# YiyanXu/DiFashion

Hardware: AMD Instinct MI355X
Metric: U-Net denoise steps/sec, 4-item outfit @ 64x64x4 latent (higher is better)
Workload: dtype bf16; 1 GPU; BASELINE configs[1]: one 4-item outfit, CFG on (4 branches) -> U-Net batch 16, DDIM-50 schedule, sd15 shape in_channels=8, 64x64x4 latents, 77 text tokens; one outfit per GPU; unet_batch=16, latent=64x64x4, parallelism=outfit-replicas x1 (no data-path collective)

## Files before the change

### difashion_amd/_lib.py

```python
from __future__ import annotations

import ctypes as C
import os
import subprocess

_HERE = os.path.dirname(os.path.abspath(__file__))
CSRC = os.path.join(_HERE, "csrc")
_LIB_NAMES = {"bf16": "libdifashion_hip.so", "fp16": "libdifashion_hip_f16.so"}


def _env_storage() -> str:
    v = (os.environ.get("DFH_STORAGE") or "bf16").strip().lower()
    if v not in _LIB_NAMES:
        raise ValueError(f"DFH_STORAGE={v!r}: the storage format is 'bf16' (default) or 'fp16'")
    return v


_STORAGE = _env_storage()
LIB_PATH = os.environ.get("DFH_LIB") or os.path.join(CSRC, _LIB_NAMES[_STORAGE])
HEADER = os.path.join(os.path.dirname(_HERE), "include", "difashion_hip.h")

DFH_MAX_BLOCKS = 4


# ... 210 lines not shown
    "dfh_imgproc_crop_top": (_i, [_vp]),
    "dfh_imgproc_crop_left": (_i, [_vp]),
    "dfh_imgproc_ksize_x": (_i, [_vp]),
    "dfh_imgproc_ksize_y": (_i, [_vp]),
    "dfh_imgproc_table_bytes": (_sz, [_vp]),
    "dfh_imgproc_fill_tables": (_i, [_vp, _vp, _sz]),
    "dfh_imgproc_run": (_i, [_vp, _vp, _vp, _vp, _i, _i, _vp, _vp, _vp]),
    "dfh_jpeg_quant_tables": (_i, [_i, C.POINTER(C.c_int), C.POINTER(C.c_int)]),
    "dfh_jpeg_workspace_bytes": (_sz, [_i, _i, _i, _i]),
    "dfh_jpeg_coef_count": (_sz, [_i, _i, _i, _i]),
    "dfh_jpeg_roundtrip": (_i, [_vp, _i, _i, _i, _i, _i, _i, _vp, _vp, _vp, _sz, _vp]),
    "dfh_lpips_create": (_i, [C.POINTER(LpipsConfigC), C.POINTER(_vp)]),
    "dfh_lpips_destroy": (None, [_vp]),
    "dfh_lpips_num_params": (_i, [_vp]),
    "dfh_lpips_param_name": (C.c_char_p, [_vp, _i]),
    "dfh_lpips_param_ndim": (_i, [_vp, _i]),
    "dfh_lpips_param_dim": (_i, [_vp, _i, _i]),
    "dfh_lpips_packed_bytes": (_sz, [_vp]),
    "dfh_lpips_pack": (_i, [_vp, C.POINTER(_vp), _i, _vp, _vp]),
    "dfh_lpips_workspace_bytes": (_sz, [_vp, _i, _i, _i]),
    "dfh_lpips_forward": (_i, [_vp, C.POINTER(_vp), _i, _vp, _vp, _vp, _i, _vp, _i, _i, _i, _i, _vp, _vp, _vp, _sz, _vp]),
    "dfh_lpips_group_argmin": (_i, [_vp, _vp, _i, _i, _vp]),
    "dfh_lpips_prep": (_i, [_vp, _i, _vp, _vp, _vp, _i, _vp, _i, _i, _i, _vp]),
    "dfh_lpips_conv3x3_relu": (_i, [_vp, _vp, _i, _vp, _vp, _vp, _i, _i, _i, _i, _i, _vp]),
    "dfh_lpips_maxpool2x2": (_i, [_vp, _vp, _i, _i, _i, _i, _vp]),
    "dfh_lpips_layer_score": (_i, [_vp, _vp, _i, _i, _i, _i, _vp, _vp, _vp]),
    "dfh_incep_create": (_i, [C.POINTER(IncepConfigC), C.POINTER(_vp)]),
    "dfh_incep_destroy": (None, [_vp]),
    "dfh_incep_num_params": (_i, [_vp]),
    "dfh_incep_param_name": (C.c_char_p, [_vp, _i]),
    "dfh_incep_param_ndim": (_i, [_vp, _i]),
    "dfh_incep_param_dim": (_i, [_vp, _i, _i]),
    "dfh_incep_packed_bytes": (_sz, [_vp]),
    "dfh_incep_pack": (_i, [_vp, C.POINTER(_vp), _i, _vp, _vp]),
    "dfh_incep_plan_count": (_i, [_vp, _i, _i, _i]),
    "dfh_incep_plan_entry": (_i, [_vp, _i, _i, _i, _i, C.POINTER(IncepLaunchC)]),
    "dfh_incep_workspace_bytes": (_sz, [_vp, _i, _i, _i]),
    "dfh_incep_forward": (_i, [_vp, C.POINTER(_vp), _i, _vp, _vp, _i, _i, _i, C.POINTER(_vp), _vp, _vp, _sz, _vp]),
    "dfh_incep_prep": (_i, [_vp, _i, _i, _i, _i, _i, _i, _vp, _vp]),
    "dfh_incep_conv_bn_relu": (_i, [_vp, _vp, _i, C.POINTER(_vp), _vp, _vp, _i, _i, _i, _i, _i, _i, _i, _i, _i, _i, _i, _i, _vp]),
    "dfh_incep_pool": (_i, [_vp, _vp, _i, _i, _i, _i, _i, _i, _i, _vp]),
    "dfh_incep_global_mean": (_i, [_vp, _vp, _i, _i, _i, _vp]),
    "dfh_incep_fc_softmax": (_i, [_vp, _vp, _vp, _vp, _vp, _i, _i, _i, _vp]),
    "dfh_incep_is_rows": (_i, [_vp, _vp, _i, _i, _f, _vp, _vp, _vp, _vp, _vp]),
    "dfh_incep_is_splits": (_i, [_vp, _vp, _vp, _i, _i, _vp, _vp]),
    "dfh_incep_stats": (_i, [_vp, _i, _i, _vp, _vp, _vp]),
    "dfh_vae_create": (_i, [C.POINTER(VAEConfigC), C.POINTER(_vp)]),
    "dfh_vae_destroy": (None, [_vp]),
    "dfh_vae_num_params": (_i, [_vp]),
    "dfh_vae_param_name": (C.c_char_p, [_vp, _i]),
    "dfh_vae_param_ndim": (_i, [_vp, _i]),
    "dfh_vae_param_dim": (_i, [_vp, _i, _i]),
    "dfh_vae_arena16_bytes": (_sz, [_vp]),
    "dfh_vae_arena32_bytes": (_sz, [_vp]),
    "dfh_vae_workspace_bytes": (_sz, [_vp, _i, _i, _i]),
    "dfh_vae_bind": (_i, [_vp, _vp, _vp, _vp, _sz]),
    "dfh_vae_pack": (_i, [_vp, C.POINTER(_vp), _i, _vp]),
    "dfh_vae_encode": (_i, [_vp, _vp, _vp, _i, _i, _vp]),
    "dfh_vae_decode": (_i, [_vp, _vp, _vp, _i, _i, _vp]),
    "dfh_unet_arena16t_bytes": (_sz, [_vp]),
    "dfh_unet_grad16_bytes": (_sz, [_vp]),
    "dfh_unet_grad32_bytes": (_sz, [_vp]),
    "dfh_unet_train_workspace_bytes": (_sz, [_vp, _i]),
    "dfh_unet_bind_train": (_i, [_vp, _vp, _vp, _vp, _vp, _sz, _i]),
    "dfh_unet_pack_train": (_i, [_vp, C.POINTER(_vp), _i, _vp]),
    "dfh_unet_pack_all": (_i, [_vp, C.POINTER(_vp), _i, _vp]),
    "dfh_unet_grad_sumsq": (_i, [_vp, _vp]),
    "dfh_unet_forward_train": (_i, [_vp, _vp, _i, _vp, _vp, _i, _vp, _i, _vp]),
    "dfh_unet_backward": (_i, [_vp, _vp, _vp, C.POINTER(_vp), _i, _i, _vp]),
    "dfh_unet_backward_begin": (_i, [_vp, _vp, _vp, _sz, _vp]),
    "dfh_unet_backward_next": (_i, [_vp, C.POINTER(_sz), C.POINTER(_sz), _vp]),
    "dfh_unet_backward_finish": (_i, [_vp, C.POINTER(_vp), _i, _i, _vp]),
    "dfh_gemm_partial_floats": (_sz, [C.POINTER(GemmDesc)]),
    "dfh_gemm": (_i, [C.POINTER(GemmDesc), _vp]),
    "dfh_gemm_wgrad": (_i, [C.POINTER(GemmDesc), _vp, _i, _vp, _i, _i, _vp]),
    "dfh_gemm_wgrad_partial_floats": (_sz, [C.POINTER(GemmDesc), _i]),
    "dfh_groupnorm_fold": (_i, [_vp, _i, _i, _i, _i, _vp, _vp, C.c_float, _vp, _i, _vp, _vp, _i, _i, _vp, _vp, _vp, _vp]),
    "dfh_gemm_wgrad_plan": (_i, [C.POINTER(GemmDesc), _i, C.POINTER(C.c_int), C.POINTER(C.c_int), C.POINTER(C.c_int)]),
    "dfh_gemm_plan": (_i, [C.POINTER(GemmDesc), C.POINTER(GemmPlanExtra), C.POINTER(GemmPlanInfo)]),
    "dfh_colsum": (_i, [_vp, _i, _i, _i, _i, _vp, _i, _vp]),
    "dfh_groupnorm": (_i, [_vp, _i, _vp, _i, _i, _i, _i, _vp, _vp, _f, _i, _vp, _vp, _vp]),
    "dfh_gemm_gstat": (_i, [C.POINTER(GemmDesc), _vp, C.POINTER(C.c_int)]),
    "dfh_groupnorm_pre": (_i, [_vp, _i, _i, _i, _i, _vp, _vp, _f, _i, _vp, _vp, _i, _vp, _vp]),
    "dfh_groupnorm_stats": (_i, [_vp, _i, _vp, _i, _i, _i, _i, _vp, _vp, _f, _i, _vp, _vp, _vp, _vp]),
    "dfh_groupnorm_bwd": (_i, [_vp, _i, _vp, _i, _vp, _i, _i, _i, _vp, _vp, _vp, _i, _vp, _i, _vp, _i, _vp, _vp, _vp, _vp]),
    "dfh_attention_lse": (_i, [_vp, _i, _vp, _i, _vp, _i, _vp, _i, _i, _i, _i, _i, _i, _f, _vp, _vp]),
    "dfh_attention_delta": (_i, [_vp, _vp, _i, _vp, _i, _i, _i, _i, _vp]),
    "dfh_attention_bwd": (_i, [_vp, _i, _vp, _i, _vp, _i, _vp, _i, _vp, _vp, _vp, _i, _vp, _i, _vp, _i, _i, _i, _i, _i, _i, _f, _vp]),
    "dfh_layernorm_bwd": (_i, [_vp, _vp, _vp, _vp, _i, _vp, _vp, _i, _i, _f, _vp]),
    "dfh_pack_matrix_t": (_i, [_vp, _vp, _i, _i, _i, _i, _i, _i, _vp]),
    "dfh_pack_conv3x3_t": (_i, [_vp, _vp, _i, _i, _i, _i, _i, _vp]),
    "dfh_unpack_matrix": (_i, [_vp, _vp, _i, _i, _i, _i, _i, _i, _vp]),
    "dfh_unpack_conv3x3": (_i, [_vp, _vp, _i, _i, _i, _i, _i, _vp]),
    "dfh_unpack_vector": (_i, [_vp, _vp, _i, _i, _i, _vp]),
    "dfh_pool2x2_sum": (_i, [_vp, _vp, _i, _i, _i, _i, _vp]),
    "dfh_add_bf16": (_i, [_vp, _vp, _sz, _i, _vp]),
    "dfh_geglu_fwd": (_i, [_vp, _vp, _sz, _i, _vp]),
    "dfh_geglu_bwd": (_i, [_vp, _vp, _vp, _sz, _i, _vp]),
    "dfh_act_fwd": (_i, [_vp, _vp, _sz, _i, _vp]),
    "dfh_act_bwd": (_i, [_vp, _vp, _vp, _vp, _vp, _sz, _i, _f, _vp]),
    "dfh_nhwc_to_nchw_f32": (_i, [_vp, _vp, _i, _i, _i, _i, _f, _i, _vp]),
    "dfh_transpose_bf16": (_i, [_vp, _vp, _i, _i, _i, _i, _i, _sz, _sz, _vp]),
    "dfh_mse_bwd": (_i, [_vp, _vp, _vp, _vp, _i, _i, _f, _vp, _vp]),
    "dfh_assemble_bwd": (_i, [_vp, _vp, _vp, _i, _i, _f, _vp]),
    "dfh_sumsq": (_i, [_vp, _sz, _vp, _vp]),
    "dfh_adamw": (_i, [_vp, _vp, _vp, _vp, _sz, _f, _f, _f, _f, _f, _i, _vp, _f, _vp]),
    "dfh_ema": (_i, [_vp, _vp, _sz, _f, _vp]),
    "dfh_adamw_ema": (_i, [_vp, _vp, _vp, _vp, _vp, _sz, _f, _f, _f, _f, _f, _i, _vp, _f, _f, _vp]),
    "dfh_q8_table": (_i, [_i, _vp]),
    "dfh_q8_quantize": (_i, [_vp, _vp, _vp, _sz, _i, _vp]),
    "dfh_q8_dequantize": (_i, [_vp, _vp, _vp, _sz, _i, _vp]),
    "dfh_adamw8": (_i, [_vp, _vp, _vp, _vp, _vp, _vp, _vp, _sz, _f, _f, _f, _f, _f, _i, _vp, _f, _f, _vp]),
    "dfh_wire_pack": (_i, [_vp, _vp, _sz, _sz, _vp]),
    "dfh_wire_shard_mean": (_i, [_vp, _vp, _i, _sz, _vp]),
    "dfh_wire_unpack": (_i, [_vp, _vp, _sz, _vp]),
    "dfh_layernorm": (_i, [_vp, _vp, _vp, _vp, _i, _i, _f, _vp]),
    "dfh_gemm_out2": (_i, [C.POINTER(GemmDesc), _vp, _i, _i, _vp]),
    "dfh_ups_phase_fold": (_i, [_vp, _i, _vp, _i, _i, _vp]),
    "dfh_conv_up2x": (_i, [_vp, _i, _i, _i, _i, _vp, _i, _vp, _vp, _vp, _vp]),
    "dfh_wino_weights": (_i, [_vp, _i, _vp, _i, _i, _i, _vp]),
    "dfh_wino_blocked": (_i, [_i, _i]),
    "dfh_prof_saved_flops": (C.c_double, []),
    "dfh_wino_input": (_i, [_vp, _vp, _i, _i, _i, _i, _vp]),
    "dfh_gn_wino_input_ok": (_i, [_i, _i, _i, _i, _i]),
    "dfh_gn_wino_input_chain": (_i, [_vp, _vp, _vp, _i, _i, _i, _vp, _vp, _f, _i, _vp, _i, _i, _i, _vp]),
    "dfh_gn_wino_input": (_i, [_vp, _i, _vp, _i, _vp, _vp, _f, _i, _vp, _i, _i, _i, _vp]),
    "dfh_conv3x3_wino_scratch_bytes": (C.c_size_t, [_i, _i, _i, _i, _i]),
    "dfh_conv3x3_wino": (_i, [_vp, _i, _i, _i, _i, _vp, _i, _i, _vp, _vp, _i, _i, _vp, _vp, _vp, C.c_size_t, _vp, _vp]),
    "dfh_gemm_batched": (_i, [C.POINTER(GemmDesc), _i, C.c_long, C.c_long, C.c_long, _vp]),
    "dfh_ln_fold": (_i, [_vp, _i, _vp, _vp, _vp, _vp, _vp, _vp, _i, _i, _vp]),
    "dfh_gemm_ln": (_i, [C.POINTER(GemmDesc), _vp, C.POINTER(C.c_int), _vp, _i, _i, _f, _vp, _vp]),
    "dfh_quantize_rows_fp8": (_i, [_vp, _i, _vp, _vp, _i, _i, _vp]),
    "dfh_layernorm_fp8": (_i, [_vp, _vp, _vp, _vp, _vp, _i, _i, _f, _vp]),
    "dfh_gemm_fp8": (_i, [C.POINTER(Fp8GemmDesc), _vp]),
    "dfh_mlp_fused_image_bytes": (_sz, []),
    "dfh_mlp_fused_pack": (_i, [_vp, _vp, _vp, _vp, _vp, _i, _vp]),
    "dfh_mlp_fused": (_i, [_vp, _vp, _vp, _vp, _i, _i, _f, _vp, _vp, _i, _i, _vp, _i, _i, _vp]),
    "dfh_groupnorm_fp8": (_i, [_vp, _i, _i, _i, _i, _f, _f, _vp, _vp, _vp]),
    "dfh_attention_fp8out": (_i, [_vp, _i, _vp, _i, _vp, _i, _vp, _i, _vp, _i, _i, _i, _i, _i, _f, _vp]),
    "dfh_amax_slabs": (_i, [_vp, C.c_long, _i, _i, _vp, _vp, _vp, _i, _i, _vp]),
    "dfh_attention_fp8": (_i, [_vp, _i, _vp, _i, _vp, _i, _vp, _i, _vp, _vp, _vp, _vp, _i, _i, _i, _i, _i, _f, _vp]),
    "dfh_attn_scales": (_i, [_vp, _vp, _i, _i, _vp, _vp, _vp, _vp, _vp]),
    "dfh_unet_enable_fp8": (_i, [_vp]),
    "dfh_unet_enable_fp8_attention": (_i, [_vp, _i]),
    "dfh_unet_arena8_bytes": (_sz, [_vp]),
    "dfh_unet_bind_fp8": (_i, [_vp, _vp]),
    "dfh_attention": (_i, [_vp, _i, _vp, _i, _vp, _i, _vp, _i, _i, _i, _i, _i, _i, _f, _vp]),
    "dfh_timestep_embedding": (_i, [_vp, _vp, _i, _i, _vp]),
    "dfh_nchw_to_nhwc_bf16": (_i, [_vp, _i, _vp, _i, _i, _i, _vp]),
    "dfh_cast_f32_to_bf16": (_i, [_vp, _vp, _sz, _vp]),
    "dfh_pack_conv3x3": (_i, [_vp, _vp, _i, _i, _i, _i, _vp]),
    "dfh_pack_matrix": (_i, [_vp, _vp, _i, _i, _i, _i, _i, _i, _vp]),
    "dfh_pack_vector": (_i, [_vp, _vp, _i, _i, _i, _i, _vp]),
    "dfh_mutual_reduce": (_i, [_vp, _vp, _vp, _vp, _vp, _vp, _i, _i, _i, _vp]),
    "dfh_assemble_input": (_i, [_vp, _vp, _vp, _vp, _vp, _vp, _vp, _i, _i, _i, _f, _f, _i, _vp]),
    "dfh_cfg_step": (_i, [_vp, _vp, _vp, _vp, _sz, _i, _f, _f, _f, C.POINTER(StepCoef), _vp]),
    "dfh_cfg_multistep": (_i, [_vp] * 9 + [_sz, _i, _f, _f, _f, C.POINTER(MultistepCoef), _vp]),
    "dfh_noise_mix": (_i, [_vp, _vp, _vp, _vp, _vp, _vp, _vp, _i, _i, _vp]),
    "dfh_mse_rows": (_i, [_vp, _vp, _vp, _i, _i, _vp]),
}
_NO_STATUS = {"dfh_abi_version", "dfh_census_count", "dfh_unet_num_params", "dfh_unet_param_ndim", "dfh_unet_param_dim", "dfh_vae_num_params",
              "dfh_vae_param_ndim", "dfh_vae_param_dim", "dfh_clip_num_params", "dfh_clip_param_ndim", "dfh_clip_param_dim",
              "dfh_clipv_num_params", "dfh_clipv_param_ndim", "dfh_clipv_param_dim", "dfh_lpips_num_params", "dfh_lpips_param_ndim", "dfh_lpips_param_dim",
              "dfh_imgproc_resized_height", "dfh_imgproc_resized_width", "dfh_imgproc_out_height", "dfh_imgproc_out_width", "dfh_imgproc_crop_top",
              "dfh_imgproc_crop_left", "dfh_imgproc_ksize_x", "dfh_imgproc_ksize_y",
              "dfh_incep_num_params", "dfh_incep_param_ndim", "dfh_incep_param_dim"}

_lib = None
_UNBOUND = set()
ABI_VERSION = 8


def storage() -> str:
    return _STORAGE


def set_storage(name: str) -> None:
    global _STORAGE, LIB_PATH
    name = str(name).strip().lower()
    if name not in _LIB_NAMES:
        raise ValueError(f"set_storage({name!r}): the storage format is 'bf16' or 'fp16'")
    if name == _STORAGE:
        return
    if _lib is not None:
        raise DfhError(f"set_storage({name!r}): the {_STORAGE} library is already loaded ({LIB_PATH}); the storage format is fixed "
                       "per process -- set DFH_STORAGE or call set_storage() before the first use")
    _STORAGE = name
    if not os.environ.get("DFH_LIB"):
        LIB_PATH = os.path.join(CSRC, _LIB_NAMES[name])


def storage_dtype():
    import torch
    return torch.float16 if _STORAGE == "fp16" else torch.bfloat16


def dtype_code(t, what: str = "tensor") -> int:
    import torch
    if t.dtype == torch.float32:
        return 0
    if t.dtype == storage_dtype():
        return 1
# ... 144 lines not shown
```

### difashion_amd/csrc/api.hip

```cpp
#include <cstdio>
#include <cstdlib>
#include <cstring>
#include <string>
#include <vector>

#include "../../include/difashion_hip.h"
#include "attention.h"
#include "dfh_common.h"
#include "elementwise.h"
#include "gemm.h"
#include "gemm_plan.h"
#include "mlp_fused.h"
#include "norm.h"
#include "walk_knobs.h"
#include "wgrad.h"
#include "bwd_elementwise.h"

namespace dfh {
static thread_local std::string g_err;
void set_error(const std::string& msg) { g_err = msg; }
const char* last_error() { return g_err.c_str(); }
int check_launch(const char* what) {
  hipError_t e = hipGetLastError();
  if (e != hipSuccess) {
    g_err = std::string(what) + ": " + hipGetErrorString(e);
    return -2;
  }
  return 0;
}

static long g_census[CK_COUNT] = {0};
void census(int id) { if (id >= 0 && id < CK_COUNT) ++g_census[id]; }
static const char* const kCensusNames[CK_COUNT] = {"gemm_wide", "gemm_8wave", "gemm_lean", "gemm_other", "gemm_row", "splitk_reduce",
    "splitk_fused", "gstat_written", "gn_pre", "gn_stats", "gn_small", "gn_mid", "layernorm", "ln_folded", "attention_x32", "attention_16",
    "gemm_fp8", "text_cached", "conv_phase", "conv_wino", "gemm_rows_geglu", "attention_fp8", "mlp_fused", "gn_folded", "token_linear", "dup_prefix", "gemm_persist",
    "clipv_embed", "clipv_linear", "clipv_layernorm", "clipv_attention", "imgproc", "cliph_attention", "cliph_embed"};

struct ProfRec { hipEvent_t e0, e1; int cls; double flops, bytes; };
static std::vector<ProfRec> g_recs;
static std::vector<hipEvent_t> g_pool;
static size_t g_pool_next = 0;
static bool g_prof = false;
bool prof_enabled() { return g_prof; }
static hipEvent_t pool_get() {
  if (g_pool_next == g_pool.size()) { hipEvent_t e; (void)hipEventCreate(&e); g_pool.push_back(e); }
  return g_pool[g_pool_next++];
}
void prof_open(int cls, double flops, double bytes, hipStream_t s) {
  ProfRec r; r.e0 = pool_get(); r.e1 = pool_get(); r.cls = cls; r.flops = flops; r.bytes = bytes;
  (void)hipEventRecord(r.e0, s);
  g_recs.push_back(r);
}
void prof_close(hipStream_t s) { (void)hipEventRecord(g_recs.back().e1, s); }
static double g_prof_saved = 0.0;
void prof_note_saved(double flops) { if (g_prof) g_prof_saved += flops; }
}

static int fill_gemm(const dfh_gemm_desc* d, GemmArgs* g) {
  DFH_REQUIRE(d != nullptr, "null descriptor");
  std::memset(g, 0, sizeof(*g));
  if (d->conv) {
    DFH_REQUIRE(d->stride == 1 || d->stride == 2, "stride must be 1 or 2");
    DFH_REQUIRE(!(d->upsample && d->stride != 1), "upsample only with stride 1");
    g->conv_src = (const bf16_t*)d->conv_src; g->conv_c = d->conv_c; g->ntaps = 9;
    g->Hin = d->Hin; g->Win = d->Win; g->stride = d->stride; g->ups = d->upsample;
    g->Hout = d->upsample ? d->Hin * 2 : (d->stride == 2 ? d->Hin / 2 : d->Hin);
    g->Wout = d->upsample ? d->Win * 2 : (d->stride == 2 ? d->Win / 2 : d->Win);
    DFH_REQUIRE(d->M == d->batch * g->Hout * g->Wout, "M must equal batch * Hout * Wout");
  }
  if (d->a0) { g->p_src[g->nplain] = (const bf16_t*)d->a0; g->p_c[g->nplain] = d->a0_c; ++g->nplain; }
  if (d->a1) { DFH_REQUIRE(d->a0 != nullptr, "a1 without a0"); g->p_src[g->nplain] = (const bf16_t*)d->a1; g->p_c[g->nplain] = d->a1_c; ++g->nplain; }
  g->W = (const bf16_t*)d->W; g->ldw = d->ldw; g->zero = (const bf16_t*)d->zero_page;
  g->M = d->M; g->N = d->N;
  g->bias = d->bias; g->rowvec = d->rowvec; g->rv_ld = d->rv_ld; g->rv_off = d->rv_off;
  g->rows_per_b = d->rows_per_b > 0 ? d->rows_per_b : d->M;
  g->w_img_bs = (long)d->w_img_stride;
  g->resid = (const bf16_t*)d->resid; g->ld_res = d->ld_res;
  g->act = d->act; g->out = d->out; g->ld_out = d->ld_out; g->out_mode = d->out_mode;
  g->partial = d->partial;
  DFH_REQUIRE(g->W && g->out, "null W / out");
  return 0;
}

extern "C" {

int dfh_abi_version(void) { return DFH_ABI_VERSION; }

int dfh_prof_begin(void) {
  dfh::g_recs.clear(); dfh::g_pool_next = 0; dfh::g_prof = true; dfh::g_prof_saved = 0.0;
  return 0;
}
double dfh_prof_saved_flops(void) { return dfh::g_prof_saved; }
int dfh_prof_end(dfh_prof_class* out, int max_classes) {
  dfh::g_prof = false;
  DFH_REQUIRE(out != nullptr && max_classes >= dfh::PC_COUNT, "need room for every kernel class");
  static const char* names[dfh::PC_COUNT] = {"gemm_conv3x3", "gemm_linear", "attention", "groupnorm", "layernorm", "splitk_reduce", "other",
                                                  "gemm_wgrad", "attention_bwd", "norm_bwd", "optimizer", "gemm_linear_fp8"};
  for (int i = 0; i < dfh::PC_COUNT; ++i) {
    std::memset(&out[i], 0, sizeof(out[i]));
    std::strncpy(out[i].name, names[i], sizeof(out[i].name) - 1);
  }
  if (hipDeviceSynchronize() != hipSuccess) { dfh::set_error("hipDeviceSynchronize failed in dfh_prof_end"); return -2; }
  const char* dump_path = std::getenv("DFH_PROF_DUMP");
  FILE* dump = dump_path ? std::fopen(dump_path, "w") : nullptr;
  for (const auto& r : dfh::g_recs) {
    float ms = 0.f;
    if (hipEventElapsedTime(&ms, r.e0, r.e1) != hipSuccess) continue;
    out[r.cls].launches += 1; out[r.cls].ms += ms; out[r.cls].flops += r.flops; out[r.cls].bytes += r.bytes;
    if (dump) std::fprintf(dump, "%s %.0f %.0f %.6f\n", names[r.cls], r.flops, r.bytes, ms);
  }
  if (dump) std::fclose(dump);
  dfh::g_recs.clear();
  return dfh::PC_COUNT;
}
void dfh_census_reset(void) { std::memset(dfh::g_census, 0, sizeof(dfh::g_census)); }
int dfh_census_count(void) { return dfh::CK_COUNT; }
const char* dfh_census_name(int i) { return (i >= 0 && i < dfh::CK_COUNT) ? dfh::kCensusNames[i] : ""; }
// ... 50 lines not shown
  w.partial = d->partial; w.partial_cap = d->partial_floats;
  return 0;
}

int dfh_gemm_wgrad(const dfh_gemm_desc* d, const void* dY, int ldy, float* dW, int ldw, int msplit, void* stream) {
  DFH_BF16_ONLY_TRAINING;
  DFH_REQUIRE(d && dY && dW, "null argument");
  WgradArgs w;
  if (int rc = fill_wgrad(d, dY, ldy, dW, ldw, msplit, w)) return rc;
  return dfh::wgrad_launch(w, (hipStream_t)stream);
}

size_t dfh_gemm_wgrad_partial_floats(const dfh_gemm_desc* d, int msplit) {
  DFH_BF16_ONLY_TRAINING_SIZE;
  WgradArgs w;
  if (!d || fill_wgrad(d, nullptr, 8, nullptr, 8, msplit, w)) return 0;
  return dfh::wgrad_partial_floats(w);
}

int dfh_gemm_wgrad_plan(const dfh_gemm_desc* d, int msplit, int* tiles, int* whole_tiles, int* slices) {
  DFH_BF16_ONLY_TRAINING;
  WgradArgs w;
  DFH_REQUIRE(d && tiles && whole_tiles && slices, "null argument");
  if (int rc = fill_wgrad(d, nullptr, 8, nullptr, 8, msplit, w)) return rc;
  dfh::wgrad_plan_only(w);
  *tiles = w.xblocks; *whole_tiles = w.whole; *slices = w.msplit;
  return 0;
}

int dfh_gemm_plan(const dfh_gemm_desc* d, const dfh_gemm_plan_extra* x, dfh_gemm_plan_info* out) {
  DFH_REQUIRE(d && out, "null argument");
  std::memset(out, 0, sizeof(*out));
  static float present[4];
  dfh_gemm_desc t = *d;
  if (!t.W) t.W = present;
  if (!t.out) t.out = present;
  if (!t.zero_page) t.zero_page = present;
  if (!t.partial) t.partial = present;
  GemmArgs g;
  if (int rc = fill_gemm(&t, &g)) return rc;
  if (d->gstat_cpg > 0 && d->gstat_hw > 0) { g.gstat = present; g.gstat_cpg = d->gstat_cpg; g.gstat_hw = d->gstat_hw; }
  if (x) {
    g.nbatch = x->nbatch; g.w_blocked = x->w_blocked;
    if (x->phase2x) { g.phase2x = x->phase2x; g.ntaps = 4; g.nbatch = 4; }
    if (x->n_split > 0) { g.out2 = present; g.ld_out2 = g.rows_per_b; g.n_split = x->n_split; }
    if (x->want_rowstat) g.rowstat = present;
    if (x->ln_cnt > 0) { g.ln_stat = present; g.ln_s = present; g.ln_cnt = x->ln_cnt; g.ln_parts = g.p_c[0] / x->ln_cnt; g.ln_eps = 1e-5f; }
    if (x->pre_out) { g.pre_out = present; g.ld_pre = g.N; }
  }
  const GemmArgs given = g;
  dfh::GemmPlan p;
  const int rc = dfh::gemm_plan(g, dfh::gemm_force_decode(d->force_tile, d->force_split, d->force_order), dfh::GemmKnobs::from_env(), p);
  dfh::gemm_plan_format(out->line, sizeof(out->line), given, rc ? nullptr : &p, rc ? dfh::last_error() : nullptr);
  if (rc) return rc;
  out->kernel = p.kernel; out->tile = p.tile; out->bm = p.bm; out->bn = p.bn; out->stages = p.stages; out->lean = p.lean; out->wide = p.wide;
  out->split = p.split; out->n_major = p.n_major; out->tm_xm = p.tm_xm; out->tm_gm = p.tm_gm; out->gstat_rows = p.gstat_rows;
  out->rowstat_bn = p.rowstat_bn; out->census = p.census;
  return 0;
}

int dfh_colsum(const void* Y, int ldy, int N, int groups, int rows_per_group, float* out, int ld_out, void* stream) {
  DFH_BF16_ONLY_TRAINING;
  DFH_REQUIRE(Y && out, "null argument");
  return dfh::colsum_launch((const bf16_t*)Y, ldy, N, groups, rows_per_group, out, ld_out, (hipStream_t)stream);
}

int dfh_groupnorm(const void* src0, int c0, const void* src1, int c1, int batch, int hw, int groups, const float* gamma,
                  const float* beta, float eps, int silu, void* out, float* partial, void* stream) {
  GnArgs a; std::memset(&a, 0, sizeof(a));
  a.src0 = (const bf16_t*)src0; a.C0 = c0; a.src1 = (const bf16_t*)src1; a.C1 = src1 ? c1 : 0;
  a.B = batch; a.HW = hw; a.G = groups; a.gamma = gamma; a.beta = beta; a.eps = eps; a.silu = silu;
  a.out = (bf16_t*)out; a.partial = partial;
  return dfh::groupnorm_launch(a, (hipStream_t)stream);
}

int dfh_groupnorm_pre(const void* src, int c, int batch, int hw, int groups, const float* gamma, const float* beta, float eps, int silu,
                      void* out, const float* gstat, int chunks, float* stats_out, void* stream) {
  GnArgs a; std::memset(&a, 0, sizeof(a));
  a.src0 = (const bf16_t*)src; a.C0 = c; a.B = batch; a.HW = hw; a.G = groups; a.gamma = gamma; a.beta = beta; a.eps = eps;
  a.silu = silu; a.out = (bf16_t*)out; a.pre = gstat; a.pre_chunks = chunks; a.stats_out = stats_out;
  return dfh::groupnorm_launch(a, (hipStream_t)stream);
}

int dfh_groupnorm_stats(const void* src0, int c0, const void* src1, int c1, int batch, int hw, int groups, const float* gamma,
                        const float* beta, float eps, int silu, void* out, float* partial, float* stats_out, void* stream) {
  GnArgs a; std::memset(&a, 0, sizeof(a));
  a.src0 = (const bf16_t*)src0; a.C0 = c0; a.src1 = (const bf16_t*)src1; a.C1 = src1 ? c1 : 0;
  a.B = batch; a.HW = hw; a.G = groups; a.gamma = gamma; a.beta = beta; a.eps = eps; a.silu = silu;
  a.out = (bf16_t*)out; a.partial = partial; a.stats_out = stats_out;
  return dfh::groupnorm_launch(a, (hipStream_t)stream);
}
int dfh_groupnorm_bwd(const void* src0, int c0, const void* src1, int c1, const void* dy, int batch, int hw, int groups,
                      const float* gamma, const float* beta, const float* stats, int silu, void* dx0, int acc0, void* dx1,
                      int acc1, float* dgamma, float* dbeta, float* partial, void* stream) {
  DFH_BF16_ONLY_TRAINING;
  GnBwdArgs a; std::memset(&a, 0, sizeof(a));
  a.src0 = (const bf16_t*)src0; a.C0 = c0; a.src1 = (const bf16_t*)src1; a.C1 = src1 ? c1 : 0; a.dy = (const bf16_t*)dy;
  a.B = batch; a.HW = hw; a.G = groups; a.gamma = gamma; a.beta = beta; a.stats = stats; a.silu = silu;
  a.dx0 = (bf16_t*)dx0; a.dx1 = (bf16_t*)dx1; a.acc0 = acc0; a.acc1 = acc1; a.dgamma = dgamma; a.dbeta = dbeta; a.partial = partial;
  return dfh::groupnorm_bwd_launch(a, (hipStream_t)stream);
}
int dfh_attention_lse(const void* Q, int ldq, const void* K, int ldk, const void* Vt, int ldvt, void* O, int ldo, int batch,
                      int heads, int head_dim, int Nq, int Nk, float scale, float* lse, void* stream) {
  AttnArgs a; std::memset(&a, 0, sizeof(a));
  a.Q = (const bf16_t*)Q; a.ldq = ldq; a.K = (const bf16_t*)K; a.ldk = ldk; a.Vt = (const bf16_t*)Vt; a.ldvt = ldvt;
  a.O = (bf16_t*)O; a.ldo = ldo; a.B = batch; a.H = heads; a.D = head_dim; a.Nq = Nq; a.Nk = Nk; a.scale = scale; a.lse = lse;
  return dfh::attention_launch(a, (hipStream_t)stream);
}
int dfh_attention_delta(const void* O, const void* dO, int ld, float* delta, int batch, int heads, int head_dim, int Nq, void* stream) {
  DFH_BF16_ONLY_TRAINING;
  return dfh::attention_delta_launch((const bf16_t*)O, (const bf16_t*)dO, ld, delta, batch, heads, head_dim, Nq, (hipStream_t)stream);
}
int dfh_attention_bwd(const void* Q, int ldq, const void* K, int ldk, const void* V, int ldv, const void* dO, int ldo,
                      const float* lse, const float* delta, void* dQ, int lddq, void* dK, int lddk, void* dV, int lddv, int batch,
                      int heads, int head_dim, int Nq, int Nk, float scale, void* stream) {
  DFH_BF16_ONLY_TRAINING;
  AttnBwdArgs a; std::memset(&a, 0, sizeof(a));
  a.Q = (const bf16_t*)Q; a.ldq = ldq; a.K = (const bf16_t*)K; a.ldk = ldk; a.V = (const bf16_t*)V; a.ldv = ldv;
  a.dO = (const bf16_t*)dO; a.ldo = ldo; a.lse = lse; a.delta = delta;
  a.dQ = (bf16_t*)dQ; a.lddq = lddq; a.dK = (bf16_t*)dK; a.lddk = lddk; a.dV = (bf16_t*)dV; a.lddv = lddv;
  a.B = batch; a.H = heads; a.D = head_dim; a.Nq = Nq; a.Nk = Nk; a.scale = scale;
  return dfh::attention_bwd_launch(a, (hipStream_t)stream);
}
int dfh_layernorm_bwd(const void* x, const void* dy, const float* gamma, void* dx, int accumulate, float* dgamma, float* dbeta,
                      int M, int C, float eps, void* stream) {
  DFH_BF16_ONLY_TRAINING;
  return dfh::layernorm_bwd_launch((const bf16_t*)x, (const bf16_t*)dy, gamma, (bf16_t*)dx, accumulate, dgamma, dbeta, M, C, eps,
                                   (hipStream_t)stream);
}
int dfh_pack_matrix_t(const float* w, void* out, int N, int K, int ldt, int t_row_off, int t_col_off, int geglu, void* stream) {
  DFH_BF16_ONLY_TRAINING;
  return dfh::pack_matrix_t_launch(w, (bf16_t*)out, N, K, ldt, t_row_off, t_col_off, geglu, (hipStream_t)stream);
}
int dfh_pack_conv3x3_t(const float* w, void* out, int Cout, int Cin, int ldt, int t_col_off, int o_pad, void* stream) {
  DFH_BF16_ONLY_TRAINING;
  return dfh::pack_conv3x3_t_launch(w, (bf16_t*)out, Cout, Cin, ldt, t_col_off, o_pad, (hipStream_t)stream);
}
int dfh_unpack_matrix(const float* g, float* grad, int N, int K, int ldw, int row_off, int col_off, int geglu, void* stream) {
  DFH_BF16_ONLY_TRAINING;
  return dfh::unpack_matrix_launch(g, grad, N, K, ldw, row_off, col_off, geglu, (hipStream_t)stream);
}
int dfh_unpack_conv3x3(const float* g, float* grad, int Cout, int Cin, int ldw, int col_off, int cin_pad, void* stream) {
  DFH_BF16_ONLY_TRAINING;
  return dfh::unpack_conv3x3_launch(g, grad, Cout, Cin, ldw, col_off, cin_pad, (hipStream_t)stream);
}
int dfh_unpack_vector(const float* g, float* grad, int N, int off, int geglu, void* stream) {
  DFH_BF16_ONLY_TRAINING;
  return dfh::unpack_vector_launch(g, grad, N, off, geglu, (hipStream_t)stream);
}
int dfh_pool2x2_sum(const void* in, void* out, int batch, int H, int W, int C, void* stream) {
  return dfh::pool2x2_sum_launch((const bf16_t*)in, (bf16_t*)out, batch, H, W, C, (hipStream_t)stream);
}
int dfh_add_bf16(void* dst, const void* src, size_t n, int accumulate, void* stream) {
  return dfh::add_bf16_launch((bf16_t*)dst, (const bf16_t*)src, (long)n, accumulate, (hipStream_t)stream);
}
int dfh_geglu_fwd(const void* pre, void* y, size_t M, int N2, void* stream) {
  return dfh::geglu_fwd_launch((const bf16_t*)pre, (bf16_t*)y, (long)M, N2, (hipStream_t)stream);
}
int dfh_geglu_bwd(const void* pre, const void* dy, void* dpre, size_t M, int N2, void* stream) {
  DFH_BF16_ONLY_TRAINING;
  return dfh::geglu_bwd_launch((const bf16_t*)pre, (const bf16_t*)dy, (bf16_t*)dpre, (long)M, N2, (hipStream_t)stream);
}
int dfh_act_fwd(const void* pre, void* y, size_t n, int kind, void* stream) {
  return dfh::act_fwd_launch((const bf16_t*)pre, (bf16_t*)y, (long)n, kind, (hipStream_t)stream);
}
int dfh_act_bwd(const void* ref_bf16, const float* ref_f32, const void* dy_bf16, const float* dy_f32, void* dpre, size_t n, int kind,
// ... 48 lines not shown
}
int dfh_q8_dequantize(const unsigned char* codes, const float* absmax, float* x, size_t n, int is_signed, void* stream) {
  DFH_BF16_ONLY_TRAINING;
  DFH_REQUIRE(x != nullptr && codes != nullptr && absmax != nullptr, "null pointer");
  return dfh::q8_dequantize_launch(codes, absmax, x, (long)n, is_signed, (hipStream_t)stream);
}
int dfh_adamw8(float* p, const float* g, unsigned char* m8, float* m_absmax, unsigned char* v8, float* v_absmax, float* shadow, size_t n,
               float lr, float beta1, float beta2, float eps, float weight_decay, int step, const float* sumsq, float max_norm,
               float ema_decay, void* stream) {
  DFH_BF16_ONLY_TRAINING;
  DFH_REQUIRE(p != nullptr && g != nullptr && m8 != nullptr && m_absmax != nullptr && v8 != nullptr && v_absmax != nullptr, "null pointer");
  return dfh::adamw8_launch(p, g, m8, m_absmax, v8, v_absmax, shadow, (long)n, lr, beta1, beta2, eps, weight_decay, step, sumsq, max_norm,
                            ema_decay, (hipStream_t)stream);
}

int dfh_wire_pack(const float* g, void* wire, size_t n, size_t n_pad, void* stream) {
  DFH_BF16_ONLY_TRAINING;
  return dfh::wire_pack_launch(g, (bf16_t*)wire, (long)n, (long)n_pad, (hipStream_t)stream);
}
int dfh_wire_shard_mean(const void* recv, void* shard, int world, size_t per, void* stream) {
  DFH_BF16_ONLY_TRAINING;
  return dfh::wire_shard_mean_launch((const bf16_t*)recv, (bf16_t*)shard, world, (long)per, (hipStream_t)stream);
}
int dfh_wire_unpack(const void* wire, float* g, size_t n, void* stream) {
  DFH_BF16_ONLY_TRAINING;
  return dfh::wire_unpack_launch((const bf16_t*)wire, g, (long)n, (hipStream_t)stream);
}

int dfh_layernorm(const void* x, const float* gamma, const float* beta, void* y, int M, int C, float eps, void* stream) {
  return dfh::layernorm_launch((const bf16_t*)x, gamma, beta, (bf16_t*)y, M, C, eps, (hipStream_t)stream);
}

int dfh_groupnorm_fold(const void* x, int B, int HW, int C, int G, const float* gamma, const float* beta, float eps, const float* pre,
                       int pre_chunks, float* partial, const void* W, int ldw, int N, const float* bias, void* Wimg, float* rv, void* stream) {
  GnFoldArgs f; std::memset(&f, 0, sizeof(f));
  f.x = (const bf16_t*)x; f.B = B; f.HW = HW; f.C = C; f.G = G; f.eps = eps; f.gamma = gamma; f.beta = beta; f.pre = pre; f.pre_chunks = pre_chunks;
  f.partial = partial; f.W = (const bf16_t*)W; f.ldw = ldw; f.N = N; f.bias = bias; f.Wimg = (bf16_t*)Wimg; f.rv = rv;
  return dfh::groupnorm_fold_launch(f, (hipStream_t)stream);
}

int dfh_ln_fold(const void* W, int ldw, const float* gamma, const float* beta, const float* bias, void* WF, float* s, float* b, int N, int K,
                void* stream) {
  return dfh::ln_fold_launch((const bf16_t*)W, ldw, gamma, beta, bias, (bf16_t*)WF, s, b, N, K, (hipStream_t)stream);
}

int dfh_gemm_ln(const dfh_gemm_desc* d, float* rowstat, int* rowstat_bn, const float* ln_stat, int ln_parts, int ln_cnt, float ln_eps,
                const float* ln_s, void* stream) {
  GemmArgs g;
  if (int rc = fill_gemm(d, &g)) return rc;
  const size_t need = d->force_split > 1 ? (size_t)d->force_split * g.M * g.N : dfh::gemm_partial_floats(g);
  DFH_REQUIRE(need == 0 || (d->partial && d->partial_floats >= need), "partial buffer too small for split-K");
  g.rowstat = rowstat;
  g.ln_stat = ln_stat; g.ln_parts = ln_parts; g.ln_cnt = ln_cnt; g.ln_eps = ln_eps; g.ln_s = ln_s;
  if (ln_stat) DFH_REQUIRE(dfh::gemm_ln_consumer_ok(g), "this launch shape cannot consume folded-LayerNorm statistics (split-K / unstaged GEGLU)");
  int bn = 0;
  const int rc = dfh::gemm_launch(g, (hipStream_t)stream, d->force_tile, d->force_split, d->force_order, nullptr, &bn);
  if (rowstat_bn) *rowstat_bn = bn;
  return rc;
}

int dfh_gemm_out2(const dfh_gemm_desc* d, void* out2, int ld_out2, int n_split, void* stream) {
  GemmArgs g;
  if (int rc = fill_gemm(d, &g)) return rc;
  DFH_REQUIRE(out2 != nullptr, "null argument");
  g.out2 = out2; g.ld_out2 = ld_out2; g.n_split = n_split;
  DFH_REQUIRE(dfh::gemm_out2_ok(g), "this launch cannot carry a second destination (split-K, or n_split is no multiple of its column tile)");
  const int ft = (d->force_tile == 10 || d->force_tile == 24) ? d->force_tile : 0;
  return dfh::gemm_launch(g, (hipStream_t)stream, ft, 0, d->force_order);
}

int dfh_ups_phase_fold(const void* W, int ldw, void* WP, int N, int C, void* stream) {
  return dfh::ups_phase_fold_launch((const bf16_t*)W, ldw, (bf16_t*)WP, N, C, (hipStream_t)stream);
}
int dfh_conv_up2x(const void* src, int batch, int H, int W, int C, const void* WP, int N, const float* bias, void* out,
                  const void* zero_page, void* stream) {
  DFH_REQUIRE(src && WP && out && zero_page, "null argument");
  DFH_REQUIRE(batch > 0 && H > 0 && W > 0 && C > 0 && C % 8 == 0 && N > 0 && N % 8 == 0, "bad shape (C and N multiples of 8)");
  GemmArgs g; std::memset(&g, 0, sizeof(g));
  g.M = batch * H * W; g.N = N; g.rows_per_b = H * W; g.out_mode = OUT_BF16; g.ld_out = N;
  g.conv_src = (const bf16_t*)src; g.conv_c = C; g.ntaps = 4; g.phase2x = 1; g.nbatch = 4; g.w_bs = (long)N * 4 * C;
  g.Hin = H; g.Win = W; g.Hout = H; g.Wout = W; g.stride = 1;
  g.W = (const bf16_t*)WP; g.ldw = 4 * C; g.bias = bias; g.out = out; g.zero = (const bf16_t*)zero_page;
  return dfh::gemm_launch(g, (hipStream_t)stream, 0, 0, -1);
}
int dfh_wino_weights(const void* W, int ldw, void* U, int N, int C, int blocked, void* stream) {
  return dfh::wino_weight_launch((const bf16_t*)W, ldw, (bf16_t*)U, N, C, blocked, (hipStream_t)stream);
}
int dfh_wino_blocked(int N, int C) { return dfh::wino_blocked(N, C) ? 1 : 0; }
int dfh_wino_input(const void* src, void* V, int batch, int H, int W, int C, void* stream) {
  return dfh::wino_input_launch((const bf16_t*)src, (bf16_t*)V, batch, H, W, C, (hipStream_t)stream);
}
int dfh_gn_wino_input_ok(int c0, int c1, int groups, int H, int W) { return dfh::gn_wino_ok(c0, c1, groups, H, W) ? 1 : 0; }
int dfh_gn_wino_input(const void* src0, int c0, const void* src1, int c1, const float* gamma, const float* beta, float eps, int groups,
                      void* V, int batch, int H, int W, void* stream) {
  return dfh::gn_wino_input_launch((const bf16_t*)src0, c0, (const bf16_t*)src1, c1, gamma, beta, eps, groups, (bf16_t*)V, batch, H, W,
                                   (hipStream_t)stream);
}
int dfh_gn_wino_input_chain(const void* Mprev, const float* pbias, const float* prowvec, int prv_ld, int prv_off, int C, const float* gamma,
                            const float* beta, float eps, int groups, void* V, int batch, int H, int W, void* stream) {
  DFH_REQUIRE(Mprev != nullptr, "null argument");
  return dfh::gn_wino_input_launch((const bf16_t*)Mprev, C, nullptr, 0, gamma, beta, eps, groups, (bf16_t*)V, batch, H, W, (hipStream_t)stream,
                                   (const bf16_t*)Mprev, pbias, prowvec, prv_ld, prv_off);
}
size_t dfh_conv3x3_wino_scratch_bytes(int batch, int H, int W, int C, int N) {
  if (batch <= 0 || H <= 0 || W <= 0 || C <= 0 || N <= 0) return 0;
  const size_t mt = (size_t)batch * (H / 2) * (W / 2);
  return ((16 * mt * C * 2 + 255) & ~(size_t)255) + ((16 * mt * N * 2 + 255) & ~(size_t)255);
}
int dfh_conv3x3_wino(const void* src, int batch, int H, int W, int C, const void* U, int u_blocked, int N, const float* bias, const float* rowvec,
                     int rv_ld, int rv_off, const void* resid, void* out, void* scratch, size_t scratch_bytes, const void* zero_page,
                     void* stream) {
  DFH_REQUIRE(src && U && bias && out && scratch && zero_page, "null argument");
  DFH_REQUIRE(batch > 0 && H > 0 && W > 0 && (H & 1) == 0 && (W & 1) == 0 && C > 0 && C % 8 == 0 && N > 0 && N % 8 == 0,
              "even image sides, channel counts multiples of 8");
  DFH_REQUIRE(scratch_bytes >= dfh_conv3x3_wino_scratch_bytes(batch, H, W, C, N) && (uintptr_t)scratch % 256 == 0, "scratch too small or misaligned");
  const long mt = (long)batch * (H / 2) * (W / 2);
  bf16_t* V = (bf16_t*)scratch;
  bf16_t* Mb = (bf16_t*)((char*)scratch + ((16 * (size_t)mt * C * 2 + 255) & ~(size_t)255));
  hipStream_t s = (hipStream_t)stream;
  if (int rc = dfh::wino_input_launch((const bf16_t*)src, V, batch, H, W, C, s)) return rc;
  GemmArgs g; std::memset(&g, 0, sizeof(g));
  g.M = (int)mt; g.N = N; g.rows_per_b = (int)mt; g.out_mode = OUT_BF16; g.ld_out = N;
  g.p_src[0] = V; g.p_c[0] = C; g.nplain = 1; g.W = (const bf16_t*)U; g.ldw = C;
  g.nbatch = 16; g.a_bs = mt * C; g.w_bs = (long)N * C; g.o_bs = mt * N; g.w_blocked = u_blocked;
  g.out = Mb; g.zero = (const bf16_t*)zero_page;
  g.prof_flops = 2.0 * batch * H * W * (double)N * 9.0 * C;
  if (int rc = dfh::gemm_launch(g, s, dfh::wino_gemm_tile(g), 0, -1)) return rc;
  return dfh::wino_output_launch(Mb, (bf16_t*)out, bias, rowvec, rv_ld, rv_off, (const bf16_t*)resid, batch, H, W, N, s);
}
int dfh_gemm_batched(const dfh_gemm_desc* d, int nbatch, long a_bs, long w_bs, long o_bs, void* stream) {
  GemmArgs g;
  if (int rc = fill_gemm(d, &g)) return rc;
  DFH_REQUIRE(nbatch >= 1, "nbatch must be positive");
  g.nbatch = nbatch; g.a_bs = a_bs; g.w_bs = w_bs; g.o_bs = o_bs;
  return dfh::gemm_launch(g, (hipStream_t)stream, d->force_tile, 0, d->force_order);
}

int dfh_gemm_fp8(const dfh_gemm_fp8_desc* d, void* stream) {
  DFH_BF16_ONLY_FP8;
  DFH_REQUIRE(d != nullptr, "null descriptor");
  Fp8GemmArgs g; std::memset(&g, 0, sizeof(g));
  g.A = (const uint8_t*)d->A; g.lda = d->lda; g.sA = d->sA; g.sa_div = d->sa_div; g.sa_mul = d->sa_mul; g.sx = (const uint8_t*)d->sx;
  g.W = (const uint8_t*)d->W; g.sW = d->sW; g.M = d->M; g.N = d->N; g.K = d->K; g.bias = d->bias;
  g.resid = (const bf16_t*)d->resid; g.ld_res = d->ld_res; g.act = d->act; g.out = d->out; g.ld_out = d->ld_out; g.out_mode = d->out_mode;
  g.out_sx = (uint8_t*)d->out_sx; g.rows_per_b = d->rows_per_b; g.amax = d->amax; g.zero = (const uint8_t*)d->zero_page;
  return dfh::gemm_fp8_launch(g, (hipStream_t)stream);
}
size_t dfh_mlp_fused_image_bytes(void) { return dfh::mlp_fused_image_bytes(); }
int dfh_mlp_fused_pack(const void* w1, const float* s1, const float* b1, const void* w2p, void* img, int form, void* stream) {
#ifdef DFH_PROBES
  if (form == 1) return dfh::mlp_pack_launch((const bf16_t*)w1, s1, b1, (const bf16_t*)w2p, img, (hipStream_t)stream);
#endif
  DFH_REQUIRE(form == 2, "fused MLP: form 2 (form 1 is a probe kernel: scripts/probes)");
  return dfh::mlp2_pack_launch((const bf16_t*)w1, s1, b1, (const bf16_t*)w2p, img, (hipStream_t)stream);
}
int dfh_mlp_fused(const void* x, const void* resid, const void* img, const float* ln_stat, int ln_parts, int ln_cnt, float ln_eps,
                  const float* bias, void* out, int M, int form, float* gstat, int gstat_cpg, int gstat_hw, void* stream) {
#ifndef DFH_PROBES
  DFH_REQUIRE(form == 2, "fused MLP: form 2 (form 1 is a probe kernel: scripts/probes)");
#endif
  DFH_REQUIRE(form == 1 || form == 2, "fused MLP: form 1 or 2");
  DFH_REQUIRE(gstat == nullptr || form == 2, "fused MLP: output statistics are written by form 2 only");
  MlpArgs a; std::memset(&a, 0, sizeof(a));
  a.gstat = gstat; a.gstat_cpg = gstat_cpg; a.gstat_hw = gstat_hw;
  a.x = (const bf16_t*)x; a.resid = (const bf16_t*)resid; a.img = (const unsigned char*)img; a.ln_stat = ln_stat; a.ln_parts = ln_parts;
  a.ln_cnt = ln_cnt; a.ln_eps = ln_eps; a.bias = bias; a.out = (bf16_t*)out; a.M = M;
// ... 136 lines not shown
```

### difashion_amd/csrc/dfh_common.h

```cpp
#pragma once
#include <hip/hip_runtime.h>
#include <stdint.h>

typedef uint16_t bf16_t;

typedef __attribute__((ext_vector_type(4))) float f32x4_t;
typedef __attribute__((ext_vector_type(2))) float f32x2_t;

#define DFH_DEVICE __device__ __forceinline__

#ifdef DFH_F16
#define DFH_STORAGE_NAME "fp16"
typedef __attribute__((ext_vector_type(8))) _Float16 h16x8_t;
typedef __attribute__((ext_vector_type(2))) _Float16 h16x2_t;
#define DFH_MFMA_16x16x32 __builtin_amdgcn_mfma_f32_16x16x32_f16
#define DFH_MFMA_32x32x16 __builtin_amdgcn_mfma_f32_32x32x16_f16
#define DFH_MFMA_16x16x32_ASM "v_mfma_f32_16x16x32_f16"
#define DFH_MFMA_32x32x16_ASM "v_mfma_f32_32x32x16_f16"
#define DFH_H16_ONE 0x3C00
#define DFH_H16_ONE2 0x3c003c00u
#define DFH_H16_ONE_LO 0x00003c00u
constexpr bool DFH_H16_WIDE_EXPONENT = false;
constexpr float DFH_H16_MAX = 65504.0f;

// ... 140 lines not shown

DFH_DEVICE uint2 geglu4p(const f32x4_t v, const f32x4_t g, const float4 bv, const float4 bg, const GeluK& k, uint2& pre_v, uint2& pre_g) {
  const f32x2_t v0 = f32x2_t{v[0] + bv.x, v[1] + bv.y}, v1 = f32x2_t{v[2] + bv.z, v[3] + bv.w};
  const f32x2_t g0 = f32x2_t{g[0] + bg.x, g[1] + bg.y}, g1 = f32x2_t{g[2] + bg.z, g[3] + bg.w};
  pre_v.x = pack2bf(v0[0], v0[1]); pre_v.y = pack2bf(v1[0], v1[1]);
  pre_g.x = pack2bf(g0[0], g0[1]); pre_g.y = pack2bf(g1[0], g1[1]);
  const f32x2_t o0 = v0 * gelu_erf_f2(g0, k), o1 = v1 * gelu_erf_f2(g1, k);
  uint2 o;
  o.x = pack2bf(o0[0], o0[1]); o.y = pack2bf(o1[0], o1[1]);
  return o;
}

DFH_DEVICE float lane_xor16(float x) {
  const unsigned u = __float_as_uint(x);
  const auto r = __builtin_amdgcn_permlane16_swap(u, u, false, false);
  const bool odd_row = (__lane_id() & 16) != 0;
  return __uint_as_float(odd_row ? r[0] : r[1]);
}
DFH_DEVICE float lane_xor32(float x) {
  const unsigned u = __float_as_uint(x);
  const auto r = __builtin_amdgcn_permlane32_swap(u, u, false, false);
  const bool upper = (__lane_id() & 32) != 0;
  return __uint_as_float(upper ? r[0] : r[1]);
}
DFH_DEVICE float rows_max(float x) {
  unsigned u = __float_as_uint(x);
  auto r = __builtin_amdgcn_permlane16_swap(u, u, false, false);
  u = __float_as_uint(fmaxf(__uint_as_float(r[0]), __uint_as_float(r[1])));
  r = __builtin_amdgcn_permlane32_swap(u, u, false, false);
  return fmaxf(__uint_as_float(r[0]), __uint_as_float(r[1]));
}
DFH_DEVICE float rows_sum(float x) {
  unsigned u = __float_as_uint(x);
  auto r = __builtin_amdgcn_permlane16_swap(u, u, false, false);
  u = __float_as_uint(__uint_as_float(r[0]) + __uint_as_float(r[1]));
  r = __builtin_amdgcn_permlane32_swap(u, u, false, false);
  return __uint_as_float(r[0]) + __uint_as_float(r[1]);
}
DFH_DEVICE float wave_sum(float v) {
#pragma unroll
  for (int o = 8; o > 0; o >>= 1) v += __shfl_xor(v, o, 64);
  return rows_sum(v);
}

#include <string>
#include <vector>
namespace dfh {
struct ParamDesc { std::string name; std::vector<int> shape; };
struct ParamList {
  std::vector<ParamDesc> params;
  int add_param(const std::string& name, std::vector<int> shape) { params.push_back({name, std::move(shape)}); return (int)params.size() - 1; }
  int num_params() const { return (int)params.size(); }
  const char* param_name(int i) const { return i >= 0 && i < num_params() ? params[i].name.c_str() : ""; }
  int param_ndim(int i) const { return i >= 0 && i < num_params() ? (int)params[i].shape.size() : 0; }
  int param_dim(int i, int d) const { return d >= 0 && d < param_ndim(i) ? params[i].shape[d] : 0; }
};
void set_error(const std::string& msg);
const char* last_error();
int check_launch(const char* what);
struct WorkspaceCarve {
  float* base; size_t round, floats = 0;
  WorkspaceCarve(void* b, size_t round_floats) : base((float*)b), round(round_floats) {}
  float* take(size_t n) { float* p = base ? base + floats : nullptr; floats += (n + round - 1) / round * round; return p; }
  size_t bytes() const { return floats * sizeof(float) + 256; }
};
template <class NameOf>
int check_param_pointers(const float* const* params, int count, const std::string& who, NameOf name_of) {
  for (int i = 0; i < count; ++i) {
    const char* fault = params[i] == nullptr ? "null parameter pointer" : ((uintptr_t)params[i] & 15) != 0 ? "parameter pointer not 16-byte aligned" : nullptr;
    if (fault) { set_error(who + ": " + fault + name_of(i)); return -1; }
  }
  return 0;
}
inline int require_params(const ParamList& t, const float* const* params, int count, const std::string& who, const std::string& count_query,
                          const std::string& arg = "params") {
  if (!params) { set_error(who + ": null argument: " + arg); return -1; }
  if (count != t.num_params()) { set_error(who + ": " + arg + " count does not match " + count_query); return -1; }
  return check_param_pointers(params, count, who, [&](int i) { return ": " + t.params[i].name; });
}
inline bool aligned16(const void* p) { return ((uintptr_t)p & 15) == 0; }
enum ProfClass { PC_CONV3 = 0, PC_LINEAR = 1, PC_ATTN = 2, PC_GNORM = 3, PC_LNORM = 4, PC_SPLITK = 5, PC_OTHER = 6,
                 PC_WGRAD = 7, PC_ATTN_BWD = 8, PC_NORM_BWD = 9, PC_OPTIM = 10, PC_LINEAR_FP8 = 11, PC_COUNT = 12 };
enum CensusId { CK_GEMM_WIDE = 0, CK_GEMM_8WAVE, CK_GEMM_LEAN, CK_GEMM_OTHER, CK_GEMM_ROW, CK_SPLITK, CK_SPLITK_FUSED, CK_GSTAT_WRITTEN,
                CK_GN_PRE, CK_GN_STATS, CK_GN_SMALL, CK_GN_MID, CK_LAYERNORM, CK_LN_FOLDED, CK_ATTN_X32, CK_ATTN_16, CK_GEMM_FP8,
                CK_TEXT_CACHED, CK_CONV_PHASE, CK_CONV_WINO, CK_GEMM_ROWS_GEGLU, CK_ATTN_FP8, CK_MLP_FUSED, CK_GN_FOLDED, CK_TOKEN_LINEAR, CK_DUP_PREFIX, CK_GEMM_PERSIST,
                CK_CLIPV_EMBED, CK_CLIPV_LINEAR, CK_CLIPV_LAYERNORM, CK_CLIPV_ATTN, CK_IMGPROC, CK_CLIPH_ATTN, CK_CLIPH_EMBED, CK_COUNT };
void census(int id);
bool prof_enabled();
void prof_open(int cls, double flops, double bytes, hipStream_t s);
void prof_close(hipStream_t s);
void prof_note_saved(double flops);
struct ProfScope {
  hipStream_t s; bool on;
  ProfScope(int cls, double flops, double bytes, hipStream_t st) : s(st), on(prof_enabled()) { if (on) prof_open(cls, flops, bytes, s); }
  ~ProfScope() { if (on) prof_close(s); }
};
}
#define DFH_REQUIRE(cond, msg)                                   \
  do {                                                           \
    if (!(cond)) {                                               \
      dfh::set_error(std::string(__func__) + ": " + (msg));      \
      return -1;                                                 \
    }                                                            \
  } while (0)

#ifdef DFH_F16
#define DFH_BF16_ONLY_TRAINING_SIZE do { dfh::set_error(std::string(__func__) + ": refused by the fp16-storage library: training entry points are bf16 only; unset DFH_STORAGE"); return 0; } while (0)
#define DFH_BF16_ONLY_TRAINING DFH_REQUIRE(false, "refused by the fp16-storage library: training / backward / optimizer entry points are bf16 only (no loss scaling); unset DFH_STORAGE")
#define DFH_BF16_ONLY_FP8 DFH_REQUIRE(false, "refused by the fp16-storage library: the fp8 (e4m3) legs are calibrated against bf16 producers; unset DFH_STORAGE")
#else
#define DFH_BF16_ONLY_TRAINING
#define DFH_BF16_ONLY_TRAINING_SIZE
#define DFH_BF16_ONLY_FP8
#endif

DFH_DEVICE int xcd_remap(int bid, int nblk) {
  const int q = nblk >> 3, r = nblk & 7;
  const int xcd = bid & 7, idx = bid >> 3;
  const int base = (xcd < r) ? xcd * (q + 1) : r * (q + 1) + (xcd - r) * q;
  return base + idx;
}

DFH_DEVICE void tile_coords(int bid, int ntm, int ntn, int n_major, int xm, int gm, int& mt, int& nt) {
  if (gm <= 0) {
    const int tile = xcd_remap(bid, ntm * ntn);
    mt = n_major ? tile % ntm : tile / ntn;
    nt = n_major ? tile / ntm : tile % ntn;
    return;
  }
  int rm = ntm, rn = ntn, mbase = 0, nbase = 0, idx;
  const int xn = xm > 0 ? 8 / xm : 0;
  if (xm > 0 && ntm % xm == 0 && ntn % xn == 0) {
    const int xcd = bid & 7;
    rm = ntm / xm; rn = ntn / xn;
    mbase = (xcd / xn) * rm; nbase = (xcd % xn) * rn;
    idx = bid >> 3;
  } else {
    idx = xcd_remap(bid, ntm * ntn);
  }
  const int per = gm * rn, group = idx / per, first = group * gm;
  const int gsz = (rm - first) < gm ? (rm - first) : gm;
  const int w = idx - group * per;
  mt = mbase + first + w % gsz;
  nt = nbase + w / gsz;
}
```

### difashion_amd/csrc/gemm_plan.h

```cpp
#pragma once
#include <stddef.h>
#include "gemm.h"
#include "norm.h"

namespace dfh {

struct GemmForce {
  int tile;
  bool deep;
  bool big, bigg;
  int wide;
  int ws;
  bool halo, persist, token;
  int split, order;
  bool kernel_pinned() const { return wide || ws || halo; }
  bool none() const { return tile == 0 && !kernel_pinned(); }
};
GemmForce gemm_force_decode(int force_tile, int force_split, int force_order);

struct GemmKnobs {
  bool deep4_off, deep4_all;
  int tmap_xm, tmap_gm;
  int big_mode;
  int bigg_mode;
  bool w_blocked_off;
  int wino_tile;
  bool batch_big_off;
  bool batch_nmajor_off;
  bool gstat128_off;
  bool ws_on, halo_on;
  int persist_mode;
  static GemmKnobs defaults();
  static const GemmKnobs& from_env();
};

enum GemmKernel { GK_TILE = 0, GK_BIG, GK_BIG_GEGLU, GK_WIDE,
                  GK_WS, GK_HALO, GK_GEGLU_ROWS, GK_PERSIST, GK_TOKEN_LINEAR,
                  GK_COUNT };
struct GemmTile { int bm, bn, stages; };
extern const GemmTile kGemmTiles[6];
constexpr int kEightWave = 5;

struct GemmPlan {
  int kernel;
  int tile;
  int bm, bn, stages, lean;
  int wide;
  int split;
  int n_major, tm_xm, tm_gm;
  int gstat_rows;
  int rowstat_bn;
  int census;
};

int gemm_plan(GemmArgs& a, const GemmForce& f, const GemmKnobs& k, GemmPlan& p);

bool gemm_lean_plain(const GemmArgs& a);
void gemm_plan_stats(GemmArgs& a, const GemmKnobs& k, GemmPlan& p);
inline bool gstat_chunks_fit(int hw, int rows) { return hw % rows == 0 && hw / rows <= (int)GN_MAX_CHUNKS; }

struct GemmWork { double flops, saved, bytes; int cls; };
GemmWork gemm_work(const GemmArgs& a);

const char* gemm_kernel_name(int kernel);
int gemm_plan_format(char* buf, size_t n, const GemmArgs& given, const GemmPlan* p, const char* refusal);

#ifdef DFH_PROBES
int gemm_plan_probes(GemmArgs& a, const GemmForce& f, const GemmKnobs& k, GemmPlan& p, bool wide_ok);
int gemm_launch_probes(const GemmPlan& p, const GemmArgs& a, hipStream_t stream);
#endif
}
```

### difashion_amd/csrc/gemm_plan.hip

```cpp
#include "gemm_plan.h"

#include <algorithm>
#include <cstdio>
#include <cstdlib>
#include <cstring>
#include <string>

namespace dfh {

namespace {
constexpr int BK = 64;
constexpr int BKW = 32;
constexpr int kNumTiles = 5;
}

const GemmTile kGemmTiles[6] = {{256, 160, 3}, {256, 128, 3}, {128, 64, 3}, {128, 160, 2}, {128, 128, 2}, {128, 160, 2}};

GemmForce gemm_force_decode(int force_tile, int force_split, int force_order) {
  GemmForce f{};
  f.split = force_split; f.order = force_order;
  switch (force_tile) {
    case GF_8WAVE: f.deep = true; break;
    case GF_WS_160: f.ws = 160; break;
    case GF_WS_128: f.ws = 128; break;
    case GF_HALO: f.halo = true; break;
    case GF_BIG: f.big = true; break;
    case GF_BIG_GEGLU: f.bigg = true; break;
    case GF_PERSIST: f.persist = true; break;
    case GF_TOKEN_LINEAR: f.token = true;
    default:
      if (force_tile > kNumTiles) f.wide = force_tile - GF_WIDE + 1;
      else f.tile = force_tile;
  }
  return f;
}

GemmKnobs GemmKnobs::defaults() {
  GemmKnobs k{};
  k.deep4_all = true; k.tmap_xm = -1; k.big_mode = 2; k.bigg_mode = 1; k.wino_tile = -1;
  return k;
}

const GemmKnobs& GemmKnobs::from_env() {
  static const GemmKnobs knobs = [] {
    GemmKnobs k = defaults();
    const auto is = [](const char* name, char c) { const char* e = getenv(name); return e && e[0] == c; };
    const auto num = [](const char* name, int dflt) { const char* e = getenv(name); return e ? atoi(e) : dflt; };
    k.deep4_off = is("DFH_DEEP4", '0');
    k.deep4_all = !is("DFH_DEEP4", '1');
    if (const char* e = getenv("DFH_TMAP")) { const char* c = strchr(e, ','); k.tmap_xm = atoi(e); k.tmap_gm = c ? atoi(c + 1) : 0; }
    k.big_mode = num("DFH_GEMM_BIG", k.big_mode);
    k.bigg_mode = num("DFH_GEMM_BIGG", k.bigg_mode);
    k.w_blocked_off = is("DFH_W_BLOCKED", '0');
    k.wino_tile = num("DFH_WINO_TILE", k.wino_tile);
    k.batch_big_off = is("DFH_BATCH_BIG", '0');
    k.batch_nmajor_off = is("DFH_BATCH_NMAJOR", '0');
    k.gstat128_off = is("DFH_GSTAT128", '0');
    k.ws_on = is("DFH_GEMM_WS", '1'); k.halo_on = is("DFH_GEMM_HALO", '1'); k.persist_mode = num("DFH_PERSIST", 0);
    return k;
  }();
  return knobs;
}

int gemm_count_ksteps(const GemmArgs& a) {
  int n = a.ntaps * ((a.conv_c + BK - 1) / BK);
  for (int i = 0; i < a.nplain; ++i) n += (a.p_c[i] + BK - 1) / BK;
  return n;
}

int gemm_wide_ksteps(const GemmArgs& a) {
  int n = a.ntaps * ((a.conv_c + BKW - 1) / BKW);
  for (int i = 0; i < a.nplain; ++i) n += (a.p_c[i] + BKW - 1) / BKW;
  return n;
}

bool gemm_lean_plain(const GemmArgs& a) {
  if (a.ntaps != 0 || a.nplain < 1 || a.p_c[0] % BK != 0 || a.p_c[0] <= 0) return false;
  const double amax = (double)a.M * std::max(a.p_c[0], a.nplain > 1 ? a.p_c[1] : 0) * 2.0, wmax = (double)a.N * a.ldw * 2.0;
  if (amax >= 4.0e9 || wmax >= 4.0e9) return false;
  return a.nplain == 1 || (a.p_c[1] % BK == 0 && a.p_c[1] > 0);
}

int gemm_pick_split(const GemmArgs& a, int* tile_out) {
  const bool geglu = a.act == ACT_GEGLU;
  const bool n160 = !geglu && (a.N % 160 == 0 || (a.N % 128 != 0 && a.N > 128));
  const int ksteps = gemm_count_ksteps(a);
  if (gemm_act_is_xact(a.act)) {
    if (tile_out) *tile_out = kEightWave;
    return 1;
  }
  int tile;
  if (a.N <= 64 && !geglu) tile = 2;
  else if (a.M > 128 && a.M <= 1024 && ksteps >= 64) tile = n160 ? 0 : 1;
  else tile = n160 ? kEightWave : 4;
  const GemmTile ti = kGemmTiles[tile];
  const int blocks = ((a.M + ti.bm - 1) / ti.bm) * ((a.N + ti.bn - 1) / ti.bn);
  int split = 1;
  if (!geglu && blocks < 384 && ksteps >= (a.ntaps ? 64 : 160)) {
    const int target = ti.bm == 256 ? 256 : 512;
    split = std::max(1, std::min((target + blocks / 2) / blocks, ksteps / 16));
  } else if (!geglu && blocks < 160 && ksteps >= 16) {
    split = std::min({(256 + blocks - 1) / blocks, ksteps / 8, 64});
    if (split < 1) split = 1;
  }
  if (tile_out) *tile_out = tile;
  return split;
}

size_t gemm_partial_floats(const GemmArgs& a) {
  if (a.nbatch > 1) return 0;
  const int s = gemm_pick_split(a, nullptr);
  return s > 1 ? (size_t)s * a.M * a.N : 0;
}

static bool out2_fits(const GemmArgs& a, int tile, int split) {
  return split == 1 && a.n_split > 0 && a.n_split % kGemmTiles[tile].bn == 0 && a.out_mode == OUT_BF16 && a.act != ACT_GEGLU && !a.resid;
}
static bool ln_single_pass(const GemmArgs& a, int split) { return split == 1 && !a.rowvec && !a.resid; }
static bool ln_geglu_staged(const GemmArgs& a) { return a.act != ACT_GEGLU || (a.ld_out & 7) == 0; }

bool gemm_out2_ok(GemmArgs a) {
  int tile;
  const int split = gemm_pick_split(a, &tile);
  return a.out2 != nullptr && a.n_split < a.N && out2_fits(a, tile, split);
}

bool gemm_ln_consumer_ok(GemmArgs a) {
  return ln_single_pass(a, gemm_pick_split(a, nullptr)) && ln_geglu_staged(a) && (a.act != ACT_GEGLU || a.N % 32 == 0) && a.ntaps == 0;
}

static void gemm_pick_tile_order(GemmArgs& a, const GemmKnobs& k, int split, int bm, int bn) {
  a.tm_xm = 0; a.tm_gm = 0;
  if (k.tmap_xm >= 0) {
    a.tm_xm = (k.tmap_xm == 1 || k.tmap_xm == 2 || k.tmap_xm == 4 || k.tmap_xm == 8) ? k.tmap_xm : 0; a.tm_gm = k.tmap_gm; return;
  }
  if (split > 1 || a.n_major) return;
  double kk = (double)a.ntaps * a.conv_c;
  for (int i = 0; i < a.nplain; ++i) kk += a.p_c[i];
  const double w_bytes = (double)a.N * kk * 2.0;
  const double a_bytes = a.ntaps ? (double)(a.M / (a.Hout * a.Wout)) * a.Hin * a.Win * a.conv_c * 2.0 : (double)a.M * kk * 2.0;
  const int ntm = (a.M + bm - 1) / bm, ntn = (a.N + bn - 1) / bn;
  if (w_bytes <= 2.0e6 || ntm < 16) return;
  if (ntn >= 16) { a.tm_gm = 8; return; }
  if (!a.ntaps) return;
  int best = 8; double cost = a_bytes + 8.0 * w_bytes;
  for (int xm = 4; xm >= 2; xm >>= 1) {
    if (ntm % xm || ntn % (8 / xm)) continue;
    const double c = (8.0 / xm) * a_bytes + xm * w_bytes;
    if (c < 0.95 * cost) { cost = c; best = xm; }
  }
  if (best != 8) { a.tm_xm = best; a.tm_gm = 8; }
}

static bool whole_rounds(long tiles, long always_from) {
  const long rem = tiles % 256;
  return tiles >= 224 && (rem == 0 || rem >= 224 || tiles >= always_from);
}

static bool gemm_big_pick(const GemmArgs& a, const GemmKnobs& k) {
  if (k.big_mode == 0) return false;
  if (a.out_mode != OUT_BF16 || a.act == ACT_GEGLU || a.ln_stat) return false;
  if (a.N % 320 != 0 || (a.ld_out & 7) || (a.resid && (a.ld_res & 7))) return false;
  if (a.ksteps < 16 && (a.ntaps || k.big_mode < 3)) return false;
  if (a.ntaps == 0 && k.big_mode < 2) return false;
  return whole_rounds((long)((a.M + 255) / 256) * (a.N / 320), 1024);
}

static bool gemm_big_geglu_pick(const GemmArgs& a, const GemmKnobs& k) {
  if (k.bigg_mode == 0 || a.act != ACT_GEGLU || a.out_mode != OUT_BF16 || a.resid || a.rowvec) return false;
  if (a.N % 256 != 0 || (a.ld_out & 7)) return false;
  return whole_rounds((long)((a.M + 255) / 256) * (a.N / 256), 512);
}

static bool batched_big_pick(const GemmArgs& a, const GemmKnobs& k) {
  if (k.batch_big_off || a.nbatch <= 1 || a.M < 512 || a.N % 320 != 0) return false;
  return whole_rounds((long)((a.M + 255) / 256) * (a.N / 320) * a.nbatch, 1024);
}

bool wino_blocked(int N, int C) {
  return !GemmKnobs::from_env().w_blocked_off && N % 160 == 0 && C % 64 == 0;
}

int wino_gemm_tile(const GemmArgs&) {
  const int pin = GemmKnobs::from_env().wino_tile;
  return pin >= 0 ? pin : 0;
}

int gemm_wide_pick(const GemmArgs& a) {
  if (a.out_mode != OUT_BF16) return 0;
  if (a.ln_stat && !(a.act == ACT_GEGLU && a.N % 128 == 0)) return 0;
  if (a.act == ACT_GEGLU && (a.resid || a.rowvec)) return 0;
  if ((a.N & 7) || (a.ld_out & 7) || (a.resid && (a.ld_res & 7))) return 0;
  if (a.act == ACT_GEGLU && a.N % 128 == 0) return (long)((a.M + 255) / 256) * (a.N / 128) >= 448 ? 4 : 0;
  if (a.act == ACT_GEGLU && a.N % 160 != 0) return 0;
  if (a.N % 160 != 0 && a.N % 128 == 0) {
    return (long)((a.M + 255) / 256) * (a.N / 128) >= 448 ? 4 : 0;
  }
  if (a.N % 160 != 0 && a.N < 640) return 0;
  if (a.ntaps == 0 && a.N % 160 == 0 && !(a.resid && a.nplain == 1 && a.p_c[0] <= 320 && !a.rowstat)) return 0;
  const long nt = (a.N + 159) / 160;
  return (long)((a.M + 255) / 256) * nt >= 448 ? 1 : 0;
}

bool gemm_wide_eligible(const GemmArgs& a) {
  if (a.out_mode != OUT_BF16) return false;
  if (a.act == ACT_GEGLU && (a.N % 160 != 0 || a.resid || a.rowvec)) return false;
  if ((a.N & 7) || (a.ld_out & 7) || (a.resid && (a.ld_res & 7))) return false;
  if (a.N % 160 != 0 && a.N < 640) return false;
  const long tiles = (long)((a.M + 255) / 256) * ((a.N + 159) / 160);
  return tiles >= 448;
}

void gemm_plan_stats(GemmArgs& a, const GemmKnobs& k, GemmPlan& p) {
  const bool big = p.kernel == GK_BIG, wide1 = p.kernel == GK_WIDE && p.wide == 1, halo = p.kernel == GK_HALO;
  const bool tile = p.kernel == GK_TILE || p.kernel == GK_PERSIST;
  const bool staged = p.split == 1 && a.out_mode == OUT_BF16 && (a.N & 7) == 0 && (a.ld_out & 7) == 0;
  const int gbn = big ? 320 : 160;
  const bool gst256 = (halo || big || wide1) && a.M % 256 == 0 && gstat_chunks_fit(a.gstat_hw, 256);
  const bool gst128 = !k.gstat128_off && tile && p.tile == kEightWave && staged && a.M % 128 == 0 && gstat_chunks_fit(a.gstat_hw, 128) &&
                      a.nbatch <= 1 && !a.phase2x && a.out2 == nullptr;
  const bool gst_ok = a.gstat && (gst256 || gst128) && a.gstat_cpg > 0 && gbn % a.gstat_cpg == 0 && a.N % gbn == 0 &&
                      a.N % a.gstat_cpg == 0 && a.act != ACT_GEGLU;
  p.gstat_rows = !gst_ok ? 0 : gst256 ? 256 : 128;
  if (!gst_ok) a.gstat = nullptr;
  const int bn = big ? 320 : wide1 ? 160 : (p.kernel == GK_WIDE && (p.wide == 4 || p.wide == 5)) ? 128 : (tile || p.kernel == GK_BIG_GEGLU) ? kGemmTiles[p.tile].bn : 0;
  const bool rs_ok = a.rowstat && bn > 0 && staged && a.act != ACT_GEGLU && a.N % bn == 0;
  p.rowstat_bn = rs_ok ? bn : 0;
  if (!rs_ok) a.rowstat = nullptr;
}

#define PLAN_REQUIRE(cond, msg) \
  do { if (!(cond)) { set_error(std::string("gemm_launch: ") + (msg)); return -1; } } while (0)

int gemm_plan(GemmArgs& a, const GemmForce& f, const GemmKnobs& k, GemmPlan& p) {
  p = GemmPlan{};
  PLAN_REQUIRE(a.M > 0 && a.N > 0, "empty GEMM");
  PLAN_REQUIRE(a.N % 4 == 0, "N must be a multiple of 4");
  PLAN_REQUIRE(a.ntaps == 0 || a.ntaps == 9 || (a.ntaps == 4 && a.phase2x), "ntaps must be 0 or 9 (4 for the phase planes of an upsample conv)");
  PLAN_REQUIRE(a.ntaps + a.nplain >= 1, "no K segment");
  PLAN_REQUIRE(a.ntaps == 0 || a.conv_c % 8 == 0, "conv channels must be a multiple of 8");
  for (int i = 0; i < a.nplain; ++i) PLAN_REQUIRE(a.p_c[i] % 8 == 0, "segment length must be a multiple of 8");
  PLAN_REQUIRE(a.zero != nullptr, "zero page missing");
  if (a.rows_per_b <= 0) a.rows_per_b = a.M;
  a.ksteps = gemm_count_ksteps(a);

  int tile;
  int split = gemm_pick_split(a, &tile);
  if (f.deep) tile = kEightWave;
  if (f.tile > 0) tile = f.tile - 1;
  if (f.split > 0) split = f.split;
  if (a.act == ACT_GEGLU) {
    PLAN_REQUIRE(a.N % 32 == 0 && kGemmTiles[tile].bn != 160 && split == 1, "GEGLU needs N % 32 == 0, a 64/128-wide tile and no split-K");
    PLAN_REQUIRE(a.out_mode == OUT_BF16 && !a.resid && !a.rowvec, "GEGLU epilogue is bias-only, bf16 out");
  }
  const bool xact = gemm_act_is_xact(a.act);
  if (xact) {
    PLAN_REQUIRE(a.out_mode == OUT_BF16 && a.ntaps == 0 && a.nbatch <= 1 && !a.out2 && !a.pre_out && !a.ln_stat && !a.w_img_bs && !a.w_blocked &&
                 !a.phase2x && (a.N & 7) == 0 && (a.ld_out & 7) == 0 && (!a.resid || (a.ld_res & 7) == 0),
                 "GELU / quick-GELU epilogue: plain linears with a row-major 16-bit output and 16-byte aligned rows only");
    tile = kEightWave; split = 1;
  }
  split = std::min(split, a.ksteps);
  {
    double kk = (double)a.ntaps * a.conv_c;
    for (int i = 0; i < a.nplain; ++i) kk += a.p_c[i];
    const double w_bytes = (double)a.N * kk, a_bytes = (double)a.M * (a.ntaps ? (double)a.conv_c : kk);
    const bool conv_like = a.ntaps || (a.nbatch > 1 && !k.batch_nmajor_off);
    a.n_major = (f.order == 2 || (f.order < 0 && conv_like && w_bytes > a_bytes && a.N > 160)) ? 1 : 0;
  }
  if (a.nbatch > 1) {
    split = 1;
    PLAN_REQUIRE(((a.ntaps == 0 && a.nplain == 1) || (a.phase2x && a.nplain == 0)) && a.out_mode == OUT_BF16 && a.act != ACT_GEGLU &&
                 !a.resid && !a.rowvec && !a.out2 && !a.rowstat && !a.ln_stat && (a.N & 7) == 0 && (a.ld_out & 7) == 0 && f.split <= 1,
                 "batched launch: one plain segment (or the four phase planes of an upsample conv), plain bf16 row-major output, no split-K");
    a.gstat = nullptr;
    if (f.tile == 0 && !f.deep) tile = (a.N % 160 == 0) ? kEightWave : 4;
  }
  PLAN_REQUIRE(!a.phase2x || (a.nbatch == 4 && a.ntaps == 4 && a.stride == 1 && a.ups == 0 && !a.pad0 && a.Hin == a.Hout && a.Win == a.Wout &&
                              a.M % (a.Hout * a.Wout) == 0), "phase planes of an upsample conv: four planes over the source image");
  if (split > 1) PLAN_REQUIRE(a.partial != nullptr, "split-K needs a partial buffer");
  if (a.ln_stat) {
    PLAN_REQUIRE(ln_single_pass(a, split) && a.ln_parts > 0 && a.ln_cnt > 0 && a.ln_s != nullptr,
                 "folded LayerNorm: single-pass launches without rowvec / residual only (gemm_ln_consumer_ok)");
    PLAN_REQUIRE(ln_geglu_staged(a), "folded LayerNorm + GEGLU needs 16-byte aligned output rows");
  }
  if (a.w_img_bs) {
    split = 1;
    PLAN_REQUIRE(a.ntaps == 0 && a.nbatch <= 1 && !a.w_blocked && a.rows_per_b % kGemmTiles[tile].bm == 0 && a.M % a.rows_per_b == 0,
                 "per-image weights: plain segments, images of whole row tiles");
  }
  if (a.w_blocked) PLAN_REQUIRE(gemm_lean_plain(a) && a.N % 16 == 0 && a.ldw % 64 == 0 && a.N % 160 == 0 && f.tile == 0 && split == 1,
                                "blocked W: LEAN launches (plain 64-multiple segments) on the 128 x 160 / 256 x 320 tiles only");
  if (a.out2) PLAN_REQUIRE(out2_fits(a, tile, split) && f.tile == 0, "second destination: single pass, n_split a multiple of the column tile (gemm_out2_ok)");
  if (a.resid) PLAN_REQUIRE((double)a.M * a.ld_res * 2.0 < 4.0e9, "residual tensor must be smaller than 4 GB (32-bit lane offsets)");
  a.ksplit = p.split = split;
  p.tile = tile;

  const bool wide_ok0 = !xact && split == 1 && a.out2 == nullptr && a.out_mode == OUT_BF16 && (a.act != ACT_GEGLU || a.N % 160 == 0 || a.N % 128 == 0) && (a.N & 7) == 0 &&
                        (a.ld_out & 7) == 0 && (!a.resid || (a.ld_res & 7) == 0);
  const bool wide_ok = wide_ok0 && a.nbatch <= 1 && !a.w_img_bs;
  const bool heur = f.none() && f.split == 0;
  const bool force_big = f.big || (a.nbatch > 1 && f.none() && !f.bigg && !f.persist && !f.deep && batched_big_pick(a, k));
  const bool pre = a.pre_out != nullptr;
  if (pre) PLAN_REQUIRE(wide_ok && a.act == ACT_GEGLU && a.N % 128 == 0 && !a.ln_stat && !a.resid && !a.rowvec && (a.ld_pre & 7) == 0 && a.ld_pre >= a.N,
                        "pre_out: GEGLU launches with N % 128 == 0, no split-K, no folded LayerNorm");
  const bool bigg = !pre && wide_ok && !f.deep && !f.persist && a.act == ACT_GEGLU && a.N % 32 == 0 && !a.resid && !a.rowvec &&
                    (f.bigg || (heur && gemm_big_geglu_pick(a, k)));
  const bool big = wide_ok0 && !f.deep && a.act != ACT_GEGLU && !a.ln_stat && (a.nbatch <= 1 || force_big) && !a.w_img_bs && !f.persist &&
                   (force_big || (heur && gemm_big_pick(a, k)));
  p.wide = pre ? 5 : (!wide_ok || f.deep || big || force_big || bigg || f.bigg || f.persist) ? 0 : f.kernel_pinned() ? f.wide : heur ? gemm_wide_pick(a) : 0;
  p.kernel = bigg ? GK_BIG_GEGLU : big ? GK_BIG : p.wide ? GK_WIDE : GK_TILE;
#ifdef DFH_PROBES
  if (const int r = gemm_plan_probes(a, f, k, p, wide_ok)) return r < 0 ? r : 0;
#else
  PLAN_REQUIRE(!f.ws && !f.halo && !(f.wide >= 8 && f.wide <= 14),
               "tile ids 11-20 are probe kernels: build scripts/probes (make -C scripts/probes) and load it with DFH_LIB");
  PLAN_REQUIRE(!f.persist, "tile id 24 is a probe kernel: build scripts/probes (make -C scripts/probes) and load it with DFH_LIB");
#endif

  const bool lean = gemm_lean_plain(a);
  switch (p.kernel) {
    case GK_BIG_GEGLU: case GK_GEGLU_ROWS: p.bm = 256; p.bn = 256; p.stages = 2; p.lean = lean; break;
    case GK_BIG: p.bm = 256; p.bn = 320; p.stages = 2; p.lean = lean; break;
    case GK_WIDE: case GK_HALO: p.bm = p.wide == 2 ? 128 : 256; p.bn = p.wide == 3 ? 320 : (p.wide == 4 || p.wide == 5) ? 128 : 160; p.stages = p.wide == 3 ? 4 : 3; break;
    case GK_WS: p.bm = 256; break;
    default: {
      const GemmTile t = kGemmTiles[p.tile];
      p.bm = t.bm; p.bn = t.bn; p.stages = t.stages;
      if (p.tile == kEightWave) {
        const long wgs = (long)((a.M + 127) / 128) * ((a.N + 159) / 160) * (a.nbatch > 1 ? a.nbatch : 1) * a.ksplit;
        if (!xact && !k.deep4_off && (a.nbatch > 1 || k.deep4_all) && wgs <= 320) p.stages = 4;
        p.lean = lean;
      }
    }
  }
  gemm_pick_tile_order(a, k, split, p.bm, p.bn);
  p.n_major = a.n_major; p.tm_xm = a.tm_xm; p.tm_gm = a.tm_gm;
  gemm_plan_stats(a, k, p);
  p.census = (big || bigg) ? CK_GEMM_ROW : (p.kernel == GK_WIDE || p.kernel == GK_HALO) ? CK_GEMM_WIDE :
             (p.kernel != GK_WS && p.tile == kEightWave) ? (lean ? CK_GEMM_LEAN : CK_GEMM_8WAVE) : CK_GEMM_OTHER;
  return 0;
}

GemmWork gemm_work(const GemmArgs& a) {
  double kreal = (double)a.ntaps * a.conv_c;
  double abytes = a.ntaps ? (double)(a.M / (a.Hout * a.Wout)) * a.Hin * a.Win * a.conv_c * 2.0 : 0.0;
  for (int i = 0; i < a.nplain; ++i) { kreal += a.p_c[i]; abytes += (double)a.M * a.p_c[i] * 2.0; }
  const double obytes = (double)a.M * (a.act == ACT_GEGLU ? a.N / 2 : a.N) * ((a.out_mode == OUT_F32 || a.out_mode == OUT_F32_T) ? 4.0 : 2.0) +
                        (a.resid ? (double)a.M * a.N * 2.0 : 0.0) +
                        (a.pre_out ? (double)a.M * a.N * 2.0 : 0.0);
  const double planes = a.nbatch > 1 ? (double)a.nbatch : 1.0;
  GemmWork w;
  w.flops = a.prof_flops > 0.0 ? a.prof_flops : (a.phase2x ? 9.0 / 4.0 : 1.0) * planes * 2.0 * a.M * a.N * kreal;
  w.saved = w.flops - planes * 2.0 * a.M * a.N * kreal;
  w.bytes = (a.phase2x == 1 ? abytes : planes * abytes) + planes * ((double)a.N * kreal * 2.0 + obytes);
  w.cls = (a.ntaps || a.prof_flops > 0.0) ? PC_CONV3 : PC_LINEAR;
  return w;
}
// ... 20 lines not shown
```

### difashion_amd/csrc/gemm_wide_epilogue.h

```cpp
#pragma once
#include "gemm.h"

namespace {

template <int BM, int BN, int WN, int LDS_BYTES>
DFH_DEVICE void wide_epilogue(const GemmArgs& a, f32x4_t (&acc)[BM / 2 / 16][BN / WN / 16], unsigned char* smem, const int tid,
                              const int wm, const int wn, const int fr, const int fg, const int m0, const int n0) {
  constexpr int NWV = 2 * WN;
  constexpr int TM = BM / 2, TN = BN / WN;
  constexpr int FN = TN / 16;
  constexpr int RSF = BN * 4 + 16;
  constexpr int CPR = BN / 8;
  constexpr int EPI = (64 * CPR) / (NWV * 64);
  static_assert(64 * RSF <= LDS_BYTES, "epilogue tile must fit the pipeline buffers");
  static_assert((64 * CPR) % (NWV * 64) == 0, "whole chunks per thread");
  uint4 rnext[EPI];
  auto fetch_one = [&](int q, int e) {
    const int c = tid + e * NWV * 64;
    const int row = c / CPR, cchunk = c - row * CPR;
    const int m = m0 + q * 64 + row, n = n0 + cchunk * 8;
    rnext[e] = make_uint4(0u, 0u, 0u, 0u);
    if (m < a.M && n < a.N) rnext[e] = *(const uint4*)(a.resid + (long)m * a.ld_res + n);
  };
  auto fetch_resid = [&](int q) {
// ... 95 lines not shown
      } else if (a.act == ACT_LEAKY) {
#pragma unroll
        for (int r = 0; r < 8; ++r) v[r] = v[r] > 0.f ? v[r] : 0.01f * v[r];
      } else if (a.act == ACT_TANH) {
#pragma unroll
        for (int r = 0; r < 8; ++r) v[r] = tanhf(v[r]);
      }
      if (has_resid) {
        float f[8];
        unpack8(rcur, f);
#pragma unroll
        for (int r = 0; r < 8; ++r) v[r] += f[r];
      }
      const uint4 packed = pack8(v);
      long orow = m;
      if (a.phase2x == 1) {
        const int hw = a.Hout * a.Wout, pb = m / hw, rem = m - pb * hw;
        const int oy = rem / a.Wout, ox = rem - oy * a.Wout;
        orow = (long)pb * 4 * hw + (long)(2 * oy + (int)(blockIdx.y >> 1)) * (2 * a.Wout) + 2 * ox + (int)(blockIdx.y & 1);
      }
      *(uint4*)((bf16_t*)a.out + (long)blockIdx.y * a.o_bs + orow * a.ld_out + n) = packed;
      if (gst || rst) {
        float f[8];
        unpack8(packed, f);
        *(float4*)(smem + row * RSF + cchunk * 32) = float4{f[0], f[1], f[2], f[3]};
        *(float4*)(smem + row * RSF + cchunk * 32 + 16) = float4{f[4], f[5], f[6], f[7]};
      }
    }
    if (rst) {
      static_assert(NWV * 64 >= 256, "four threads per row of a 64-row pass");
      __syncthreads();
      if (tid < 256) {
        const int row = tid >> 2, part = tid & 3;
        const unsigned char* src = smem + row * RSF;
        float sum = 0.f;
        for (int c = part; c < BN / 4; c += 4) { const float4 x = *(const float4*)(src + c * 16); sum += (x.x + x.y) + (x.z + x.w); }
        sum += __shfl_xor(sum, 1, 64); sum += __shfl_xor(sum, 2, 64);
        const float mean = sum * (1.0f / BN);
        float m2 = 0.f;
        for (int c = part; c < BN / 4; c += 4) {
          const float4 x = *(const float4*)(src + c * 16);
          const float d0 = x.x - mean, d1 = x.y - mean, d2 = x.z - mean, d3 = x.w - mean;
          m2 = fmaf(d0, d0, m2); m2 = fmaf(d1, d1, m2); m2 = fmaf(d2, d2, m2); m2 = fmaf(d3, d3, m2);
        }
        m2 += __shfl_xor(m2, 1, 64); m2 += __shfl_xor(m2, 2, 64);
        const int m = m0 + q * 64 + row;
        if (part == 0 && m < a.M) *(float2*)(a.rowstat + ((long)(n0 / BN) * a.M + m) * 2) = float2{mean, m2};
      }
    }
    if (gst) {
      __syncthreads();
      if (tid < 4 * CQ) {
        const int cq = tid % CQ, r0 = (tid / CQ) * 16;
#pragma unroll 4
        for (int r = 0; r < 16; ++r) {
          const float4 x = *(const float4*)(smem + (r0 + r) * RSF + cq * 16);
          col_s.x += x.x; col_s.y += x.y; col_s.z += x.z; col_s.w += x.w;
          col_q.x += x.x * x.x; col_q.y += x.y * x.y; col_q.z += x.z * x.z; col_q.w += x.w * x.w;
        }
      }
    }
  }
  if (gst) {
    __syncthreads();
    float* cst = (float*)smem;
    float* qrt = cst + 2 * BN;
    if (tid < 4 * CQ) {
      const int cq = tid % CQ, rq = tid / CQ;
      float* d = qrt + (rq * BN + cq * 4) * 2;
      d[0] = col_s.x; d[1] = col_q.x; d[2] = col_s.y; d[3] = col_q.y; d[4] = col_s.z; d[5] = col_q.z; d[6] = col_s.w; d[7] = col_q.w;
    }
    __syncthreads();
    if (tid < BN) {
      float ss = 0.f, qq = 0.f;
#pragma unroll
      for (int rq = 0; rq < 4; ++rq) { ss += qrt[(rq * BN + tid) * 2]; qq += qrt[(rq * BN + tid) * 2 + 1]; }
      cst[tid * 2] = ss; cst[tid * 2 + 1] = qq;
    }
    __syncthreads();
    const int cpg = a.gstat_cpg;
    if (tid < BN / cpg) {
      float ss = 0.f, qq = 0.f;
      for (int c = tid * cpg; c < (tid + 1) * cpg; ++c) { ss += cst[c * 2]; qq += cst[c * 2 + 1]; }
      const int b = m0 / a.gstat_hw, chunk = (m0 - b * a.gstat_hw) / BM, chunks = a.gstat_hw / BM;
      const int g = (n0 + tid * cpg) / cpg, G = a.N / cpg;
      float* dst = a.gstat + (((long)b * G + g) * chunks + chunk) * 2;
      dst[0] = ss; dst[1] = qq;
    }
  }
}

}
```

### difashion_amd/csrc/norm.h

```cpp
#pragma once
#include "dfh_common.h"
#include <algorithm>

enum { GN_MAX_CHUNKS = 64 };

struct GnArgs {
  const bf16_t* src0; const bf16_t* src1;
  int C0, C1;
  int B, HW, G;
  const float* gamma; const float* beta;
  float eps; int silu;
  bf16_t* out;
  uint8_t* out8; float q_mul;
  float* partial;
  float* stats_out;
  const float* pre; int pre_chunks;
  int C, PL, chunks, pix_per_chunk, apix_per_chunk;
};

struct GnBwdArgs {
  const bf16_t* src0; const bf16_t* src1; int C0, C1;
  const bf16_t* dy;
  int B, HW, G;
  const float* gamma; const float* beta; const float* stats; int silu;
  bf16_t* dx0; bf16_t* dx1; int acc0, acc1;
  float* dgamma; float* dbeta;
  float* partial;
  int C, PL, chunks, pix_per_chunk, apix_per_chunk;
};

struct GnFoldArgs {
  const bf16_t* x; int B, HW, C, G; float eps;
  const float* gamma; const float* beta;
  const float* pre; int pre_chunks;
  float* partial;
  const bf16_t* W; int ldw; int N; const float* bias;
  bf16_t* Wimg;
  float* rv;
};

namespace dfh {
struct GnTwoKernel { int block, achunks; size_t lds; };
template <class Args>
int gn_two_kernel_geometry(Args& a, int stats_target, int apply_target, GnTwoKernel* g) {
  const int C8 = a.C / 8;
  a.PL = std::max(1, std::min(256 / C8, a.HW));
  g->block = ((C8 * a.PL + 63) / 64) * 64;
  DFH_REQUIRE(g->block <= 512, "block too large (more than 4096 channels)");
  const int max_by_pix = (a.HW + a.PL - 1) / a.PL;
  const int chunks = std::max(1, std::min({(stats_target + a.B - 1) / a.B, max_by_pix, (int)GN_MAX_CHUNKS}));
  a.pix_per_chunk = (a.HW + chunks - 1) / chunks;
  a.chunks = (a.HW + a.pix_per_chunk - 1) / a.pix_per_chunk;
  const int ac = std::max(1, std::min((apply_target + a.B - 1) / a.B, max_by_pix));
  a.apix_per_chunk = (a.HW + ac - 1) / ac;
  g->achunks = (a.HW + a.apix_per_chunk - 1) / a.apix_per_chunk;
  g->lds = (size_t)a.PL * a.C * 2 * sizeof(float);
  DFH_REQUIRE(g->lds <= 64 * 1024, "GroupNorm LDS reduction too large");
  return 0;
}

int groupnorm_fold_launch(GnFoldArgs a, hipStream_t stream);
int groupnorm_bwd_launch(GnBwdArgs a, hipStream_t stream);
int layernorm_bwd_launch(const bf16_t* x, const bf16_t* dy, const float* gamma, bf16_t* dx, int accumulate, float* dgamma,
                         float* dbeta, int M, int C, float eps, hipStream_t stream);
int groupnorm_launch(GnArgs a, hipStream_t stream);
int layernorm_launch(const bf16_t* x, const float* gamma, const float* beta, bf16_t* y, int M, int C, float eps,
                     hipStream_t stream);
}
```

### difashion_amd/csrc/norm.hip

```cpp
#include "dfh_common.h"
#include "norm.h"
#include "norm_steps.h"
#include "walk_knobs.h"
#include <cstring>
#include <cstdlib>

namespace {

DFH_DEVICE void gn_sum_sq(const uint4& raw, float* s, float* q) {
  float f[8];
  unpack8(raw, f);
#pragma unroll
  for (int k = 0; k < 8; ++k) { s[k] += f[k]; q[k] += f[k] * f[k]; }
}

__global__ __launch_bounds__(512) void gn_stats_kernel(const GnArgs a) {
  extern __shared__ __attribute__((aligned(16))) float red[];
  const int C8 = a.C >> 3;
  const int tid = threadIdx.x;
  const int o = tid % C8, pl = tid / C8;
  const int b = blockIdx.y;
  const int p_begin = blockIdx.x * a.pix_per_chunk;
  const int p_end = min(a.HW, p_begin + a.pix_per_chunk);
  float s[8], q[8];
#pragma unroll
  for (int k = 0; k < 8; ++k) { s[k] = 0.f; q[k] = 0.f; }
  if (pl < a.PL) {
    int p = p_begin + pl;
    for (; p + 7 * a.PL < p_end; p += 8 * a.PL) {
      uint4 v[8];
#pragma unroll
      for (int u = 0; u < 8; ++u) v[u] = *gn_src(a, b, p + u * a.PL, o);
#pragma unroll
      for (int u = 0; u < 8; ++u) gn_sum_sq(v[u], s, q);
    }
    for (; p + 3 * a.PL < p_end; p += 4 * a.PL) {
      uint4 v[4];
#pragma unroll
      for (int u = 0; u < 4; ++u) v[u] = *gn_src(a, b, p + u * a.PL, o);
#pragma unroll
      for (int u = 0; u < 4; ++u) gn_sum_sq(v[u], s, q);
    }
    for (; p < p_end; p += a.PL) gn_sum_sq(*gn_src(a, b, p, o), s, q);
#pragma unroll
    for (int k = 0; k < 8; ++k) {
      red[((pl * a.C) + o * 8 + k) * 2 + 0] = s[k];
      red[((pl * a.C) + o * 8 + k) * 2 + 1] = q[k];
    }
  }
  __syncthreads();
  if (tid < a.G) {
    const int cpg = a.C / a.G;
    float ss = 0.f, qq = 0.f;
    for (int l = 0; l < a.PL; ++l)
      for (int c = tid * cpg; c < (tid + 1) * cpg; ++c) {
        ss += red[(l * a.C + c) * 2 + 0];
        qq += red[(l * a.C + c) * 2 + 1];
      }
    float* dst = a.partial + (((long)b * a.G + tid) * gridDim.x + blockIdx.x) * 2;
    dst[0] = ss; dst[1] = qq;
  }
}

constexpr int GN_PRE = 6;
__global__ void gn_apply_kernel(const GnArgs a) {
  __shared__ float mean_s[64], rstd_s[64];
  const int C8 = a.C >> 3;
  const int tid = threadIdx.x;
  const int o = tid % C8, pl = tid / C8;
  const int b = blockIdx.y;
  const int cpg = a.C / a.G;
  const int p_begin = blockIdx.x * a.apix_per_chunk;
  const int p_end = min(a.HW, p_begin + a.apix_per_chunk);
  const bool live = pl < a.PL;
  uint4 pre[GN_PRE];
#pragma unroll
  for (int u = 0; u < GN_PRE; ++u) {
    const int p = p_begin + pl + u * a.PL;
    pre[u] = make_uint4(0u, 0u, 0u, 0u);
    if (live && p < p_end) pre[u] = *gn_src(a, b, p, o);
  }
  float gmr[8], btr[8];
  if (live && !a.out8) { load8f(a.gamma + o * 8, gmr); load8f(a.beta + o * 8, btr); }
  __shared__ float2 run_s[64][8];
  const float2 sums = gn_chunk_sums(a.partial, a.chunks, a.G, b, blockDim.x >= (unsigned)a.G * 8u, run_s);
  if (tid < a.G) {
    const float2 mr = gn_mean_rstd(sums, (float)a.HW * (float)cpg, a.eps);
    mean_s[tid] = mr.x;
    rstd_s[tid] = mr.y;
    if (a.stats_out && blockIdx.x == 0) {
      a.stats_out[((long)b * a.G + tid) * 2 + 0] = mr.x;
      a.stats_out[((long)b * a.G + tid) * 2 + 1] = mr.y;
    }
  }
  __syncthreads();
  if (!live) return;
  float sc[8], sh[8];
#pragma unroll
  for (int k = 0; k < 8; ++k) {
    const int c = o * 8 + k;
    const int g = c / cpg;
    const float w = (a.out8 ? a.q_mul : gmr[k]) * rstd_s[g];
    sc[k] = w;
    sh[k] = (a.out8 ? 0.f : btr[k]) - mean_s[g] * w;
  }
  auto emit = [&](const uint4& raw, int p) {
    float f[8];
    unpack8(raw, f);
    if (a.out8) {
#pragma unroll
      for (int k = 0; k < 8; ++k) f[k] = sat_e4m3(f[k] * sc[k] + sh[k]);
      uint2 w;
      w.x = pack4_e4m3(f[0], f[1], f[2], f[3]);
      w.y = pack4_e4m3(f[4], f[5], f[6], f[7]);
      *(uint2*)(a.out8 + ((long)(b * a.HW + p) * a.C + o * 8)) = w;
      return;
    }
#pragma unroll
    for (int k = 0; k < 8; ++k) {
      float y = f[k] * sc[k] + sh[k];
      f[k] = a.silu ? silu_f(y) : y;
    }
    *(uint4*)(a.out + ((long)(b * a.HW + p) * a.C + o * 8)) = pack8(f);
  };
#pragma unroll
  for (int u = 0; u < GN_PRE; ++u) {
    const int p = p_begin + pl + u * a.PL;
    if (p < p_end) emit(pre[u], p);
  }
  int p = p_begin + pl + GN_PRE * a.PL;
  for (; p + 3 * a.PL < p_end; p += 4 * a.PL) {
    uint4 v[4];
#pragma unroll
    for (int u = 0; u < 4; ++u) v[u] = *gn_src(a, b, p + u * a.PL, o);
#pragma unroll
    for (int u = 0; u < 4; ++u) emit(v[u], p + u * a.PL);
  }
  for (; p < p_end; p += a.PL) emit(*gn_src(a, b, p, o), p);
}

template <int MAXO, int R>
__global__ __launch_bounds__(256) void layernorm_kernel(const bf16_t* __restrict__ x, const float* __restrict__ gamma,
                                                        const float* __restrict__ beta, bf16_t* __restrict__ y,
                                                        int M, int C, float eps) {
  const int lane = threadIdx.x & 63;
  const int row0 = (blockIdx.x * 4 + (threadIdx.x >> 6)) * R;
  if (row0 >= M) return;
  const int C8 = C >> 3;
  uint4 raw[R][MAXO];
  ln_load_rows<MAXO, R>(x, row0, M, C, lane, raw);
  float gg[MAXO][8], bb[MAXO][8];
#pragma unroll
  for (int i = 0; i < MAXO; ++i) {
    const int o = lane + i * 64;
    if (o < C8) { load8f(gamma + o * 8, gg[i]); load8f(beta + o * 8, bb[i]); }
  }
#pragma unroll
  for (int r = 0; r < R; ++r) {
    if (row0 + r >= M) break;
    float v[MAXO][8];
#pragma unroll
    for (int i = 0; i < MAXO; ++i) unpack8(raw[r][i], v[i]);
    ln_centre<MAXO>(v, lane, C);
    float q = 0.f;
    {
#pragma clang fp contract(off)
#pragma unroll
      for (int i = 0; i < MAXO; ++i) {
// ... 128 lines not shown
    float t = 0.f;
    for (int k = 0; k < upp; ++k) t += colsum[slot][gi * upp + k];
    return t;
  };
  const float mean = group_total(s, 0) / n;
  float q = 0.f;
#pragma unroll
  for (int u = 0; u < UNITS; ++u) {
    if (pp + u * ppb < a.HW) {
      const float d0 = h16lo(v[u].x) - mean, d1 = h16hi(v[u].x) - mean;
      const float d2 = h16lo(v[u].y) - mean, d3 = h16hi(v[u].y) - mean;
      q += (d0 * d0 + d1 * d1) + (d2 * d2 + d3 * d3);
    }
  }
  const float rstd = rsqrtf(group_total(q, 1) / n + a.eps);
  if (!active) return;
  if (a.stats_out && pp == 0 && j == gi * upp) {
    a.stats_out[((long)b * a.G + g0 + gi) * 2] = mean; a.stats_out[((long)b * a.G + g0 + gi) * 2 + 1] = rstd;
  }
  const float4 gm = *(const float4*)(a.gamma + c), bt = *(const float4*)(a.beta + c);
  const float w0 = rstd * gm.x, w1 = rstd * gm.y, w2 = rstd * gm.z, w3 = rstd * gm.w;
  bf16_t* dst = a.out + (long)b * a.HW * a.C + c;
#pragma unroll
  for (int u = 0; u < UNITS; ++u) {
    const int p = pp + u * ppb;
    if (p < a.HW) {
      float y[4] = {(h16lo(v[u].x) - mean) * w0 + bt.x, (h16hi(v[u].x) - mean) * w1 + bt.y,
                    (h16lo(v[u].y) - mean) * w2 + bt.z, (h16hi(v[u].y) - mean) * w3 + bt.w};
      if (a.silu) {
#pragma unroll
        for (int k = 0; k < 4; ++k) y[k] = silu_f(y[k]);
      }
      uint2 o; o.x = pack2bf(y[0], y[1]); o.y = pack2bf(y[2], y[3]);
      *(uint2*)(dst + (long)p * a.C) = o;
    }
  }
}

namespace {
__global__ __launch_bounds__(256) void gn_fold_kernel(const GnFoldArgs a, const float* __restrict__ partial, int chunks) {
  __shared__ float mean_s[64], rstd_s[64];
  const int tid = threadIdx.x, b = blockIdx.y;
  const int cpg = a.C / a.G;
  const float2 sums = gn_chunk_sums(partial, chunks, a.G, b, false, nullptr);
  if (tid < a.G) {
    const float2 mr = gn_mean_rstd(sums, (float)a.HW * (float)cpg, a.eps);
    mean_s[tid] = mr.x;
    rstd_s[tid] = mr.y;
  }
  __syncthreads();
  const int wave = tid >> 6, lane = tid & 63;
  for (int r = wave; r < 8; r += 4) {
    const int n = blockIdx.x * 8 + r;
    if (n >= a.N) break;
    float acc = 0.f;
    for (int ch = lane; ch < (a.C >> 3); ch += 64) {
      float w[8], o[8];
      unpack8(*(const uint4*)(a.W + (long)n * a.ldw + ch * 8), w);
#pragma unroll
      for (int k = 0; k < 8; ++k) {
        const int c = ch * 8 + k, g = c / cpg;
        o[k] = w[k] * a.gamma[c] * rstd_s[g];
      }
      const uint4 packed = pack8(o);
      float wr[8];
      unpack8(packed, wr);
#pragma unroll
      for (int k = 0; k < 8; ++k) {
        const int c = ch * 8 + k;
        acc += w[k] * a.beta[c] - wr[k] * mean_s[c / cpg];
      }
      *(uint4*)(a.Wimg + ((long)b * a.N + n) * a.C + ch * 8) = packed;
    }
#pragma unroll
    for (int off = 32; off > 0; off >>= 1) acc += __shfl_xor(acc, off, 64);
    if (lane == 0) a.rv[(long)b * a.N + n] = (a.bias ? a.bias[n] : 0.f) + acc;
  }
}
}

namespace dfh {

namespace {
enum GnPath { GN_PRODUCER_STATS, GN_ONE_SLAB, GN_GROUP_QUAD, GN_TWO_KERNEL };
struct GnPlan {
  GnPath path;
  int units;
  int gq, ppb, threads;
};

GnPlan gn_select(const GnArgs& a, const WalkKnobs& knobs) {
  if (a.pre) return {GN_PRODUCER_STATS, 0, 0, 0, 0};
  const int cpg = a.C / a.G, upp = cpg >> 2;
  const long slab = (long)a.HW * upp;
  const bool one_source_per_group = a.C1 == 0 || a.C0 % cpg == 0;
  if ((cpg & 3) == 0 && slab <= 256 * knobs.gn_small_max && one_source_per_group && (long)a.B * a.G >= 64)
    return {GN_ONE_SLAB, slab <= 256 * 8 ? 8 : slab <= 256 * 16 ? 16 : 32, 0, 0, 256};
  if (knobs.gn_mid && !a.out8 && (cpg & 3) == 0 && a.HW <= 256 && a.G % 2 == 0) {
    for (int gq = 4; gq >= 2; gq >>= 1) {
      if (a.G % gq || (long)a.B * (a.G / gq) < 128 || gq * upp > 256) continue;
      const int uppb = gq * upp;
      int threads = 256;
      auto units_at = [&](int t) { return t / uppb < 1 ? 1 << 30 : (a.HW + t / uppb - 1) / (t / uppb); };
      while (threads < 1024 && units_at(threads) > 24) threads *= 2;
      if (threads == 1024 && units_at(1024) > 16) threads = 512;
      const int ppb = threads / uppb;
      if (ppb < 1) continue;
      const int units = (a.HW + ppb - 1) / ppb;
      if (units > 24) continue;
      return {GN_GROUP_QUAD, units <= 4 ? 4 : units <= 8 ? 8 : units <= 16 ? 16 : 24, gq, ppb, threads};
    }
  }
  return {GN_TWO_KERNEL, 0, 0, 0, 0};
}
}

int groupnorm_launch(GnArgs a, hipStream_t stream) {
  a.C = a.C0 + a.C1;
  DFH_REQUIRE(a.C % 8 == 0 && a.C0 % 8 == 0 && a.C1 % 8 == 0, "channels must be multiples of 8");
  DFH_REQUIRE(a.G > 0 && a.G <= 64 && a.C % a.G == 0, "bad group count");
  DFH_REQUIRE(a.C <= 4096, "GroupNorm over more than 4096 channels is not supported");
  DFH_REQUIRE((a.partial != nullptr || a.pre != nullptr) && (a.out != nullptr || a.out8 != nullptr) && a.src0 != nullptr, "null pointer");
  if (a.out8) DFH_REQUIRE(a.C1 == 0 && !a.silu && a.q_mul > 0.f && !a.stats_out, "e4m3 GroupNorm output: one source, no SiLU, a positive scale");
  DFH_REQUIRE(a.C1 == 0 || a.src1 != nullptr, "second source missing");
  if (a.pre) DFH_REQUIRE(a.C1 == 0 && a.pre_chunks > 0 && a.pre_chunks <= (int)GN_MAX_CHUNKS, "producer statistics: one source, 1..64 chunks");
  const WalkKnobs& knobs = WalkKnobs::get();
  const GnPlan plan = gn_select(a, knobs);
  GnTwoKernel tk{};
  if (plan.path == GN_PRODUCER_STATS || plan.path == GN_TWO_KERNEL)
    if (int rc = gn_two_kernel_geometry(a, knobs.gn_sc, knobs.gn_ac, &tk)) return rc;
  ProfScope ps(PC_GNORM, 0.0, (a.out8 ? 3.0 : 4.0) * a.B * (double)a.HW * a.C, stream);
  switch (plan.path) {
    case GN_PRODUCER_STATS:
      a.partial = const_cast<float*>(a.pre); a.chunks = a.pre_chunks;
      census(CK_GN_PRE);
      break;
    case GN_ONE_SLAB: {
      const auto kernel = plan.units == 8 ? gn_small_kernel<8> : plan.units == 16 ? gn_small_kernel<16> : gn_small_kernel<32>;
      census(CK_GN_SMALL);
      hipLaunchKernelGGL(kernel, dim3(a.G, a.B), dim3(plan.threads), 0, stream, a);
      return check_launch("gn_small_kernel");
    }
    case GN_GROUP_QUAD: {
      const auto kernel = plan.units == 4 ? gn_mid_kernel<4> : plan.units == 8 ? gn_mid_kernel<8> : plan.units == 16 ? gn_mid_kernel<16>
                                                                                                  : gn_mid_kernel<24, 512>;
      census(CK_GN_MID);
      hipLaunchKernelGGL(kernel, dim3(a.G / plan.gq, a.B), dim3(plan.threads), 0, stream, a, plan.gq, plan.ppb);
      return check_launch("gn_mid_kernel");
    }
    case GN_TWO_KERNEL:
      census(CK_GN_STATS);
      hipLaunchKernelGGL(gn_stats_kernel, dim3(a.chunks, a.B), dim3(tk.block), tk.lds, stream, a);
      if (int rc = check_launch("gn_stats_kernel")) return rc;
      break;
  }
  hipLaunchKernelGGL(gn_apply_kernel, dim3(tk.achunks, a.B), dim3(tk.block), 0, stream, a);
  return check_launch("gn_apply_kernel");
}

int groupnorm_fold_launch(GnFoldArgs f, hipStream_t stream) {
  DFH_REQUIRE(f.x && f.gamma && f.beta && f.W && f.Wimg && f.rv && (f.pre || f.partial), "groupnorm fold: null pointer");
  DFH_REQUIRE(f.C % 8 == 0 && f.G > 0 && f.G <= 64 && f.C % f.G == 0 && f.C <= 4096 && f.ldw % 8 == 0 && f.ldw >= f.C && f.N > 0, "groupnorm fold: bad shape");
  const float* partial = f.pre;
  int chunks = f.pre_chunks;
  if (!partial) {
    GnArgs a; std::memset(&a, 0, sizeof(a));
    a.src0 = f.x; a.C0 = a.C = f.C; a.B = f.B; a.HW = f.HW; a.G = f.G; a.partial = f.partial;
    GnTwoKernel tk;
    if (int rc = gn_two_kernel_geometry(a, WalkKnobs::get().gn_sc, WalkKnobs::get().gn_ac, &tk)) return rc;
    ProfScope ps(PC_GNORM, 0.0, 2.0 * a.B * (double)a.HW * a.C, stream);
    census(CK_GN_STATS);
    hipLaunchKernelGGL(gn_stats_kernel, dim3(a.chunks, a.B), dim3(tk.block), tk.lds, stream, a);
    if (int rc = check_launch("gn_stats_kernel")) return rc;
    partial = f.partial; chunks = a.chunks;
  } else {
    DFH_REQUIRE(chunks > 0 && chunks <= (int)GN_MAX_CHUNKS, "producer statistics: 1..64 chunks");
  }
  ProfScope ps(PC_GNORM, 0.0, (double)f.N * f.C * 2.0 * (1.0 + f.B), stream);
  census(CK_GN_FOLDED);
  hipLaunchKernelGGL(gn_fold_kernel, dim3((f.N + 7) / 8, f.B), dim3(256), 0, stream, f, partial, chunks);
  return check_launch("gn_fold_kernel");
}

int layernorm_launch(const bf16_t* x, const float* gamma, const float* beta, bf16_t* y, int M, int C, float eps,
                     hipStream_t stream) {
  DFH_REQUIRE(C % 8 == 0 && C <= 8 * 64 * 4, "LayerNorm width must be a multiple of 8 and <= 2048");
  const dim3 block(256);
  ProfScope ps(PC_LNORM, 0.0, 4.0 * (double)M * C, stream);
  census(CK_LAYERNORM);
  if (C <= 512) hipLaunchKernelGGL((layernorm_kernel<1, 4>), dim3((M + 15) / 16), block, 0, stream, x, gamma, beta, y, M, C, eps);
  else if (C <= 1024) hipLaunchKernelGGL((layernorm_kernel<2, 2>), dim3((M + 7) / 8), block, 0, stream, x, gamma, beta, y, M, C, eps);
  else hipLaunchKernelGGL((layernorm_kernel<4, 1>), dim3((M + 3) / 4), block, 0, stream, x, gamma, beta, y, M, C, eps);
  return check_launch("layernorm_kernel");
}

}
```

### difashion_amd/csrc/norm_steps.h

```cpp
#pragma once
#include "dfh_common.h"

template <class Args>
DFH_DEVICE const uint4* gn_src(const Args& a, int b, int p, int o) {
  const int o0 = a.C0 >> 3;
  if (o < o0) return (const uint4*)(a.src0 + ((long)(b * a.HW + p) * a.C0 + o * 8));
  return (const uint4*)(a.src1 + ((long)(b * a.HW + p) * a.C1 + (o - o0) * 8));
}

DFH_DEVICE void load8f(const float* p, float* f) {
  const float4 lo = *(const float4*)p, hi = *(const float4*)(p + 4);
  f[0] = lo.x; f[1] = lo.y; f[2] = lo.z; f[3] = lo.w; f[4] = hi.x; f[5] = hi.y; f[6] = hi.z; f[7] = hi.w;
}

DFH_DEVICE float2 gn_chunk_sums(const float* partial, int chunks, int G, int b, bool wide, float2 (*run_s)[8]) {
  const int tid = threadIdx.x;
  if (wide) {
    if (tid < G * 8) {
      const int g = tid >> 3, sub = tid & 7;
      const int per = (chunks + 7) >> 3, c0 = sub * per, c1 = min(chunks, c0 + per);
      const float2* src = (const float2*)(partial + ((long)b * G + g) * chunks * 2);
      float ss = 0.f, qq = 0.f;
      for (int c = c0; c < c1; ++c) { const float2 v = src[c]; ss += v.x; qq += v.y; }
      run_s[g][sub] = float2{ss, qq};
    }
    __syncthreads();
  }
  float ss = 0.f, qq = 0.f;
  if (tid < G) {
    if (wide) {
#pragma unroll
      for (int sub = 0; sub < 8; ++sub) { ss += run_s[tid][sub].x; qq += run_s[tid][sub].y; }
    } else {
      const float2* src = (const float2*)(partial + ((long)b * G + tid) * chunks * 2);
      for (int c = 0; c < chunks; ++c) { ss += src[c].x; qq += src[c].y; }
    }
  }
  return float2{ss, qq};
}

DFH_DEVICE float2 gn_mean_rstd(float2 sums, float n, float eps) {
  const float mean = sums.x / n;
  const float var = fmaxf(sums.y / n - mean * mean, 0.f);
  return float2{mean, rsqrtf(var + eps)};
}

DFH_DEVICE float block_sum4(float x, float* red4) {
  x = wave_sum(x);
  if ((threadIdx.x & 63) == 0) red4[threadIdx.x >> 6] = x;
  __syncthreads();
  return (red4[0] + red4[1]) + (red4[2] + red4[3]);
}

template <int MAXO, int R>
DFH_DEVICE void ln_load_rows(const bf16_t* __restrict__ x, int row0, int M, int C, int lane, uint4 (&raw)[R][MAXO]) {
  const int C8 = C >> 3;
#pragma unroll
  for (int r = 0; r < R; ++r)
#pragma unroll
    for (int i = 0; i < MAXO; ++i) {
      const int o = lane + i * 64;
      raw[r][i] = make_uint4(0u, 0u, 0u, 0u);
      if (o < C8 && row0 + r < M) raw[r][i] = *(const uint4*)(x + (long)(row0 + r) * C + o * 8);
    }
}
template <int MAXO>
DFH_DEVICE void ln_centre(float (&v)[MAXO][8], int lane, int C) {
  const int C8 = C >> 3;
  float s = 0.f;
#pragma unroll
  for (int i = 0; i < MAXO; ++i) {
    if (lane + i * 64 < C8) {
#pragma unroll
      for (int k = 0; k < 8; ++k) s += v[i][k];
    }
  }
  const float mean = wave_sum(s) / (float)C;
#pragma unroll
  for (int i = 0; i < MAXO; ++i) {
    if (lane + i * 64 < C8) {
#pragma unroll
      for (int k = 0; k < 8; ++k) v[i][k] -= mean;
    }
  }
}
```

### difashion_amd/csrc/unet_walk.hip

```cpp
#include "unet_model.h"

struct dfh_unet::Run : WalkBase {
  dfh_unet* u;
  int temb_ld = 0;
  float* amax_self = nullptr; const float* amax_cross = nullptr;
  const dfh::WalkKnobs& kn = dfh::WalkKnobs::get();

  int Ba;
  Run(dfh_unet* u_, int B_, hipStream_t s_, bool dry_) : WalkBase(*u_, u_->cfg.norm_num_groups, B_, s_, dry_), u(u_), Ba(B_) {}
  Tensor palloc(int H, int W, int C) { return Tensor{(bf16_t*)persist.alloc((size_t)Ba * H * W * C * 2), H, W, C}; }
  Tensor talloc(int H, int W, int C) { return Tensor{(bf16_t*)temp.alloc((size_t)Ba * H * W * C * 2), H, W, C}; }
  void dup_bytes(void* p, size_t per_image, int n) {
    if (rc || dry || n <= 0) return;
    char* c = (char*)p;
    if (hipMemcpyAsync(c + (size_t)(Ba - n) * per_image, c + (size_t)(Ba - 2 * n) * per_image, (size_t)n * per_image, hipMemcpyDeviceToDevice, s) != hipSuccess) {
      dfh::set_error("hipMemcpyAsync failed (dup_bytes)"); rc = -2;
    }
  }
  void dup_images(Tensor& t, int n) {
    t.gst = nullptr;
    dup_bytes(t.p, (size_t)t.H * t.W * t.C * 2, n);
  }

  void gemm(GemmArgs g, Tensor* o = nullptr, Bump* bump = nullptr, int* rs_bn = nullptr) {
    if (rs_bn) *rs_bn = 0;
    if (rc) return;
    float* gst = nullptr;
    const int G = groups;
    if (o && bump && kn.gn_pre && o->C % G == 0 && (dfh::gstat_chunks_fit(o->H * o->W, 256) || dfh::gstat_chunks_fit(o->H * o->W, 128))) {
      gst = (float*)bump->alloc((size_t)Ba * G * ((o->H * o->W) / 128) * 2 * sizeof(float));
      g.gstat = gst; g.gstat_cpg = o->C / G; g.gstat_hw = o->H * o->W;
    }
    if (!gemm_ready(g)) return;
    int gst_rows = 0;
    rc = dfh::gemm_launch(g, s, 0, 0, -1, &gst_rows, rs_bn);
    if (o && gst_rows) { o->gst = gst; o->gst_cpg = g.gstat_cpg; o->gst_chunks = g.gstat_hw / gst_rows; }
  }
  void linear(const bf16_t* x, int M, int K, const Mat& W, const Vec* bias, int act, const bf16_t* resid, void* out,
              int N, int out_mode = OUT_BF16, int ld_out = -1, int rows_per_b = 0, Tensor* o = nullptr, Bump* bump = nullptr,
              float* rowstat = nullptr, int* rs_bn = nullptr) {
    GemmArgs g = linear_desc(x, M, K, W, bias, resid, out, N, out_mode);
    g.act = act; g.ld_out = ld_out < 0 ? (act == ACT_GEGLU ? N / 2 : N) : ld_out;
    if (rows_per_b) g.rows_per_b = rows_per_b;
    g.rowstat = rowstat;
    gemm(g, o, bump, rs_bn);
  }
  GemmArgs folded(const bf16_t* x, int M, const Fold& f, const float* st, int st_bn, int act, void* out, int out_mode, int ld_out,
                  int rows_per_b) const {
    GemmArgs g = base(M, f.N);
    g.p_src[0] = x; g.p_c[0] = f.K; g.nplain = 1;
    g.W = u->fold_w() + f.w; g.ldw = f.K;
    g.bias = u->fold_v() + f.b; g.ln_s = u->fold_v() + f.s;
    g.ln_stat = st; g.ln_cnt = st_bn; g.ln_parts = st_bn > 0 ? f.K / st_bn : 0; g.ln_eps = 1e-5f;
    g.act = act; g.out = out; g.out_mode = out_mode; g.ld_out = ld_out < 0 ? (act == ACT_GEGLU ? f.N / 2 : f.N) : ld_out;
    if (rows_per_b) g.rows_per_b = rows_per_b;
    return g;
  }
  void groupnorm(const Tensor& x0, const Tensor* x1, const Vec& w, const Vec& b, float eps, int silu, Tensor& out) {
    if (rc || dry) return;
    GnArgs a = gn_args(x0.p, x0.C, x1 ? x1->p : nullptr, x1 ? x1->C : 0, x0.H * x0.W, w, b, eps, silu, out.p);
    if (!x1 && x0.gst && x0.gst_cpg == x0.C / a.G) { a.pre = x0.gst; a.pre_chunks = x0.gst_chunks; }
    rc = dfh::groupnorm_launch(a, s);
  }
  bool use8(const Mat8& m) const { return u->fp8 && m.on; }
  void layernorm8(const bf16_t* x, const Vec& w, const Vec& b, uint8_t* q, float* sc, int M, int C) {
    if (rc || dry) return;
    rc = dfh::layernorm_fp8_launch(x, v32(w), v32(b), q, sc, M, C, 1e-5f, s);
  }
  void linear8(const uint8_t* q, const float* sc, int M, const Mat8& W, const Vec* bias, int act, void* out, int out_mode = OUT_BF16,
               int ld_out = -1, int rows_per_b = 0, float* amax = nullptr) {
    if (rc || dry) return;
    Fp8GemmArgs g; std::memset(&g, 0, sizeof(g));
    g.A = q; g.sA = sc; g.W = u->arena8 + W.off; g.sW = (const float*)(u->arena8 + W.soff);
    g.M = M; g.N = W.N; g.K = W.K; g.bias = bias ? v32(*bias) : nullptr; g.act = act;
    g.out = out; g.out_mode = out_mode; g.ld_out = ld_out < 0 ? (act == ACT_GEGLU ? W.N / 2 : W.N) : ld_out;
    g.rows_per_b = rows_per_b; g.zero = (const uint8_t*)zero; g.amax = amax;
    rc = dfh::gemm_fp8_launch(g, s);
  }
  Fp8GemmArgs args8(const uint8_t* A, int M, const Mat8& W, const Vec* bias, void* out) const {
    Fp8GemmArgs g; std::memset(&g, 0, sizeof(g));
    g.A = A; g.W = u->arena8 + W.off; g.sW = (const float*)(u->arena8 + W.soff);
    g.M = M; g.N = W.N; g.K = W.K; g.bias = bias ? v32(*bias) : nullptr;
    g.out = out; g.out_mode = OUT_BF16; g.ld_out = W.N; g.zero = (const uint8_t*)zero;
    return g;
  }
  void gemm8(const Fp8GemmArgs& g) {
    if (rc || dry) return;
    rc = dfh::gemm_fp8_launch(g, s);
  }
  void groupnorm8(const Tensor& x, float eps, uint8_t* q) {
    if (rc || dry) return;
    GnArgs a; std::memset(&a, 0, sizeof(a));
    a.src0 = x.p; a.C0 = x.C; a.B = B; a.HW = x.H * x.W; a.G = u->cfg.norm_num_groups; a.eps = eps; a.partial = gn_partial;
    a.out8 = q; a.q_mul = 448.0f / dfh_unet::GN_Z;
    if (x.gst && x.gst_cpg == x.C / a.G) { a.pre = x.gst; a.pre_chunks = x.gst_chunks; }
    rc = dfh::groupnorm_launch(a, s);
  }
  void attention8(const bf16_t* Q, int ldq, const bf16_t* K, int ldk, const bf16_t* Vt, int ldvt, uint8_t* O8, const float* amax, int C,
                  int heads, int Nq, int Nk, long vt_bstride = 0, const float* f8 = nullptr) {
    if (rc || dry) return;
    AttnArgs a = attn_args(Q, ldq, K, ldk, Vt, ldvt, C, heads, Nq, Nk, vt_bstride);
    if (f8) { a.f8_rq = f8; a.f8_rk = f8 + C; a.f8_rv = f8 + 2 * C; a.f8_hs = f8 + 3 * C; }
    a.O8 = O8; a.o_amax = amax;
    rc = dfh::attention_launch(a, s);
  }
  void layernorm(const bf16_t* x, const Vec& w, const Vec& b, bf16_t* y, int M, int C) {
    if (rc || dry) return;
    rc = dfh::layernorm_launch(x, v32(w), v32(b), y, M, C, 1e-5f, s);
  }
  void attention(const bf16_t* Q, int ldq, const bf16_t* K, int ldk, const bf16_t* Vt, int ldvt, bf16_t* O, int C,
                 int heads, int Nq, int Nk, long vt_bstride = 0) {
    if (rc || dry) return;
    AttnArgs a = attn_args(Q, ldq, K, ldk, Vt, ldvt, C, heads, Nq, Nk, vt_bstride);
    a.O = O;
    rc = dfh::attention_launch(a, s);
  }

  void temb_rows(const bf16_t* tsin, bf16_t* e1, bf16_t* e2, float* rows) {
    const int c0 = u->cfg.block_out_channels[0], temb = 4 * c0;
    linear(tsin, B, c0, u->te1, &u->te1b, ACT_SILU, nullptr, e1, temb);
    linear(e1, B, temb, u->te2, &u->te2b, ACT_SILU, nullptr, e2, temb);
    linear(e2, B, temb, u->tproj, &u->tprojb, ACT_NONE, nullptr, rows, u->temb_total, OUT_F32);
  }
  void text_kv_all(const void* ehs, int ehs_bf16, bf16_t* ehs16, bf16_t* kx, bf16_t* vxt) {
    const int T = u->cfg.text_len, X = u->cfg.cross_attention_dim, Tp = (T + 7) & ~7;
    if (!dry && !rc) {
      if (ehs_bf16) (void)hipMemcpyAsync(ehs16, ehs, (size_t)B * T * X * 2, hipMemcpyDeviceToDevice, s);
      else rc = dfh::cast_f32_to_bf16_launch((const float*)ehs, ehs16, (long)B * T * X, s);
    }
    linear(ehs16, B * T, X, u->kx_all, nullptr, ACT_NONE, nullptr, kx, u->x_total);
    linear(ehs16, B * T, X, u->vx_all, nullptr, ACT_NONE, nullptr, vxt, u->x_total, OUT_BF16_T, Tp, T);
  }

  Tensor conv(const Tensor& x, const ConvL& c, int stride, int ups, bool to_persist) {
    const int Ho = ups ? x.H * 2 : (stride == 2 ? x.H / 2 : x.H);
    const int Wo = ups ? x.W * 2 : (stride == 2 ? x.W / 2 : x.W);
    Tensor o = to_persist ? palloc(Ho, Wo, c.cout) : talloc(Ho, Wo, c.cout);
    if (ups == 1 && c.has_ph && u->fold_valid && kn.ups_phase && !dry && x.C == c.cin) {
      GemmArgs g = base(B * x.H * x.W, c.cout);
      g.conv_src = x.p; g.conv_c = x.C; g.ntaps = 4; g.phase2x = 1; g.nbatch = 4; g.w_bs = (long)c.cout * 4 * x.C;
      g.Hin = x.H; g.Win = x.W; g.Hout = x.H; g.Wout = x.W; g.stride = 1; g.rows_per_b = x.H * x.W;
      g.W = u->fold_w() + c.ph; g.ldw = 4 * x.C; g.bias = v32(c.b);
      g.out = o.p;
      gemm(g);
      return o;
    }
    GemmArgs g = conv_desc(x.p, x.C, x.H, x.W, Ho, Wo, stride, ups, c.w, c.b);
    g.out = o.p;
    gemm(g, &o, to_persist ? &persist : &temp);
    return o;
  }

  bf16_t* wino_in(const Tensor& x, const Tensor* x1, const Vec* nw, const Vec* nb, const bf16_t* Mprev = nullptr, const Vec* pbias = nullptr,
                  const float* prowvec = nullptr, int prv_off = 0) {
    const int C = x.C + (x1 ? x1->C : 0);
    const long mt = (long)B * (x.H / 2) * (x.W / 2);
    bf16_t* V = (bf16_t*)temp.alloc((size_t)16 * mt * C * 2);
    if (rc || dry) return V;
    if (nw) rc = dfh::gn_wino_input_launch(x.p, x.C, x1 ? x1->p : nullptr, x1 ? x1->C : 0, v32(*nw), v32(*nb), u->cfg.norm_eps,
                                           u->cfg.norm_num_groups, V, B, x.H, x.W, s, Mprev, pbias ? v32(*pbias) : nullptr, prowvec, temb_ld, prv_off);
    else rc = dfh::wino_input_launch(x.p, V, B, x.H, x.W, C, s);
    return V;
  }
  bf16_t* wino_gemm(const bf16_t* V, int H, int W, int C, size_t uoff, int cout) {
    const long mt = (long)B * (H / 2) * (W / 2);
    bf16_t* Mb = (bf16_t*)temp.alloc((size_t)16 * mt * cout * 2);
    if (rc || dry) return Mb;
    GemmArgs g = base((int)mt, cout);
    g.p_src[0] = V; g.p_c[0] = C; g.nplain = 1; g.W = u->fold_w() + uoff; g.ldw = C;
    g.nbatch = 16; g.a_bs = mt * C; g.w_bs = (long)cout * C; g.o_bs = mt * cout; g.w_blocked = dfh::wino_blocked(cout, C);
    g.out = Mb; g.zero = zero;
    g.prof_flops = 2.0 * B * H * W * (double)cout * 9.0 * C;
    rc = dfh::gemm_launch(g, s, dfh::wino_gemm_tile(g), 0, -1);
    dfh::census(dfh::CK_CONV_WINO);
    return Mb;
  }
  void wino_out(const bf16_t* Mb, const Vec& bias, const float* rowvec, int rv_off, const bf16_t* resid, Tensor& o) {
    if (rc || dry) return;
    rc = dfh::wino_output_launch(Mb, o.p, v32(bias), rowvec, temb_ld, rv_off, resid, B, o.H, o.W, o.C, s);
  }

  Tensor resnet(const Tensor& x0, const Tensor* x1, const ResL& r, const float* temb_all) {
    const int H = x0.H, W = x0.W;
    Tensor out = palloc(H, W, r.cout);
    const size_t mark = temp.off;
    Tensor g1 = talloc(H, W, r.cin);
    Tensor h1 = talloc(H, W, r.cout);
    const bool wino = r.has_u && (dry || u->fold_valid) && ((kn.wino >= 1 && H * W <= 64) || (kn.wino >= 2 && H * W <= kn.wino_maxhw));
    if (wino) {
      const int G = u->cfg.norm_num_groups;
      const bf16_t* V1;
      if (kn.wino_gn && dfh::gn_wino_ok(x0.C, x1 ? x1->C : 0, G, H, W)) V1 = wino_in(x0, x1, &r.n1w, &r.n1b);
      else {
        groupnorm(x0, x1, r.n1w, r.n1b, u->cfg.norm_eps, 1, g1);
        V1 = wino_in(g1, nullptr, nullptr, nullptr);
      }
      const bf16_t* M1 = wino_gemm(V1, H, W, r.cin, r.u1, r.cout);
      const bool gn2 = kn.wino_gn && dfh::gn_wino_ok(r.cout, 0, G, H, W);
      const bool chain = gn2 && kn.wino_chain;
      Tensor g2 = talloc(H, W, r.cout);
      const bf16_t* V2;
      if (chain) V2 = wino_in(h1, nullptr, &r.n2w, &r.n2b, M1, &r.b1, temb_all, r.temb_off);
      else {
        wino_out(M1, r.b1, temb_all, r.temb_off, nullptr, h1);
        if (gn2) V2 = wino_in(h1, nullptr, &r.n2w, &r.n2b);
        else {
          groupnorm(h1, nullptr, r.n2w, r.n2b, u->cfg.norm_eps, 1, g2);
          V2 = wino_in(g2, nullptr, nullptr, nullptr);
        }
      }
      const bf16_t* resid = x0.p;
      if (r.shortcut) {
        Tensor sc = talloc(H, W, r.cout);
        GemmArgs g = conv2_desc(nullptr, H, W, r.cout, r.w2, r.b2, true, x0.p, x0.C, x1 ? x1->p : nullptr, x1 ? x1->C : 0);
        g.out = sc.p;
        gemm(g);
        resid = sc.p;
      }
      const bf16_t* M2 = wino_gemm(V2, H, W, r.cout, r.u2, r.cout);
      wino_out(M2, r.b2, nullptr, 0, resid, out);
      temp.off = mark;
      return out;
    }
    groupnorm(x0, x1, r.n1w, r.n1b, u->cfg.norm_eps, 1, g1);
    {
      GemmArgs g = conv_desc(g1.p, r.cin, H, W, H, W, 1, 0, r.w1, r.b1);
      g.rowvec = temb_all; g.rv_ld = temb_ld; g.rv_off = r.temb_off; g.rows_per_b = H * W;
      g.out = h1.p;
      gemm(g, &h1, &temp);
    }
    Tensor g2 = talloc(H, W, r.cout);
    groupnorm(h1, nullptr, r.n2w, r.n2b, u->cfg.norm_eps, 1, g2);
    {
      GemmArgs g = conv2_desc(g2.p, H, W, r.cout, r.w2, r.b2, r.shortcut, x0.p, x0.C, x1 ? x1->p : nullptr, x1 ? x1->C : 0);
      g.out = out.p;
      gemm(g, &out, &persist);
    }
    temp.off = mark;
    return out;
  }

  struct Block {
    int C, N, Np, pre_n; bool pre;
    size_t mark; Tensor out, h0, n1, qk, at, h1, h2;
    float* st;
    uint8_t* n8; float* s8; bf16_t* vt;
  };
  Block block_enter(const Tensor& x, int C, int pre_n) {
    Block b{}; b.C = C; b.N = x.H * x.W; b.pre_n = pre_n;
    b.out = palloc(x.H, x.W, C);
    b.mark = temp.off;
    b.pre = pre_n > 0 && !dry && 2 * pre_n <= B;
    if (b.pre) B -= pre_n;
    b.st = (float*)temp.alloc((size_t)Ba * b.N * ((C + 63) / 64) * 2 * sizeof(float));
    b.h0 = talloc(x.H, x.W, C);
    return b;
  }
  void block_scratch(Block& b, bool f8) {
    const int H = b.out.H, W = b.out.W, C = b.C;
    b.n1 = talloc(H, W, C);
    b.n8 = f8 ? (uint8_t*)temp.alloc((size_t)Ba * b.N * C) : nullptr;
    b.s8 = f8 ? (float*)temp.alloc((size_t)Ba * b.N * sizeof(float)) : nullptr;
    b.qk = talloc(H, W, 2 * C);
    b.Np = (b.N + 7) & ~7;
    b.vt = (bf16_t*)temp.alloc((size_t)Ba * C * b.Np * 2);
    b.at = talloc(H, W, C); b.h1 = talloc(H, W, C); b.h2 = talloc(H, W, C);
  }
  void prefix_end(Block& b) {
    B += b.pre_n;
    dup_images(b.h0, b.pre_n);
    dfh::census(dfh::CK_DUP_PREFIX);
  }
  Tensor block_leave(const Block& b) { temp.off = b.mark; return b.out; }
  struct TextKV { const bf16_t* k; int ldk; const bf16_t* vt; int ldvt; long vt_bs; };
  TextKV text_kv(const AttL& a, const bf16_t* kx, const bf16_t* vxt, int T) const {
    const int Tp = (T + 7) & ~7, XT = u->x_total;
    return {kx + a.x_off, XT, vxt + (size_t)a.x_off * Tp, Tp, (long)XT * Tp};
  }

  Tensor transformer(const Tensor& x, const AttL& a, const bf16_t* kx, const bf16_t* vxt, int T, int pre_n = 0) {
    if (use8(a.qk8) && a.pin8.on) return transformer_fp8(x, a, kx, vxt, T, pre_n);
    const int H = x.H, W = x.W, C = a.C, N = H * W;
    const bool f8 = use8(a.qk8);
    const bool fold = u->fold_valid && kn.ln_fold && !f8 && !dry;
    Block b = block_enter(x, C, pre_n);
    Tensor &out = b.out, &h0 = b.h0;
    float* const st = b.st;
    int M = B * N, bn = 0;
    auto try_folded = [&](std::initializer_list<GemmArgs> gs) {
      if (!fold || bn <= 0 || C % bn) return false;
      for (const GemmArgs& g : gs) if (!dfh::gemm_ln_consumer_ok(g)) return false;
      for (const GemmArgs& g : gs) gemm(g);
      dfh::census(dfh::CK_LN_FOLDED);
      return true;
    };
#ifdef DFH_PROBES
    const bool tl = fold && kn.token_linear && a.has_tl && dfh::token_linear_eligible(C, C, M);
    auto token_linear = [&](const bf16_t* xin, size_t img, const float* bias, const bf16_t* resid, const Fold* f, bf16_t* o, bool stats) {
      if (rc) return;
      TokLinArgs t; std::memset(&t, 0, sizeof(t));
      t.x = xin; t.img = (const unsigned char*)(u->fold_w() + img); t.bias = bias; t.resid = resid; t.out = o; t.M = M;
      if (f) { t.ln_stat = st; t.ln_parts = C / bn; t.ln_cnt = bn; t.ln_eps = 1e-5f; t.ln_s = u->fold_v() + f->s; t.bias = u->fold_v() + f->b; }
      if (stats) t.rowstat = st;
      rc = dfh::token_linear_launch(t, s);
      if (stats) bn = C;
    };
#else
    constexpr bool tl = false;
    auto token_linear = [](const bf16_t*, size_t, const float*, const bf16_t*, const Fold*, bf16_t*, bool) {};
#endif
    const bool gfold = !tl && C <= kn.gn_fold && N % 128 == 0 && a.pin.K == C && a.pin.N == C;
    if (gfold) {
      bf16_t* wimg = (bf16_t*)temp.alloc((size_t)Ba * C * C * 2);
      float* rv = (float*)temp.alloc((size_t)Ba * C * sizeof(float));
      if (!rc && !dry) {
        GnFoldArgs f; std::memset(&f, 0, sizeof(f));
        f.x = x.p; f.B = B; f.HW = N; f.C = C; f.G = u->cfg.norm_num_groups; f.eps = 1e-6f; f.gamma = v32(a.nw); f.beta = v32(a.nb);
        if (x.gst && x.gst_cpg == C / f.G) { f.pre = x.gst; f.pre_chunks = x.gst_chunks; }
        f.partial = gn_partial; f.W = w16(a.pin); f.ldw = a.pin.K; f.N = C; f.bias = v32(a.pinb); f.Wimg = wimg; f.rv = rv;
        rc = dfh::groupnorm_fold_launch(f, s);
      }
      GemmArgs g = base(M, C);
      g.p_src[0] = x.p; g.p_c[0] = C; g.nplain = 1;
      g.W = wimg; g.ldw = C; g.w_img_bs = (long)C * C;
      g.rowvec = rv; g.rv_ld = C; g.rv_off = 0; g.rows_per_b = N;
      g.out = h0.p; g.rowstat = fold ? st : nullptr;
      gemm(g, nullptr, nullptr, &bn);
    } else {
      Tensor gn = talloc(H, W, C);
      groupnorm(x, nullptr, a.nw, a.nb, 1e-6f, 0, gn);
      if (tl) token_linear(gn.p, a.tl_pin, v32(a.pinb), nullptr, nullptr, h0.p, true);
      else linear(gn.p, M, C, a.pin, &a.pinb, ACT_NONE, nullptr, h0.p, C, OUT_BF16, -1, 0, nullptr, nullptr, fold ? st : nullptr, &bn);
    }
    block_scratch(b, f8);
    Tensor &n1 = b.n1, &qk = b.qk, &at = b.at, &h1 = b.h1, &h2 = b.h2;
    uint8_t* const n8 = b.n8; float* const s8 = b.s8; bf16_t* const vt = b.vt; const int Np = b.Np;
    auto with_v = [&](GemmArgs g) {
      g.N = 3 * C; g.out2 = vt; g.ld_out2 = Np; g.n_split = 2 * C; g.rows_per_b = N;
      return g;
    };
    const bool v_contig = a.v.off == a.qk.off + (size_t)2 * C * C && a.v.K == a.qk.K;
    bool done = false;
    if (!f8 && kn.qkv_merge && !dry) {
      GemmArgs gq = with_v(folded(h0.p, M, a.fqk, st, bn, ACT_NONE, qk.p, OUT_BF16, 2 * C, 0));
      if (dfh::gemm_out2_ok(gq)) done = try_folded({gq});
    }
    if (!done) done = try_folded({folded(h0.p, M, a.fqk, st, bn, ACT_NONE, qk.p, OUT_BF16, -1, 0),
                                  folded(h0.p, M, a.fv, st, bn, ACT_NONE, vt, OUT_BF16_T, Np, N)});
    if (!done) {
      if (f8) layernorm8(h0.p, a.l1w, a.l1b, n8, s8, M, C);
      else layernorm(h0.p, a.l1w, a.l1b, n1.p, M, C);
      bool merged = false;
      if (!f8 && kn.qkv_merge && !dry && v_contig) {
        GemmArgs g = base(M, 2 * C);
        g.p_src[0] = n1.p; g.p_c[0] = C; g.nplain = 1; g.W = w16(a.qk); g.ldw = C; g.out = qk.p; g.ld_out = 2 * C;
        g = with_v(g);
        if (dfh::gemm_out2_ok(g)) { gemm(g); merged = true; }
      }
      if (!merged) {
        if (f8) linear8(n8, s8, M, a.qk8, nullptr, ACT_NONE, qk.p);
        else linear(n1.p, M, C, a.qk, nullptr, ACT_NONE, nullptr, qk.p, 2 * C);
        if (f8) linear8(n8, s8, M, a.v8, nullptr, ACT_NONE, vt, OUT_BF16_T, Np, N);
        else linear(n1.p, M, C, a.v, nullptr, ACT_NONE, nullptr, vt, C, OUT_BF16_T, Np, N);
      }
    }
    attention(qk.p, 2 * C, qk.p + C, 2 * C, vt, Np, at.p, C, a.heads, N, N);
    if (b.pre) {
      prefix_end(b); dup_images(at, pre_n);
      M = B * N;
    }
    if (tl) token_linear(at.p, a.tl_o1, v32(a.o1b), h0.p, nullptr, h1.p, true);
    else linear(at.p, M, C, a.o1, &a.o1b, ACT_NONE, h0.p, h1.p, C, OUT_BF16, -1, 0, nullptr, nullptr, fold ? st : nullptr, &bn);
    if (tl && bn > 0 && C % bn == 0) {
      token_linear(h1.p, a.tl_q2, nullptr, nullptr, &a.fq2, qk.p, false);
      dfh::census(dfh::CK_LN_FOLDED);
    } else if (!try_folded({folded(h1.p, M, a.fq2, st, bn, ACT_NONE, qk.p, OUT_BF16, -1, 0)})) {
      if (f8) { layernorm8(h1.p, a.l2w, a.l2b, n8, s8, M, C); linear8(n8, s8, M, a.q28, nullptr, ACT_NONE, qk.p); }
      else {
        layernorm(h1.p, a.l2w, a.l2b, n1.p, M, C);
        linear(n1.p, M, C, a.q2, nullptr, ACT_NONE, nullptr, qk.p, C);
      }
    }
    const TextKV t = text_kv(a, kx, vxt, T);
    attention(qk.p, C, t.k, t.ldk, t.vt, t.ldvt, at.p, C, a.heads, N, T, t.vt_bs);
    if (tl) token_linear(at.p, a.tl_o2, v32(a.o2b), h1.p, nullptr, h2.p, true);
    else linear(at.p, M, C, a.o2, &a.o2b, ACT_NONE, h1.p, h2.p, C, OUT_BF16, -1, 0, nullptr, nullptr, fold ? st : nullptr, &bn);
    const int G = u->cfg.norm_num_groups;
    const bool mlp_gst_ok = a.has_mlp && N % 128 == 0 && C % G == 0 && N / 128 <= (int)GN_MAX_CHUNKS;
    float* mlp_gst = mlp_gst_ok ? (float*)persist.alloc((size_t)B * G * (N / 128) * 2 * sizeof(float)) : nullptr;
    Tensor ff = talloc(H, W, 4 * C);
    const bool mlp_off = dfh::mlp_fused_form() == 0;
    if (fold && !mlp_off && a.has_mlp && bn > 0 && C % bn == 0 && dfh::mlp_fused_eligible(C, M)) {
      MlpArgs ma; std::memset(&ma, 0, sizeof(ma));
      ma.x = h2.p; ma.resid = x.p; ma.img = (const unsigned char*)(u->fold_w() + a.mlp_img);
      ma.ln_stat = st; ma.ln_parts = C / bn; ma.ln_cnt = bn; ma.ln_eps = 1e-5f;
      ma.bias = u->fold_v() + a.fffp.b; ma.out = out.p; ma.M = M;
      if (dfh::mlp_fused_form() == 2 && mlp_gst && kn.gn_pre) {
        ma.gstat = mlp_gst; ma.gstat_cpg = C / G; ma.gstat_hw = N;
        out.gst = mlp_gst; out.gst_cpg = C / G; out.gst_chunks = N / 128;
        dfh::census(dfh::CK_GSTAT_WRITTEN);
      }
#ifdef DFH_PROBES
      if (!rc && dfh::mlp_fused_form() == 1) rc = dfh::mlp_fused_launch(ma, s); else
#endif
      if (!rc) rc = dfh::mlp2_fused_launch(ma, s);
      dfh::census(dfh::CK_LN_FOLDED);
      return block_leave(b);
    }
    if (!try_folded({folded(h2.p, M, a.fff1, st, bn, ACT_GEGLU, ff.p, OUT_BF16, -1, 0)})) {
      if (f8) { layernorm8(h2.p, a.l3w, a.l3b, n8, s8, M, C); linear8(n8, s8, M, a.ff18, &a.ff1b, ACT_GEGLU, ff.p); }
      else {
        layernorm(h2.p, a.l3w, a.l3b, n1.p, M, C);
        linear(n1.p, M, C, a.ff1, &a.ff1b, ACT_GEGLU, nullptr, ff.p, 8 * C);
      }
    }
    GemmArgs gf = base(M, C);
    gf.p_src[0] = ff.p; gf.p_c[0] = 4 * C; gf.p_src[1] = h2.p; gf.p_c[1] = C; gf.nplain = 2;
    gf.ldw = 5 * C; gf.resid = x.p; gf.ld_res = C; gf.out = out.p;
    if (dry) gemm(gf);
    if (u->fold_valid && kn.ffp_fold && !dry) {
      gf.W = u->fold_w() + a.fffp.w; gf.bias = u->fold_v() + a.fffp.b;
      gemm(gf, &out, &persist);
    } else {
      linear(ff.p, M, 4 * C, a.ff2, &a.ff2b, ACT_NONE, h2.p, h0.p, C);
      linear(h0.p, M, C, a.pout, &a.poutb, ACT_NONE, x.p, out.p, C, OUT_BF16, -1, 0, &out, &persist);
    }
    return block_leave(b);
  }

  Tensor transformer_fp8(const Tensor& x, const AttL& a, const bf16_t* kx, const bf16_t* vxt, int T, int pre_n) {
    const int C = a.C, N = x.H * x.W;
    Block b = block_enter(x, C, pre_n);
    uint8_t* a8 = (uint8_t*)temp.alloc((size_t)Ba * N * C);
    block_scratch(b, true);
    float* am_self = amax_self + (size_t)a.idx * Ba;
    const float* am_cross = amax_cross + (size_t)a.idx * Ba;
    int M = B * N;
    groupnorm8(x, 1e-6f, a8);
    Fp8GemmArgs g = args8(a8, M, a.pin8, nullptr, b.h0.p);
    g.bias = (const float*)(u->arena8 + a.pin8.boff); g.sa_mul = dfh_unet::GN_Z / 448.0f;
    gemm8(g);
    layernorm8(b.h0.p, a.l1w, a.l1b, b.n8, b.s8, M, C);
    linear8(b.n8, b.s8, M, a.qk8, nullptr, ACT_NONE, b.qk.p);
    linear8(b.n8, b.s8, M, a.v8, nullptr, ACT_NONE, b.vt, OUT_BF16_T, b.Np, N, am_self);
    const float* f8attn = (a.f8a && N % 64 == 0) ? (const float*)(u->arena8 + a.f8a_off) : nullptr;
    attention8(b.qk.p, 2 * C, b.qk.p + C, 2 * C, b.vt, b.Np, a8, am_self, C, a.heads, N, N, 0, f8attn);
    if (b.pre) {
      prefix_end(b); dup_bytes(a8, (size_t)N * C, pre_n); dup_bytes(am_self, sizeof(float), pre_n);
      M = B * N;
    }
    g = args8(a8, M, a.o18, &a.o1b, b.h1.p);
    g.sA = am_self; g.sa_div = N; g.sa_mul = 1.0f / 448.0f; g.resid = b.h0.p; g.ld_res = C;
    gemm8(g);
    layernorm8(b.h1.p, a.l2w, a.l2b, b.n8, b.s8, M, C);
    linear8(b.n8, b.s8, M, a.q28, nullptr, ACT_NONE, b.qk.p);
    const TextKV t = text_kv(a, kx, vxt, T);
    attention8(b.qk.p, C, t.k, t.ldk, t.vt, t.ldvt, a8, am_cross, C, a.heads, N, T, t.vt_bs);
    g = args8(a8, M, a.o28, &a.o2b, b.h2.p);
    g.sA = am_cross; g.sa_div = N; g.sa_mul = 1.0f / 448.0f; g.resid = b.h1.p; g.ld_res = C;
    gemm8(g);
    uint8_t* ff8 = (uint8_t*)temp.alloc((size_t)M * 4 * C);
    uint8_t* ffsx = (uint8_t*)temp.alloc((size_t)(4 * C / 32) * M + 256);
    uint8_t* t8 = (uint8_t*)temp.alloc((size_t)M * C);
    uint8_t* tsx = (uint8_t*)temp.alloc((size_t)(C / 32) * M + 256);
    layernorm8(b.h2.p, a.l3w, a.l3b, b.n8, b.s8, M, C);
    g = args8(b.n8, M, a.ff18, &a.ff1b, ff8);
    g.sA = b.s8; g.act = ACT_GEGLU; g.out_mode = OUT_FP8_MX; g.ld_out = 4 * C; g.out_sx = ffsx;
    gemm8(g);
    g = args8(ff8, M, a.ff28, &a.ff2b, t8);
    g.sx = ffsx; g.resid = b.h2.p; g.ld_res = C; g.out_mode = OUT_FP8_MX; g.ld_out = C; g.out_sx = tsx;
    gemm8(g);
    g = args8(t8, M, a.pout8, &a.poutb, b.out.p);
    g.sx = tsx; g.resid = x.p; g.ld_res = C;
    gemm8(g);
    return block_leave(b);
  }
};

int dfh_unet::cross_amax(const bf16_t* vxt, int B, float* out, hipStream_t s) {
  const int Tp = (cfg.text_len + 7) & ~7;
  return dfh::amax_slabs_launch(vxt, (long)x_total * Tp, Tp, cfg.text_len, slab_row0(), slab_rows(), out, n_att, B, s);
}


int dfh_unet::run(const void* sample, int sample_bf16, const float* timestep, const void* ehs, int ehs_bf16, float* out, int B,
                  hipStream_t s, bool dry, const RunCache* rcache) {
  if (!dry && B != plan.batch) run(nullptr, 0, nullptr, nullptr, 0, nullptr, B, nullptr, true);
  Run r(this, B, s, dry);
  r.temb_ld = (rcache && rcache->temb_row) ? 0 : temb_total;
  const int dup = (!dry && dup_tail > 0 && 2 * dup_tail <= B) ? dup_tail : 0;
  if (!dry) dup_tail = 0;
  const int S = cfg.sample_size, T = cfg.text_len, X = cfg.cross_attention_dim;
  const int* boc = cfg.block_out_channels;
  const int nb = cfg.num_blocks, temb = boc[0] * 4;
  if (!dry && !r.bind(ws + fold_bytes(), walk_bytes(), plan)) return r.rc;
  if (!dry && fold_dirty) { if (int rc = fold_layernorms(s)) return rc; }
  taps.clear();

  bf16_t* tsin = (bf16_t*)r.persist.alloc((size_t)B * boc[0] * 2);
  bf16_t* e1 = (bf16_t*)r.persist.alloc((size_t)B * temb * 2);
  bf16_t* e2 = (bf16_t*)r.persist.alloc((size_t)B * temb * 2);
  float* temb_all = (float*)r.persist.alloc((size_t)B * temb_total * 4);
  const bool t_cached = rcache && rcache->temb_row, x_cached = rcache && rcache->kx && rcache->vxt;
  if (!dry && !t_cached) r.rc = dfh::timestep_embed_launch(timestep, tsin, B, boc[0], s);
  if (dry || !t_cached) r.temb_rows(tsin, e1, e2, temb_all);
  else temb_all = const_cast<float*>(rcache->temb_row);

  const int Tp = (T + 7) & ~7;
  bf16_t* ehs16 = (bf16_t*)r.persist.alloc((size_t)B * T * X * 2);
  bf16_t* kx = (bf16_t*)r.persist.alloc((size_t)B * T * x_total * 2);
  bf16_t* vxt = (bf16_t*)r.persist.alloc((size_t)B * x_total * Tp * 2);
  if (dry || !x_cached) r.text_kv_all(ehs, ehs_bf16, ehs16, kx, vxt);
  else {
    kx = const_cast<bf16_t*>(rcache->kx); vxt = const_cast<bf16_t*>(rcache->vxt);
    dfh::census(dfh::CK_TEXT_CACHED);
  }
  if (fp8) {
    r.amax_self = (float*)r.persist.alloc((size_t)n_att * B * 4);
    float* xam = (float*)r.persist.alloc((size_t)n_att * B * 4);
    r.amax_cross = xam;
    if (!dry && !r.rc) {
      if (hipMemsetAsync(r.amax_self, 0, (size_t)n_att * B * 4, s) != hipSuccess) { dfh::set_error("hipMemsetAsync failed"); return -2; }
      if (x_cached && rcache->xamax) r.amax_cross = rcache->xamax;
      else r.rc = cross_amax(vxt, B, xam, s);
    }
  }
  Tensor x = r.palloc(S, S, conv_in.cin);
  if (!dry && !r.rc) r.rc = dfh::nchw_to_nhwc_launch(sample, sample_bf16, x.p, B, cfg.in_channels, S * S, s);
  if (dup && !r.rc) {
    if (dfh::WalkKnobs::get().check_dup) {
      const size_t per = (size_t)S * S * conv_in.cin * 2, n = (size_t)dup * per;
      std::vector<char> a(n), b(n);
      if (hipStreamSynchronize(s) != hipSuccess || hipMemcpy(a.data(), (char*)x.p + (size_t)(B - 2 * dup) * per, n, hipMemcpyDeviceToHost) != hipSuccess ||
          hipMemcpy(b.data(), (char*)x.p + (size_t)(B - dup) * per, n, hipMemcpyDeviceToHost) != hipSuccess) { dfh::set_error("DFH_CHECK_DUP: copy failed"); return -2; }
      if (std::memcmp(a.data(), b.data(), n) != 0) { dfh::set_error("dfh_unet_set_dup_tail: the last images do NOT repeat the inputs of the ones before them"); return -1; }
      if (timestep && !(rcache && rcache->temb_row)) {
        std::vector<float> t(B);
        if (hipMemcpy(t.data(), timestep, (size_t)B * 4, hipMemcpyDeviceToHost) != hipSuccess) { dfh::set_error("DFH_CHECK_DUP: copy failed"); return -2; }
        for (int i = 0; i < dup; ++i)
          if (t[B - dup + i] != t[B - 2 * dup + i]) { dfh::set_error("dfh_unet_set_dup_tail: the repeated images sit at other timesteps"); return -1; }
      }
    }
  }

  if (dup) r.B = B - dup;
  Tensor h = r.conv(x, conv_in, 1, 0, true);
  taps["conv_in"] = h;
  std::vector<Tensor> skips{h};
  for (int i = 0; i < nb; ++i) {
    for (int j = 0; j < cfg.layers_per_block; ++j) {
      const bool first = dup && i == 0 && j == 0;
      h = r.resnet(h, nullptr, down_res[i][j], temb_all);
      if (first) {
        r.B = B;
        r.dup_images(skips[0], dup); taps["conv_in"] = skips[0];
        if (!cfg.down_attn[i]) r.dup_images(h, dup);
        else { const float* g = h.gst; r.dup_images(h, dup); h.gst = g; }
      }
      if (cfg.down_attn[i]) h = r.transformer(h, down_att[i][j], kx, vxt, T, first ? dup : 0);
      skips.push_back(h);
    }
    if (i != nb - 1) { h = r.conv(h, down_samp[i], 2, 0, true); skips.push_back(h); }
    taps["down" + std::to_string(i)] = h;
  }
  h = r.resnet(h, nullptr, mid_res[0], temb_all);
  h = r.transformer(h, mid_att, kx, vxt, T);
  h = r.resnet(h, nullptr, mid_res[1], temb_all);
  taps["mid"] = h;
  for (int i = 0; i < nb; ++i) {
    for (int j = 0; j < (int)up_res[i].size(); ++j) {
      Tensor sk = skips.back(); skips.pop_back();
      h = r.resnet(h, &sk, up_res[i][j], temb_all);
      if (!up_att[i].empty()) h = r.transformer(h, up_att[i][j], kx, vxt, T);
    }
    if (i != nb - 1) h = r.conv(h, up_samp[i], 1, 1, true);
    taps["up" + std::to_string(i)] = h;
  }
  Tensor g = r.palloc(h.H, h.W, h.C);
  r.groupnorm(h, nullptr, cnw, cnb, cfg.norm_eps, 1, g);
  {
    GemmArgs ga = r.conv_desc(g.p, g.C, S, S, S, S, 1, 0, conv_out.w, conv_out.b);
    ga.out = out; ga.out_mode = OUT_F32_T; ga.ld_out = S * S; ga.rows_per_b = S * S;
    r.gemm(ga);
  }
  if (dry) { plan = r.plan(); taps.clear(); }
  else last_batch = B;
  return r.rc;
}

int dfh_unet::run_cache(const void* ehs, int ehs_bf16, int B, const float* timesteps, int n_t, void* cache, hipStream_t s) {
  if (B != plan.batch) run(nullptr, 0, nullptr, nullptr, 0, nullptr, B, nullptr, true);
  Run r(this, B, s, false);
  if (!r.bind(ws + fold_bytes(), walk_bytes(), plan)) return r.rc;
  const int T = cfg.text_len, X = cfg.cross_attention_dim;
  const int temb = cfg.block_out_channels[0] * 4, c0 = cfg.block_out_channels[0];
  bf16_t* kx = (bf16_t*)cache;
  bf16_t* vxt = (bf16_t*)((char*)cache + cache_kx_bytes(*this, B));
  float* table = (float*)((char*)cache + cache_kx_bytes(*this, B) + cache_vxt_bytes(*this, B));
  float* xamax = (float*)((char*)table + (((size_t)n_t * temb_total * 4 + 255) & ~(size_t)255));
  bf16_t* ehs16 = (bf16_t*)r.persist.alloc((size_t)B * T * X * 2);
  r.text_kv_all(ehs, ehs_bf16, ehs16, kx, vxt);
  if (fp8 && !r.rc) r.rc = cross_amax(vxt, B, xamax, s);
  bf16_t* tsin = (bf16_t*)r.persist.alloc((size_t)B * c0 * 2);
  bf16_t* e1 = (bf16_t*)r.persist.alloc((size_t)B * temb * 2);
  bf16_t* e2 = (bf16_t*)r.persist.alloc((size_t)B * temb * 2);
  float* trow = (float*)r.persist.alloc((size_t)B * temb_total * 4);
  for (int t0 = 0; t0 < n_t && !r.rc; t0 += B) {
    const int n = std::min(B, n_t - t0);
    r.rc = dfh::timestep_embed_launch(timesteps + t0, tsin, n, c0, s);
    if (r.rc) break;
    if (n < B) (void)hipMemsetAsync(tsin + (size_t)n * c0, 0, (size_t)(B - n) * c0 * 2, s);
    r.temb_rows(tsin, e1, e2, trow);
    if (!r.rc) (void)hipMemcpyAsync(table + (size_t)t0 * temb_total, trow, (size_t)n * temb_total * 4, hipMemcpyDeviceToDevice, s);
  }
  return r.rc;
}
```

### include/difashion_hip.h

```cpp
#ifndef DIFASHION_HIP_H
#define DIFASHION_HIP_H

#include <stddef.h>
#include <stdint.h>

#ifdef __cplusplus
extern "C" {
#endif

#define DFH_ABI_VERSION 8
#define DFH_MAX_BLOCKS 4

int dfh_abi_version(void);
const char* dfh_last_error(void);
const char* dfh_build_info(void);

typedef struct dfh_prof_class {
  char name[32];
  int launches;
  double ms, flops, bytes;
} dfh_prof_class;
int dfh_prof_begin(void);
int dfh_prof_end(dfh_prof_class* out, int max_classes);
double dfh_prof_saved_flops(void);
// ... 321 lines not shown
  int src_region, dst_region;
  size_t src_off, src_floats, dst_off, dst_floats;
  char name[48];
} dfh_incep_launch;
typedef struct dfh_incep dfh_incep;
int dfh_incep_create(const dfh_incep_config* cfg, dfh_incep** out);
void dfh_incep_destroy(dfh_incep* c);
int dfh_incep_num_params(const dfh_incep* c);
const char* dfh_incep_param_name(const dfh_incep* c, int i);
int dfh_incep_param_ndim(const dfh_incep* c, int i);
int dfh_incep_param_dim(const dfh_incep* c, int i, int d);
size_t dfh_incep_packed_bytes(const dfh_incep* c);
int dfh_incep_pack(dfh_incep* c, const float* const* params, int count, void* packed, void* stream);
int dfh_incep_plan_count(const dfh_incep* c, int n, int H, int W);
int dfh_incep_plan_entry(const dfh_incep* c, int n, int H, int W, int i, dfh_incep_launch* out);
size_t dfh_incep_workspace_bytes(const dfh_incep* c, int n, int H, int W);
int dfh_incep_forward(dfh_incep* c, const float* const* params, int count, const void* packed, const float* in, int n, int H, int W,
                      float* const* taps, float* probs, void* workspace, size_t workspace_bytes, void* stream);
int dfh_incep_prep(const float* src, int n, int H, int W, int resize, int normalize, int affine, float* out, void* stream);
int dfh_incep_conv_bn_relu(const float* x, const float* weight, int w_cin, const float* const* bn, float* packed, float* out, int n, int H, int W,
                           int C_in, int C_out, int KH, int KW, int stride, int padH, int padW, int ldc, int offset, void* stream);
int dfh_incep_pool(const float* x, float* out, int mode, int n, int H, int W, int C, int ldc, int offset, void* stream);
int dfh_incep_global_mean(const float* x, float* out, int n, int HW, int C, void* stream);
int dfh_incep_fc_softmax(const float* feat, const float* weight, const float* bias, float* logits, float* probs, int n, int K, int classes,
                         void* stream);
int dfh_incep_is_rows(const float* probs, const int64_t* cate, int n, int classes, float eps, int64_t* label, float* ent, float* kl,
                      float* correct, void* stream);
int dfh_incep_is_splits(const float* ent, const float* kl, const float* correct, int n, int splits, float* out, void* stream);
int dfh_incep_stats(const float* act, int N, int D, double* mu, double* sigma, void* stream);

typedef struct dfh_gemm_desc {
  const void* conv_src; int conv_c; int conv;
  int batch, Hin, Win, stride, upsample;
  const void* a0; int a0_c; const void* a1; int a1_c;
  const void* W; int ldw;
  int M, N;
  const float* bias;
  const float* rowvec; int rv_ld, rv_off, rows_per_b;
  const void* resid; int ld_res;
  int act;
  void* out; int ld_out; int out_mode;
  float* partial; size_t partial_floats;
  const void* zero_page;
  int force_tile, force_split, force_order;
  float* gstat; int gstat_cpg, gstat_hw;
  size_t w_img_stride;
} dfh_gemm_desc;
size_t dfh_gemm_partial_floats(const dfh_gemm_desc* d);
int dfh_gemm(const dfh_gemm_desc* d, void* stream);
int dfh_gemm_gstat(const dfh_gemm_desc* d, void* stream, int* written);
int dfh_groupnorm_fold(const void* x, int B, int HW, int C, int G, const float* gamma, const float* beta, float eps, const float* pre,
                       int pre_chunks, float* partial, const void* W, int ldw, int N, const float* bias, void* Wimg, float* rv, void* stream);
int dfh_gemm_wgrad(const dfh_gemm_desc* d, const void* dY, int ldy, float* dW, int ldw, int msplit, void* stream);
size_t dfh_gemm_wgrad_partial_floats(const dfh_gemm_desc* d, int msplit);
int dfh_gemm_wgrad_plan(const dfh_gemm_desc* d, int msplit, int* tiles, int* whole_tiles, int* slices);
typedef struct dfh_gemm_plan_extra {
  int nbatch;
  int phase2x;
  int w_blocked;
  int n_split;
  int want_rowstat;
  int ln_cnt;
  int pre_out;
} dfh_gemm_plan_extra;
typedef struct dfh_gemm_plan_info {
  int kernel;
  int tile;
  int bm, bn, stages, lean;
  int wide;
  int split;
  int n_major, tm_xm, tm_gm;
  int gstat_rows;
  int rowstat_bn;
  int census;
  char line[512];
} dfh_gemm_plan_info;
int dfh_gemm_plan(const dfh_gemm_desc* d, const dfh_gemm_plan_extra* x, dfh_gemm_plan_info* out);
int dfh_colsum(const void* Y, int ldy, int N, int groups, int rows_per_group, float* out, int ld_out, void* stream);

int dfh_groupnorm(const void* src0, int c0, const void* src1, int c1, int batch, int hw, int groups,
                  const float* gamma, const float* beta, float eps, int silu, void* out, float* partial, void* stream);
int dfh_groupnorm_pre(const void* src, int c, int batch, int hw, int groups, const float* gamma, const float* beta, float eps,
                      int silu, void* out, const float* gstat, int chunks, float* stats_out, void* stream);
int dfh_layernorm(const void* x, const float* gamma, const float* beta, void* y, int M, int C, float eps, void* stream);
int dfh_gemm_out2(const dfh_gemm_desc* d, void* out2, int ld_out2, int n_split, void* stream);
int dfh_ln_fold(const void* W, int ldw, const float* gamma, const float* beta, const float* bias, void* WF, float* s, float* b, int N, int K,
                void* stream);
int dfh_gemm_ln(const dfh_gemm_desc* d, float* rowstat, int* rowstat_bn, const float* ln_stat, int ln_parts, int ln_cnt, float ln_eps,
                const float* ln_s, void* stream);
int dfh_ups_phase_fold(const void* W, int ldw, void* WP, int N, int C, void* stream);
int dfh_conv_up2x(const void* src, int batch, int H, int W, int C, const void* WP, int N, const float* bias, void* out,
                  const void* zero_page, void* stream);
int dfh_wino_weights(const void* W, int ldw, void* U, int N, int C, int blocked, void* stream);
int dfh_wino_input(const void* src, void* V, int batch, int H, int W, int C, void* stream);
int dfh_gn_wino_input_ok(int c0, int c1, int groups, int H, int W);
int dfh_gn_wino_input(const void* src0, int c0, const void* src1, int c1, const float* gamma, const float* beta, float eps, int groups,
                      void* V, int batch, int H, int W, void* stream);
int dfh_gn_wino_input_chain(const void* Mprev, const float* pbias, const float* prowvec, int prv_ld, int prv_off, int C, const float* gamma,
                            const float* beta, float eps, int groups, void* V, int batch, int H, int W, void* stream);
int dfh_wino_blocked(int N, int C);
size_t dfh_conv3x3_wino_scratch_bytes(int batch, int H, int W, int C, int N);
int dfh_conv3x3_wino(const void* src, int batch, int H, int W, int C, const void* U, int u_blocked, int N, const float* bias, const float* rowvec,
                     int rv_ld, int rv_off, const void* resid, void* out, void* scratch, size_t scratch_bytes, const void* zero_page,
                     void* stream);
int dfh_gemm_batched(const dfh_gemm_desc* d, int nbatch, long a_bs, long w_bs, long o_bs, void* stream);
typedef struct dfh_gemm_fp8_desc {
  const void* A; int lda;
  const float* sA; int sa_div; float sa_mul;
  const void* sx;
  const void* W; const float* sW;
  int M, N, K;
  const float* bias; const void* resid; int ld_res; int act;
  void* out; int ld_out; int out_mode; void* out_sx; int rows_per_b; float* amax;
  const void* zero_page;
} dfh_gemm_fp8_desc;
int dfh_quantize_rows_fp8(const void* x, int ldx, void* q, float* scale, int R, int K, void* stream);
int dfh_layernorm_fp8(const void* x, const float* gamma, const float* beta, void* q, float* scale, int M, int C, float eps, void* stream);
int dfh_gemm_fp8(const dfh_gemm_fp8_desc* d, void* stream);
size_t dfh_mlp_fused_image_bytes(void);
int dfh_mlp_fused_pack(const void* w1, const float* s1, const float* b1, const void* w2p, void* img, int form, void* stream);
int dfh_mlp_fused(const void* x, const void* resid, const void* img, const float* ln_stat, int ln_parts, int ln_cnt, float ln_eps,
                  const float* bias, void* out, int M, int form, float* gstat, int gstat_cpg, int gstat_hw, void* stream);
int dfh_groupnorm_fp8(const void* src, int batch, int HW, int C, int groups, float eps, float q_mul, void* q, float* partial, void* stream);
int dfh_attention_fp8out(const void* Q, int ldq, const void* K, int ldk, const void* Vt, int ldvt, void* O8, int ldo, const float* v_amax,
                         int batch, int heads, int head_dim, int Nq, int Nk, float scale, void* stream);
int dfh_amax_slabs(const void* x, long bstride, int ld, int cols, const int* row0, const int* nrows, float* out, int nslab, int batch,
                   void* stream);
int dfh_attention_fp8(const void* Q, int ldq, const void* K, int ldk, const void* Vt, int ldvt, void* O, int ldo, const float* rq,
                      const float* rk, const float* rv, const float* hs, int batch, int heads, int head_dim, int Nq, int Nk, float scale,
                      void* stream);
int dfh_attn_scales(const void* wf, const float* bf, int C, int heads, float* rq, float* rk, float* rv, float* hs, void* stream);
int dfh_attention(const void* Q, int ldq, const void* K, int ldk, const void* Vt, int ldvt, void* O, int ldo,
                  int batch, int heads, int head_dim, int Nq, int Nk, float scale, void* stream);
int dfh_timestep_embedding(const float* t, void* out, int batch, int dim, void* stream);
int dfh_nchw_to_nhwc_bf16(const void* x, int x_bf16, void* out, int batch, int C, int HW, void* stream);
int dfh_cast_f32_to_bf16(const float* x, void* y, size_t n, void* stream);

int dfh_pack_conv3x3(const float* w_oihw, void* out, int Cout, int Cin, int ldw, int col_off, void* stream);
int dfh_pack_matrix(const float* w, void* out, int N, int K, int ldw, int row_off, int col_off, int geglu, void* stream);
int dfh_pack_vector(const float* v, float* out, int N, int off, int geglu, int accumulate, void* stream);

int dfh_groupnorm_stats(const void* src0, int c0, const void* src1, int c1, int batch, int hw, int groups,
                        const float* gamma, const float* beta, float eps, int silu, void* out, float* partial,
                        float* stats_out, void* stream);
int dfh_groupnorm_bwd(const void* src0, int c0, const void* src1, int c1, const void* dy, int batch, int hw, int groups,
                      const float* gamma, const float* beta, const float* stats, int silu, void* dx0, int acc0,
                      void* dx1, int acc1, float* dgamma, float* dbeta, float* partial, void* stream);
int dfh_attention_lse(const void* Q, int ldq, const void* K, int ldk, const void* Vt, int ldvt, void* O, int ldo,
                      int batch, int heads, int head_dim, int Nq, int Nk, float scale, float* lse, void* stream);
int dfh_attention_delta(const void* O, const void* dO, int ld, float* delta, int batch, int heads, int head_dim, int Nq, void* stream);
int dfh_attention_bwd(const void* Q, int ldq, const void* K, int ldk, const void* V, int ldv, const void* dO, int ldo,
                      const float* lse, const float* delta, void* dQ, int lddq, void* dK, int lddk, void* dV, int lddv,
                      int batch, int heads, int head_dim, int Nq, int Nk, float scale, void* stream);
int dfh_layernorm_bwd(const void* x, const void* dy, const float* gamma, void* dx, int accumulate, float* dgamma,
                      float* dbeta, int M, int C, float eps, void* stream);
int dfh_pack_matrix_t(const float* w, void* out, int N, int K, int ldt, int t_row_off, int t_col_off, int geglu, void* stream);
int dfh_pack_conv3x3_t(const float* w, void* out, int Cout, int Cin, int ldt, int t_col_off, int o_pad, void* stream);
int dfh_unpack_matrix(const float* g, float* grad, int N, int K, int ldw, int row_off, int col_off, int geglu, void* stream);
int dfh_unpack_conv3x3(const float* g, float* grad, int Cout, int Cin, int ldw, int col_off, int cin_pad, void* stream);
int dfh_unpack_vector(const float* g, float* grad, int N, int off, int geglu, void* stream);
int dfh_pool2x2_sum(const void* in, void* out, int batch, int H, int W, int C, void* stream);
int dfh_add_bf16(void* dst, const void* src, size_t n, int accumulate, void* stream);
int dfh_geglu_fwd(const void* pre, void* y, size_t M, int N2, void* stream);
int dfh_geglu_bwd(const void* pre, const void* dy, void* dpre, size_t M, int N2, void* stream);
int dfh_act_fwd(const void* pre, void* y, size_t n, int kind, void* stream);
int dfh_act_bwd(const void* ref_bf16, const float* ref_f32, const void* dy_bf16, const float* dy_f32, void* dpre, size_t n,
                int kind, float scale, void* stream);
int dfh_nhwc_to_nchw_f32(const void* src, float* dst, int batch, int HW, int Cp, int C, float scale, int accumulate, void* stream);
int dfh_transpose_bf16(const void* in, void* out, int batch, int R, int C, int ld_in, int ld_out, size_t in_bstride,
                       size_t out_bstride, void* stream);
int dfh_mse_bwd(const float* pred, const float* target, const float* w, float* dpred, int rows, int L, float loss_scale,
                const float* scale_dev , void* stream);
int dfh_assemble_bwd(const float* dx, const uint8_t* mutual_real, float* dmutual, int rows, int CL, float eta, void* stream);
int dfh_sumsq(const float* g, size_t n, float* out, void* stream);
int dfh_adamw(float* p, const float* g, float* m, float* v, size_t n, float lr, float beta1, float beta2, float eps,
// ... 48 lines not shown
```

Measured before the change: 64.77 steps/s.

## Reuse producer GroupNorm statistics for concatenated up-block inputs

The up-path resnets apply GroupNorm to a concat of the hidden state and a skip tensor. Previously that always went through a separate statistics kernel. Now producers (the folded FF GEMM, the 2x upsample phase conv, and skips) write per-record partial sums at a granularity compatible with the concat's group split. The GroupNorm apply kernel can then combine records from both sources directly, and only a source without producer statistics gets a small stats launch. The upsample phase-conv epilogue gains phase-aware chunk indexing, and image duplication now keeps the statistics by copying them. This adds complexity in record bookkeeping and carries a risk of mismatch if the groups and channels per record do not align.

```diff
diff --git a/difashion_amd/_lib.py b/difashion_amd/_lib.py
--- a/difashion_amd/_lib.py
+++ b/difashion_amd/_lib.py
@@ -316,6 +316,7 @@
     "dfh_groupnorm": (_i, [_vp, _i, _vp, _i, _i, _i, _i, _vp, _vp, _f, _i, _vp, _vp, _vp]),
     "dfh_gemm_gstat": (_i, [C.POINTER(GemmDesc), _vp, C.POINTER(C.c_int)]),
     "dfh_groupnorm_pre": (_i, [_vp, _i, _i, _i, _i, _vp, _vp, _f, _i, _vp, _vp, _i, _vp, _vp]),
+    "dfh_groupnorm_cat_pre": (_i, [_vp, _i, _vp, _i, _i, _i, _i, _vp, _vp, _f, _i, _vp, _vp, _i, _i, _vp, _i, _i, _vp, _vp, _vp]),
     "dfh_groupnorm_stats": (_i, [_vp, _i, _vp, _i, _i, _i, _i, _vp, _vp, _f, _i, _vp, _vp, _vp, _vp]),
     "dfh_groupnorm_bwd": (_i, [_vp, _i, _vp, _i, _vp, _i, _i, _i, _vp, _vp, _vp, _i, _vp, _i, _vp, _i, _vp, _vp, _vp, _vp]),
     "dfh_attention_lse": (_i, [_vp, _i, _vp, _i, _vp, _i, _vp, _i, _i, _i, _i, _i, _i, _f, _vp, _vp]),
@@ -352,6 +353,7 @@
     "dfh_gemm_out2": (_i, [C.POINTER(GemmDesc), _vp, _i, _i, _vp]),
     "dfh_ups_phase_fold": (_i, [_vp, _i, _vp, _i, _i, _vp]),
     "dfh_conv_up2x": (_i, [_vp, _i, _i, _i, _i, _vp, _i, _vp, _vp, _vp, _vp]),
+    "dfh_conv_up2x_gstat": (_i, [_vp, _i, _i, _i, _i, _vp, _i, _vp, _vp, _vp, _i, _vp, _i, C.POINTER(C.c_int), _vp]),
     "dfh_wino_weights": (_i, [_vp, _i, _vp, _i, _i, _i, _vp]),
     "dfh_wino_blocked": (_i, [_i, _i]),
     "dfh_prof_saved_flops": (C.c_double, []),
diff --git a/difashion_amd/csrc/api.hip b/difashion_amd/csrc/api.hip
--- a/difashion_amd/csrc/api.hip
+++ b/difashion_amd/csrc/api.hip
@@ -32,7 +32,7 @@
 static long g_census[CK_COUNT] = {0};
 void census(int id) { if (id >= 0 && id < CK_COUNT) ++g_census[id]; }
 static const char* const kCensusNames[CK_COUNT] = {"gemm_wide", "gemm_8wave", "gemm_lean", "gemm_other", "gemm_row", "splitk_reduce",
-    "splitk_fused", "gstat_written", "gn_pre", "gn_stats", "gn_small", "gn_mid", "layernorm", "ln_folded", "attention_x32", "attention_16",
+    "splitk_fused", "gstat_written", "gn_pre", "gn_stats", "gn_small", "gn_mid", "gn_pre_cat", "layernorm", "ln_folded", "attention_x32", "attention_16",
     "gemm_fp8", "text_cached", "conv_phase", "conv_wino", "gemm_rows_geglu", "attention_fp8", "mlp_fused", "gn_folded", "token_linear", "dup_prefix", "gemm_persist",
     "clipv_embed", "clipv_linear", "clipv_layernorm", "clipv_attention", "imgproc", "cliph_attention", "cliph_embed"};
 
@@ -249,6 +249,18 @@
   return dfh::groupnorm_launch(a, (hipStream_t)stream);
 }
 
+int dfh_groupnorm_cat_pre(const void* src0, int c0, const void* src1, int c1, int batch, int hw, int groups, const float* gamma,
+                          const float* beta, float eps, int silu, void* out, const float* gstat0, int chunks0, int u0, const float* gstat1,
+                          int chunks1, int u1, float* partial, float* stats_out, void* stream) {
+  DFH_REQUIRE(src1 != nullptr && c1 > 0, "dfh_groupnorm_cat_pre: two sources");
+  GnArgs a; std::memset(&a, 0, sizeof(a));
+  a.src0 = (const bf16_t*)src0; a.C0 = c0; a.src1 = (const bf16_t*)src1; a.C1 = c1;
+  a.B = batch; a.HW = hw; a.G = groups; a.gamma = gamma; a.beta = beta; a.eps = eps; a.silu = silu;
+  a.out = (bf16_t*)out; a.partial = partial; a.stats_out = stats_out;
+  a.pre = gstat0; a.pre_chunks = chunks0; a.pre_u = u0; a.pre1 = gstat1; a.pre1_chunks = chunks1; a.pre1_u = u1;
+  return dfh::groupnorm_launch(a, (hipStream_t)stream);
+}
+
 int dfh_groupnorm_stats(const void* src0, int c0, const void* src1, int c1, int batch, int hw, int groups, const float* gamma,
                         const float* beta, float eps, int silu, void* out, float* partial, float* stats_out, void* stream) {
   GnArgs a; std::memset(&a, 0, sizeof(a));
@@ -463,6 +475,21 @@
   g.Hin = H; g.Win = W; g.Hout = H; g.Wout = W; g.stride = 1;
   g.W = (const bf16_t*)WP; g.ldw = 4 * C; g.bias = bias; g.out = out; g.zero = (const bf16_t*)zero_page;
   return dfh::gemm_launch(g, (hipStream_t)stream, 0, 0, -1);
+}
+int dfh_conv_up2x_gstat(const void* src, int batch, int H, int W, int C, const void* WP, int N, const float* bias, void* out,
+                        const void* zero_page, int force_tile, float* gstat, int gstat_cpg, int* written, void* stream) {
+  DFH_REQUIRE(src && WP && out && zero_page && gstat && written, "null argument");
+  DFH_REQUIRE(batch > 0 && H > 0 && W > 0 && C > 0 && C % 8 == 0 && N > 0 && N % 8 == 0, "bad shape (C and N multiples of 8)");
+  GemmArgs g; std::memset(&g, 0, sizeof(g));
+  g.M = batch * H * W; g.N = N; g.rows_per_b = H * W; g.out_mode = OUT_BF16; g.ld_out = N;
+  g.conv_src = (const bf16_t*)src; g.conv_c = C; g.ntaps = 4; g.phase2x = 1; g.nbatch = 4; g.w_bs = (long)N * 4 * C;
+  g.Hin = H; g.Win = W; g.Hout = H; g.Wout = W; g.stride = 1;
+  g.W = (const bf16_t*)WP; g.ldw = 4 * C; g.bias = bias; g.out = out; g.zero = (const bf16_t*)zero_page;
+  g.gstat = gstat; g.gstat_cpg = gstat_cpg; g.gstat_hw = 4 * H * W;
+  int rows = 0;
+  const int rc = dfh::gemm_launch(g, (hipStream_t)stream, force_tile, 0, -1, &rows);
+  *written = rows;
+  return rc;
 }
 int dfh_wino_weights(const void* W, int ldw, void* U, int N, int C, int blocked, void* stream) {
   return dfh::wino_weight_launch((const bf16_t*)W, ldw, (bf16_t*)U, N, C, blocked, (hipStream_t)stream);
diff --git a/difashion_amd/csrc/dfh_common.h b/difashion_amd/csrc/dfh_common.h
--- a/difashion_amd/csrc/dfh_common.h
+++ b/difashion_amd/csrc/dfh_common.h
@@ -246,7 +246,7 @@
 enum ProfClass { PC_CONV3 = 0, PC_LINEAR = 1, PC_ATTN = 2, PC_GNORM = 3, PC_LNORM = 4, PC_SPLITK = 5, PC_OTHER = 6,
                  PC_WGRAD = 7, PC_ATTN_BWD = 8, PC_NORM_BWD = 9, PC_OPTIM = 10, PC_LINEAR_FP8 = 11, PC_COUNT = 12 };
 enum CensusId { CK_GEMM_WIDE = 0, CK_GEMM_8WAVE, CK_GEMM_LEAN, CK_GEMM_OTHER, CK_GEMM_ROW, CK_SPLITK, CK_SPLITK_FUSED, CK_GSTAT_WRITTEN,
-                CK_GN_PRE, CK_GN_STATS, CK_GN_SMALL, CK_GN_MID, CK_LAYERNORM, CK_LN_FOLDED, CK_ATTN_X32, CK_ATTN_16, CK_GEMM_FP8,
+                CK_GN_PRE, CK_GN_STATS, CK_GN_SMALL, CK_GN_MID, CK_GN_PRE_CAT, CK_LAYERNORM, CK_LN_FOLDED, CK_ATTN_X32, CK_ATTN_16, CK_GEMM_FP8,
                 CK_TEXT_CACHED, CK_CONV_PHASE, CK_CONV_WINO, CK_GEMM_ROWS_GEGLU, CK_ATTN_FP8, CK_MLP_FUSED, CK_GN_FOLDED, CK_TOKEN_LINEAR, CK_DUP_PREFIX, CK_GEMM_PERSIST,
                 CK_CLIPV_EMBED, CK_CLIPV_LINEAR, CK_CLIPV_LAYERNORM, CK_CLIPV_ATTN, CK_IMGPROC, CK_CLIPH_ATTN, CK_CLIPH_EMBED, CK_COUNT };
 void census(int id);
diff --git a/difashion_amd/csrc/gemm_plan.h b/difashion_amd/csrc/gemm_plan.h
--- a/difashion_amd/csrc/gemm_plan.h
+++ b/difashion_amd/csrc/gemm_plan.h
@@ -28,6 +28,7 @@
   bool batch_big_off;
   bool batch_nmajor_off;
   bool gstat128_off;
+  bool gn_cat_pre;
   bool ws_on, halo_on;
   int persist_mode;
   static GemmKnobs defaults();
diff --git a/difashion_amd/csrc/gemm_plan.hip b/difashion_amd/csrc/gemm_plan.hip
--- a/difashion_amd/csrc/gemm_plan.hip
+++ b/difashion_amd/csrc/gemm_plan.hip
@@ -56,6 +56,7 @@
     k.batch_big_off = is("DFH_BATCH_BIG", '0');
     k.batch_nmajor_off = is("DFH_BATCH_NMAJOR", '0');
     k.gstat128_off = is("DFH_GSTAT128", '0');
+    k.gn_cat_pre = is("DFH_GN_CAT_PRE", '1');
     k.ws_on = is("DFH_GEMM_WS", '1'); k.halo_on = is("DFH_GEMM_HALO", '1'); k.persist_mode = num("DFH_PERSIST", 0);
     return k;
   }();
@@ -216,7 +217,8 @@
   const bool tile = p.kernel == GK_TILE || p.kernel == GK_PERSIST;
   const bool staged = p.split == 1 && a.out_mode == OUT_BF16 && (a.N & 7) == 0 && (a.ld_out & 7) == 0;
   const int gbn = big ? 320 : 160;
-  const bool gst256 = (halo || big || wide1) && a.M % 256 == 0 && gstat_chunks_fit(a.gstat_hw, 256);
+  const bool phase_ok = !a.phase2x || (big && a.rows_per_b % 256 == 0 && a.gstat_hw == 4 * a.rows_per_b);
+  const bool gst256 = (halo || big || wide1) && a.M % 256 == 0 && gstat_chunks_fit(a.gstat_hw, 256) && phase_ok;
   const bool gst128 = !k.gstat128_off && tile && p.tile == kEightWave && staged && a.M % 128 == 0 && gstat_chunks_fit(a.gstat_hw, 128) &&
                       a.nbatch <= 1 && !a.phase2x && a.out2 == nullptr;
   const bool gst_ok = a.gstat && (gst256 || gst128) && a.gstat_cpg > 0 && gbn % a.gstat_cpg == 0 && a.N % gbn == 0 &&
@@ -273,7 +275,7 @@
     PLAN_REQUIRE(((a.ntaps == 0 && a.nplain == 1) || (a.phase2x && a.nplain == 0)) && a.out_mode == OUT_BF16 && a.act != ACT_GEGLU &&
                  !a.resid && !a.rowvec && !a.out2 && !a.rowstat && !a.ln_stat && (a.N & 7) == 0 && (a.ld_out & 7) == 0 && f.split <= 1,
                  "batched launch: one plain segment (or the four phase planes of an upsample conv), plain bf16 row-major output, no split-K");
-    a.gstat = nullptr;
+    if (!a.phase2x) a.gstat = nullptr;
     if (f.tile == 0 && !f.deep) tile = (a.N % 160 == 0) ? kEightWave : 4;
   }
   PLAN_REQUIRE(!a.phase2x || (a.nbatch == 4 && a.ntaps == 4 && a.stride == 1 && a.ups == 0 && !a.pad0 && a.Hin == a.Hout && a.Win == a.Wout &&
diff --git a/difashion_amd/csrc/gemm_wide_epilogue.h b/difashion_amd/csrc/gemm_wide_epilogue.h
--- a/difashion_amd/csrc/gemm_wide_epilogue.h
+++ b/difashion_amd/csrc/gemm_wide_epilogue.h
@@ -201,7 +201,8 @@
     if (tid < BN / cpg) {
       float ss = 0.f, qq = 0.f;
       for (int c = tid * cpg; c < (tid + 1) * cpg; ++c) { ss += cst[c * 2]; qq += cst[c * 2 + 1]; }
-      const int b = m0 / a.gstat_hw, chunk = (m0 - b * a.gstat_hw) / BM, chunks = a.gstat_hw / BM;
+      const int hw = a.phase2x ? a.gstat_hw / 4 : a.gstat_hw, chunks = a.gstat_hw / BM;
+      const int b = m0 / hw, chunk = (a.phase2x ? (int)blockIdx.y * (hw / BM) : 0) + (m0 - b * hw) / BM;
       const int g = (n0 + tid * cpg) / cpg, G = a.N / cpg;
       float* dst = a.gstat + (((long)b * G + g) * chunks + chunk) * 2;
       dst[0] = ss; dst[1] = qq;
diff --git a/difashion_amd/csrc/norm.h b/difashion_amd/csrc/norm.h
--- a/difashion_amd/csrc/norm.h
+++ b/difashion_amd/csrc/norm.h
@@ -15,7 +15,9 @@
   float* partial;
   float* stats_out;
   const float* pre; int pre_chunks;
+  int pre_u; const float* pre1; int pre1_chunks, pre1_u;
   int C, PL, chunks, pix_per_chunk, apix_per_chunk;
+  const float* rec_p[2]; int rec_chunks[2], rec_u[2], rec_split;
 };
 
 struct GnBwdArgs {
diff --git a/difashion_amd/csrc/norm.hip b/difashion_amd/csrc/norm.hip
--- a/difashion_amd/csrc/norm.hip
+++ b/difashion_amd/csrc/norm.hip
@@ -83,7 +83,7 @@
   float gmr[8], btr[8];
   if (live && !a.out8) { load8f(a.gamma + o * 8, gmr); load8f(a.beta + o * 8, btr); }
   __shared__ float2 run_s[64][8];
-  const float2 sums = gn_chunk_sums(a.partial, a.chunks, a.G, b, blockDim.x >= (unsigned)a.G * 8u, run_s);
+  const float2 sums = gn_record_sums([&](int g) { return gn_group_records(a, b, g); }, a.G, blockDim.x >= (unsigned)a.G * 8u, run_s);
   if (tid < a.G) {
     const float2 mr = gn_mean_rstd(sums, (float)a.HW * (float)cpg, a.eps);
     mean_s[tid] = mr.x;
@@ -378,15 +378,14 @@
 namespace dfh {
 
 namespace {
-enum GnPath { GN_PRODUCER_STATS, GN_ONE_SLAB, GN_GROUP_QUAD, GN_TWO_KERNEL };
+enum GnPath { GN_PRODUCER_STATS, GN_ONE_SLAB, GN_GROUP_QUAD, GN_TWO_KERNEL, GN_CAT_RECORDS };
 struct GnPlan {
   GnPath path;
   int units;
   int gq, ppb, threads;
 };
 
-GnPlan gn_select(const GnArgs& a, const WalkKnobs& knobs) {
-  if (a.pre) return {GN_PRODUCER_STATS, 0, 0, 0, 0};
+GnPlan gn_select_shape(const GnArgs& a, const WalkKnobs& knobs) {
   const int cpg = a.C / a.G, upp = cpg >> 2;
   const long slab = (long)a.HW * upp;
   const bool one_source_per_group = a.C1 == 0 || a.C0 % cpg == 0;
@@ -409,6 +408,45 @@
   }
   return {GN_TWO_KERNEL, 0, 0, 0, 0};
 }
+
+GnPlan gn_select(const GnArgs& a, const WalkKnobs& knobs) {
+  if (a.C1 == 0 && a.pre) return {GN_PRODUCER_STATS, 0, 0, 0, 0};
+  if (a.C1 > 0 && a.pre && a.pre1) return {GN_CAT_RECORDS, 0, 0, 0, 0};
+  const GnPlan shape = gn_select_shape(a, knobs);
+  if (a.C1 > 0 && (a.pre || a.pre1) && shape.path == GN_TWO_KERNEL) return {GN_CAT_RECORDS, 0, 0, 0, 0};
+  return shape;
+}
+
+int gcd_int(int x, int y) { while (y) { const int t = x % y; x = y; y = t; } return x; }
+
+int gn_cat_records(GnArgs& a, const WalkKnobs& knobs, hipStream_t stream) {
+  const int cpg = a.C / a.G;
+  const float* pre[2] = {a.pre, a.pre1};
+  const int chunks[2] = {a.pre_chunks, a.pre1_chunks}, us[2] = {a.pre_u, a.pre1_u}, Cs[2] = {a.C0, a.C1};
+  const bf16_t* srcs[2] = {a.src0, a.src1};
+  a.rec_split = a.C0;
+  for (int i = 0; i < 2; ++i) {
+    if (pre[i]) {
+      DFH_REQUIRE(us[i] > 0 && cpg % us[i] == 0 && a.C0 % us[i] == 0, "producer statistics of a concat: the channels per record must divide (C0 + C1) / G and C0");
+      DFH_REQUIRE(chunks[i] > 0 && chunks[i] <= (int)GN_MAX_CHUNKS, "producer statistics: 1..64 chunks");
+      a.rec_p[i] = pre[i]; a.rec_chunks[i] = chunks[i]; a.rec_u[i] = us[i];
+      continue;
+    }
+    DFH_REQUIRE(a.partial != nullptr, "null pointer");
+    GnArgs s; std::memset(&s, 0, sizeof(s));
+    const int u = gcd_int(cpg, a.C0);
+    s.src0 = srcs[i]; s.C0 = s.C = Cs[i]; s.B = a.B; s.HW = a.HW; s.G = Cs[i] / u; s.partial = a.partial;
+    const int cap = std::max(1, (int)GN_MAX_CHUNKS * a.G / s.G);
+    GnTwoKernel tk{};
+    if (int rc = gn_two_kernel_geometry(s, std::min(knobs.gn_sc, a.B * cap), knobs.gn_ac, &tk)) return rc;
+    DFH_REQUIRE(s.G <= tk.block && s.chunks <= cap, "GroupNorm over a concat: too many statistics records in the source without producer statistics");
+    census(CK_GN_STATS);
+    hipLaunchKernelGGL(gn_stats_kernel, dim3(s.chunks, s.B), dim3(tk.block), tk.lds, stream, s);
+    if (int rc = check_launch("gn_stats_kernel")) return rc;
+    a.rec_p[i] = a.partial; a.rec_chunks[i] = s.chunks; a.rec_u[i] = u;
+  }
+  return 0;
+}
 }
 
 int groupnorm_launch(GnArgs a, hipStream_t stream) {
@@ -419,17 +457,28 @@
   DFH_REQUIRE((a.partial != nullptr || a.pre != nullptr) && (a.out != nullptr || a.out8 != nullptr) && a.src0 != nullptr, "null pointer");
   if (a.out8) DFH_REQUIRE(a.C1 == 0 && !a.silu && a.q_mul > 0.f && !a.stats_out, "e4m3 GroupNorm output: one source, no SiLU, a positive scale");
   DFH_REQUIRE(a.C1 == 0 || a.src1 != nullptr, "second source missing");
-  if (a.pre) DFH_REQUIRE(a.C1 == 0 && a.pre_chunks > 0 && a.pre_chunks <= (int)GN_MAX_CHUNKS, "producer statistics: one source, 1..64 chunks");
+  DFH_REQUIRE(a.C1 > 0 || a.pre1 == nullptr, "producer statistics of a second source without a second source");
+  const int cpg = a.C / a.G;
+  if (a.pre && a.C1 == 0) {
+    DFH_REQUIRE(a.pre_chunks > 0 && a.pre_chunks <= (int)GN_MAX_CHUNKS, "producer statistics: 1..64 chunks");
+    DFH_REQUIRE(a.pre_u == 0 || cpg % a.pre_u == 0, "producer statistics: the channels per record must divide C / G");
+  }
   const WalkKnobs& knobs = WalkKnobs::get();
   const GnPlan plan = gn_select(a, knobs);
   GnTwoKernel tk{};
-  if (plan.path == GN_PRODUCER_STATS || plan.path == GN_TWO_KERNEL)
+  if (plan.path == GN_PRODUCER_STATS || plan.path == GN_TWO_KERNEL || plan.path == GN_CAT_RECORDS)
     if (int rc = gn_two_kernel_geometry(a, knobs.gn_sc, knobs.gn_ac, &tk)) return rc;
   ProfScope ps(PC_GNORM, 0.0, (a.out8 ? 3.0 : 4.0) * a.B * (double)a.HW * a.C, stream);
+  a.rec_split = a.C; a.rec_u[0] = cpg;
   switch (plan.path) {
     case GN_PRODUCER_STATS:
-      a.partial = const_cast<float*>(a.pre); a.chunks = a.pre_chunks;
+      a.rec_p[0] = a.pre; a.rec_chunks[0] = a.pre_chunks;
+      if (a.pre_u) a.rec_u[0] = a.pre_u;
       census(CK_GN_PRE);
+      break;
+    case GN_CAT_RECORDS:
+      if (int rc = gn_cat_records(a, knobs, stream)) return rc;
+      census(CK_GN_PRE_CAT);
       break;
     case GN_ONE_SLAB: {
       const auto kernel = plan.units == 8 ? gn_small_kernel<8> : plan.units == 16 ? gn_small_kernel<16> : gn_small_kernel<32>;
@@ -445,9 +494,11 @@
       return check_launch("gn_mid_kernel");
     }
     case GN_TWO_KERNEL:
+      DFH_REQUIRE(a.partial != nullptr, "null pointer");
       census(CK_GN_STATS);
       hipLaunchKernelGGL(gn_stats_kernel, dim3(a.chunks, a.B), dim3(tk.block), tk.lds, stream, a);
       if (int rc = check_launch("gn_stats_kernel")) return rc;
+      a.rec_p[0] = a.partial; a.rec_chunks[0] = a.chunks;
       break;
   }
   hipLaunchKernelGGL(gn_apply_kernel, dim3(tk.achunks, a.B), dim3(tk.block), 0, stream, a);
diff --git a/difashion_amd/csrc/norm_steps.h b/difashion_amd/csrc/norm_steps.h
--- a/difashion_amd/csrc/norm_steps.h
+++ b/difashion_amd/csrc/norm_steps.h
@@ -13,15 +13,29 @@
   f[0] = lo.x; f[1] = lo.y; f[2] = lo.z; f[3] = lo.w; f[4] = hi.x; f[5] = hi.y; f[6] = hi.z; f[7] = hi.w;
 }
 
-DFH_DEVICE float2 gn_chunk_sums(const float* partial, int chunks, int G, int b, bool wide, float2 (*run_s)[8]) {
+struct GnRecords { const float2* p0; int n0; const float2* p1; int n1; };
+template <class Records>
+DFH_DEVICE float2 gn_record_sums(Records records, int G, bool wide, float2 (*run_s)[8]) {
   const int tid = threadIdx.x;
   if (wide) {
     if (tid < G * 8) {
       const int g = tid >> 3, sub = tid & 7;
-      const int per = (chunks + 7) >> 3, c0 = sub * per, c1 = min(chunks, c0 + per);
-      const float2* src = (const float2*)(partial + ((long)b * G + g) * chunks * 2);
+      const GnRecords r = records(g);
+      const int n = r.n0 + r.n1;
+      const int per = (n + 7) >> 3, c0 = sub * per, c1 = min(n, c0 + per);
       float ss = 0.f, qq = 0.f;
-      for (int c = c0; c < c1; ++c) { const float2 v = src[c]; ss += v.x; qq += v.y; }
+      for (int c = c0; c < c1; c += 4) {
+        float2 v[4];
+#pragma unroll
+        for (int i = 0; i < 4; ++i) {
+          const int k = c + i;
+          v[i] = float2{0.f, 0.f};
+          if (k < c1) v[i] = k < r.n0 ? r.p0[k] : r.p1[k - r.n0];
+        }
+#pragma unroll
+        for (int i = 0; i < 4; ++i)
+          if (c + i < c1) { ss += v[i].x; qq += v[i].y; }
+      }
       run_s[g][sub] = float2{ss, qq};
     }
     __syncthreads();
@@ -32,11 +46,33 @@
 #pragma unroll
       for (int sub = 0; sub < 8; ++sub) { ss += run_s[tid][sub].x; qq += run_s[tid][sub].y; }
     } else {
-      const float2* src = (const float2*)(partial + ((long)b * G + tid) * chunks * 2);
-      for (int c = 0; c < chunks; ++c) { ss += src[c].x; qq += src[c].y; }
+      const GnRecords r = records(tid);
+      for (int c = 0; c < r.n0; ++c) { ss += r.p0[c].x; qq += r.p0[c].y; }
+      for (int c = 0; c < r.n1; ++c) { ss += r.p1[c].x; qq += r.p1[c].y; }
     }
   }
   return float2{ss, qq};
+}
+DFH_DEVICE float2 gn_chunk_sums(const float* partial, int chunks, int G, int b, bool wide, float2 (*run_s)[8]) {
+  return gn_record_sums([&](int g) { return GnRecords{(const float2*)(partial + ((long)b * G + g) * chunks * 2), chunks, nullptr, 0}; },
+                        G, wide, run_s);
+}
+
+template <class Args>
+DFH_DEVICE GnRecords gn_group_records(const Args& a, int b, int g) {
+  const int cpg = a.C / a.G, lo = g * cpg, hi = lo + cpg, mid = min(max(a.rec_split, lo), hi);
+  GnRecords r{nullptr, 0, nullptr, 0};
+  if (mid > lo) {
+    const int u = a.rec_u[0], ch = a.rec_chunks[0];
+    r.p0 = (const float2*)a.rec_p[0] + ((long)b * (a.rec_split / u) + lo / u) * ch;
+    r.n0 = (mid - lo) / u * ch;
+  }
+  if (hi > mid) {
+    const int u = a.rec_u[1], ch = a.rec_chunks[1];
+    r.p1 = (const float2*)a.rec_p[1] + ((long)b * ((a.C - a.rec_split) / u) + (mid - a.rec_split) / u) * ch;
+    r.n1 = (hi - mid) / u * ch;
+  }
+  return r;
 }
 
 DFH_DEVICE float2 gn_mean_rstd(float2 sums, float n, float eps) {
diff --git a/difashion_amd/csrc/unet_walk.hip b/difashion_amd/csrc/unet_walk.hip
--- a/difashion_amd/csrc/unet_walk.hip
+++ b/difashion_amd/csrc/unet_walk.hip
@@ -5,6 +5,7 @@
   int temb_ld = 0;
   float* amax_self = nullptr; const float* amax_cross = nullptr;
   const dfh::WalkKnobs& kn = dfh::WalkKnobs::get();
+  const bool cat_pre = dfh::GemmKnobs::from_env().gn_cat_pre;
 
   int Ba;
   Run(dfh_unet* u_, int B_, hipStream_t s_, bool dry_) : WalkBase(*u_, u_->cfg.norm_num_groups, B_, s_, dry_), u(u_), Ba(B_) {}
@@ -18,18 +19,25 @@
     }
   }
   void dup_images(Tensor& t, int n) {
-    t.gst = nullptr;
+    if (t.gst && cat_pre) dup_bytes(const_cast<float*>(t.gst), (size_t)(t.C / t.gst_cpg) * t.gst_chunks * 2 * sizeof(float), n);
+    else t.gst = nullptr;
     dup_bytes(t.p, (size_t)t.H * t.W * t.C * 2, n);
   }
-
-  void gemm(GemmArgs g, Tensor* o = nullptr, Bump* bump = nullptr, int* rs_bn = nullptr) {
+  int cat_u(int C0, int C1) const {
+    int x = (C0 + C1) / groups, y = C0;
+    while (y) { const int t = x % y; x = y; y = t; }
+    return x;
+  }
+
+  void gemm(GemmArgs g, Tensor* o = nullptr, Bump* bump = nullptr, int* rs_bn = nullptr, int out_u = 0) {
     if (rs_bn) *rs_bn = 0;
     if (rc) return;
     float* gst = nullptr;
     const int G = groups;
     if (o && bump && kn.gn_pre && o->C % G == 0 && (dfh::gstat_chunks_fit(o->H * o->W, 256) || dfh::gstat_chunks_fit(o->H * o->W, 128))) {
-      gst = (float*)bump->alloc((size_t)Ba * G * ((o->H * o->W) / 128) * 2 * sizeof(float));
-      g.gstat = gst; g.gstat_cpg = o->C / G; g.gstat_hw = o->H * o->W;
+      const int recs = out_u > 0 && o->C % out_u == 0 ? std::max(G, o->C / out_u) : G;
+      gst = (float*)bump->alloc((size_t)Ba * recs * ((o->H * o->W) / 128) * 2 * sizeof(float));
+      g.gstat = gst; g.gstat_cpg = (recs > G && cat_pre) ? out_u : o->C / G; g.gstat_hw = o->H * o->W;
     }
     if (!gemm_ready(g)) return;
     int gst_rows = 0;
@@ -60,6 +68,12 @@
     if (rc || dry) return;
     GnArgs a = gn_args(x0.p, x0.C, x1 ? x1->p : nullptr, x1 ? x1->C : 0, x0.H * x0.W, w, b, eps, silu, out.p);
     if (!x1 && x0.gst && x0.gst_cpg == x0.C / a.G) { a.pre = x0.gst; a.pre_chunks = x0.gst_chunks; }
+    if (x1 && cat_pre) {
+      const int cpg = (x0.C + x1->C) / a.G;
+      const auto fits = [&](const Tensor& t) { return t.gst && t.gst_cpg > 0 && cpg % t.gst_cpg == 0 && x0.C % t.gst_cpg == 0; };
+      if (fits(x0)) { a.pre = x0.gst; a.pre_chunks = x0.gst_chunks; a.pre_u = x0.gst_cpg; }
+      if (fits(*x1)) { a.pre1 = x1->gst; a.pre1_chunks = x1->gst_chunks; a.pre1_u = x1->gst_cpg; }
+    }
     rc = dfh::groupnorm_launch(a, s);
   }
   bool use8(const Mat8& m) const { return u->fp8 && m.on; }
@@ -132,7 +146,7 @@
     linear(ehs16, B * T, X, u->vx_all, nullptr, ACT_NONE, nullptr, vxt, u->x_total, OUT_BF16_T, Tp, T);
   }
 
-  Tensor conv(const Tensor& x, const ConvL& c, int stride, int ups, bool to_persist) {
+  Tensor conv(const Tensor& x, const ConvL& c, int stride, int ups, bool to_persist, int out_u = 0) {
     const int Ho = ups ? x.H * 2 : (stride == 2 ? x.H / 2 : x.H);
     const int Wo = ups ? x.W * 2 : (stride == 2 ? x.W / 2 : x.W);
     Tensor o = to_persist ? palloc(Ho, Wo, c.cout) : talloc(Ho, Wo, c.cout);
@@ -142,12 +156,13 @@
       g.Hin = x.H; g.Win = x.W; g.Hout = x.H; g.Wout = x.W; g.stride = 1; g.rows_per_b = x.H * x.W;
       g.W = u->fold_w() + c.ph; g.ldw = 4 * x.C; g.bias = v32(c.b);
       g.out = o.p;
-      gemm(g);
+      if (out_u > 0 && cat_pre) gemm(g, &o, to_persist ? &persist : &temp, nullptr, out_u);
+      else gemm(g);
       return o;
     }
     GemmArgs g = conv_desc(x.p, x.C, x.H, x.W, Ho, Wo, stride, ups, c.w, c.b);
     g.out = o.p;
-    gemm(g, &o, to_persist ? &persist : &temp);
+    gemm(g, &o, to_persist ? &persist : &temp, nullptr, out_u);
     return o;
   }
 
@@ -180,13 +195,16 @@
     rc = dfh::wino_output_launch(Mb, o.p, v32(bias), rowvec, temb_ld, rv_off, resid, B, o.H, o.W, o.C, s);
   }
 
+  bool resnet_wino(const ResL& r, int H, int W) const {
+    return r.has_u && (dry || u->fold_valid) && ((kn.wino >= 1 && H * W <= 64) || (kn.wino >= 2 && H * W <= kn.wino_maxhw));
+  }
   Tensor resnet(const Tensor& x0, const Tensor* x1, const ResL& r, const float* temb_all) {
     const int H = x0.H, W = x0.W;
     Tensor out = palloc(H, W, r.cout);
     const size_t mark = temp.off;
     Tensor g1 = talloc(H, W, r.cin);
     Tensor h1 = talloc(H, W, r.cout);
-    const bool wino = r.has_u && (dry || u->fold_valid) && ((kn.wino >= 1 && H * W <= 64) || (kn.wino >= 2 && H * W <= kn.wino_maxhw));
+    const bool wino = resnet_wino(r, H, W);
     if (wino) {
       const int G = u->cfg.norm_num_groups;
       const bf16_t* V1;
@@ -278,7 +296,7 @@
     return {kx + a.x_off, XT, vxt + (size_t)a.x_off * Tp, Tp, (long)XT * Tp};
   }
 
-  Tensor transformer(const Tensor& x, const AttL& a, const bf16_t* kx, const bf16_t* vxt, int T, int pre_n = 0) {
+  Tensor transformer(const Tensor& x, const AttL& a, const bf16_t* kx, const bf16_t* vxt, int T, int pre_n = 0, int out_u = 0) {
     if (use8(a.qk8) && a.pin8.on) return transformer_fp8(x, a, kx, vxt, T, pre_n);
     const int H = x.H, W = x.W, C = a.C, N = H * W;
     const bool f8 = use8(a.qk8);
@@ -420,7 +438,7 @@
     if (dry) gemm(gf);
     if (u->fold_valid && kn.ffp_fold && !dry) {
       gf.W = u->fold_w() + a.fffp.w; gf.bias = u->fold_v() + a.fffp.b;
-      gemm(gf, &out, &persist);
+      gemm(gf, &out, &persist, nullptr, out_u);
     } else {
       linear(ff.p, M, 4 * C, a.ff2, &a.ff2b, ACT_NONE, h2.p, h0.p, C);
       linear(h0.p, M, C, a.pout, &a.poutb, ACT_NONE, x.p, out.p, C, OUT_BF16, -1, 0, &out, &persist);
@@ -555,7 +573,7 @@
         r.B = B;
         r.dup_images(skips[0], dup); taps["conv_in"] = skips[0];
         if (!cfg.down_attn[i]) r.dup_images(h, dup);
-        else { const float* g = h.gst; r.dup_images(h, dup); h.gst = g; }
+        else { const float* g = h.gst; h.gst = nullptr; r.dup_images(h, dup); h.gst = g; }
       }
       if (cfg.down_attn[i]) h = r.transformer(h, down_att[i][j], kx, vxt, T, first ? dup : 0);
       skips.push_back(h);
@@ -567,13 +585,20 @@
   h = r.transformer(h, mid_att, kx, vxt, T);
   h = r.resnet(h, nullptr, mid_res[1], temb_all);
   taps["mid"] = h;
+  const auto next_u = [&](int i, int j, const Tensor& x0) {
+    if (i >= nb || j >= (int)up_res[i].size() || r.resnet_wino(up_res[i][j], x0.H, x0.W)) return 0;
+    return r.cat_u(x0.C, up_res[i][j].cin - x0.C);
+  };
   for (int i = 0; i < nb; ++i) {
     for (int j = 0; j < (int)up_res[i].size(); ++j) {
       Tensor sk = skips.back(); skips.pop_back();
       h = r.resnet(h, &sk, up_res[i][j], temb_all);
-      if (!up_att[i].empty()) h = r.transformer(h, up_att[i][j], kx, vxt, T);
-    }
-    if (i != nb - 1) h = r.conv(h, up_samp[i], 1, 1, true);
+      if (!up_att[i].empty()) h = r.transformer(h, up_att[i][j], kx, vxt, T, 0, next_u(i, j + 1, h));
+    }
+    if (i != nb - 1) {
+      Tensor up{nullptr, h.H * 2, h.W * 2, up_samp[i].cout};
+      h = r.conv(h, up_samp[i], 1, 1, true, next_u(i + 1, 0, up));
+    }
     taps["up" + std::to_string(i)] = h;
   }
   Tensor g = r.palloc(h.H, h.W, h.C);
diff --git a/include/difashion_hip.h b/include/difashion_hip.h
--- a/include/difashion_hip.h
+++ b/include/difashion_hip.h
@@ -427,6 +427,9 @@
                   const float* gamma, const float* beta, float eps, int silu, void* out, float* partial, void* stream);
 int dfh_groupnorm_pre(const void* src, int c, int batch, int hw, int groups, const float* gamma, const float* beta, float eps,
                       int silu, void* out, const float* gstat, int chunks, float* stats_out, void* stream);
+int dfh_groupnorm_cat_pre(const void* src0, int c0, const void* src1, int c1, int batch, int hw, int groups, const float* gamma,
+                          const float* beta, float eps, int silu, void* out, const float* gstat0, int chunks0, int u0, const float* gstat1,
+                          int chunks1, int u1, float* partial, float* stats_out, void* stream);
 int dfh_layernorm(const void* x, const float* gamma, const float* beta, void* y, int M, int C, float eps, void* stream);
 int dfh_gemm_out2(const dfh_gemm_desc* d, void* out2, int ld_out2, int n_split, void* stream);
 int dfh_ln_fold(const void* W, int ldw, const float* gamma, const float* beta, const float* bias, void* WF, float* s, float* b, int N, int K,
@@ -436,6 +439,8 @@
 int dfh_ups_phase_fold(const void* W, int ldw, void* WP, int N, int C, void* stream);
 int dfh_conv_up2x(const void* src, int batch, int H, int W, int C, const void* WP, int N, const float* bias, void* out,
                   const void* zero_page, void* stream);
+int dfh_conv_up2x_gstat(const void* src, int batch, int H, int W, int C, const void* WP, int N, const float* bias, void* out,
+                        const void* zero_page, int force_tile, float* gstat, int gstat_cpg, int* written, void* stream);
 int dfh_wino_weights(const void* W, int ldw, void* U, int N, int C, int blocked, void* stream);
 int dfh_wino_input(const void* src, void* V, int batch, int H, int W, int C, void* stream);
 int dfh_gn_wino_input_ok(int c0, int c1, int groups, int H, int W);
```

Result: no change. 64.70 steps/s (-0.1%).
